# jtschwar/tomo_TV

Hardware: AMD Instinct MI355X
Metric: SART+TV Gvoxel-updates/s (ASD-POCS outer iterations x voxels, 512x512x512 x 90 tilts, at 1/2/4/8 GPU) (higher is better)
Workload: dtype f32; 1 GPU; ASD-POCS iteration (SART sweep beta0=0.25 + 10 TV-GD steps) on ONE 512x512x512 volume, 90 tilts -70..70 deg (headline SART+TV 512^3x90 = BASELINE configs[2] shape), 512 slices on rank 0; volume=512x512x512, slices_per_gpu=512, nray=512, nproj=90, sub_slab_engines_per_gpu=1, sart_chains_per_engine=1

## Files before the change

include/tomo_hip.h:

```cpp
#ifndef TOMO_HIP_H
#define TOMO_HIP_H

#include <stdint.h>

#ifdef __cplusplus
extern "C" {
#endif

typedef struct tomo_engine tomo_engine;

enum tomo_status { TOMO_OK = 0, TOMO_ERR_ARG = 1, TOMO_ERR_HIP = 2, TOMO_ERR_STATE = 3, TOMO_ERR_GEOMETRY = 4 };

enum tomo_volume { TOMO_VOL_RECON = 0, TOMO_VOL_TEMP = 1, TOMO_VOL_ORIGINAL = 2, TOMO_VOL_YK = 3, TOMO_VOL_RECON_OLD = 4,
                   TOMO_VOL_COUNT = 5,
                   TOMO_VOL_USER0 = 5,
                   TOMO_VOL_SLOTS = 5 + 40 };
enum tomo_sinogram { TOMO_SINO_B = 0, TOMO_SINO_G = 1, TOMO_SINO_R = 2 ,
                     TOMO_SINO_USER0 = 3,
                     TOMO_SINO_SLOTS = 3 + 40,
                     TOMO_SINO_YK_MODEL = 1000 };

enum tomo_scalar { TOMO_S_DD = 0,
                   TOMO_S_DIFF = 1,
                   TOMO_S_TV = 2,
// ... 49 lines not shown
int tomo_sirt_data(tomo_engine *e, int vol, int sino_b, int niter);
int tomo_sart(tomo_engine *e, int vol, float beta, int niter, const int32_t *order);
int tomo_sart_data(tomo_engine *e, int vol, int sino_b, float beta, int niter, const int32_t *order);
int tomo_sart_tracked(tomo_engine *e, int vol, int sino_b, float beta, int niter, const int32_t *order, int track_vol, int slot);
int tomo_cgls(tomo_engine *e, int vol, int niter);
int tomo_fbp(tomo_engine *e, const float *taps_host, float scale, int apply_positivity);
int tomo_art(tomo_engine *e, float beta);
int tomo_art_order(tomo_engine *e, float beta, const int32_t *order_host);
int tomo_poisson_ml(tomo_engine *e, float lambda);
int tomo_poisson_residual(tomo_engine *e, int vol, int sino_b, int sino_out);
int tomo_scale_volume(tomo_engine *e, int vol, float factor);
int tomo_positivity(tomo_engine *e, int vol);
int tomo_soft_threshold(tomo_engine *e, int vol, float lambda);
int tomo_fista_momentum(tomo_engine *e, float beta);
int tomo_fista_project_yk(tomo_engine *e, int *done);

int tomo_data_distance_sq(tomo_engine *e, int vol);
int tomo_data_distance_sq_async(tomo_engine *e, int vol);
int tomo_async_wait(tomo_engine *e);
int tomo_diff_norm_sq(tomo_engine *e, int a, int b, int slot);
int tomo_sino_diff_norm_sq(tomo_engine *e, int a, int b, int slot);
int tomo_sino_proj_max(tomo_engine *e, int sino, float *out_host);
int tomo_sino_proj_scale(tomo_engine *e, int sino, const float *div_host, const float *mul_host);
int tomo_l1_norm(tomo_engine *e, int vol);
int tomo_read_scalars(tomo_engine *e, double *out, int count);
int tomo_scalars_snapshot(tomo_engine *e);
int tomo_scalars_snapshot_read(tomo_engine *e, double *out, int count);
int tomo_bind_scalar_buffer(tomo_engine *e, void *device_doubles);

int tomo_bind_halo(tomo_engine *e, void *device_lo, void *device_hi);
int tomo_halo_pack(tomo_engine *e, int field, int last, void *device_dst);
int tomo_halo_pack_both(tomo_engine *e, int field, void *first_plane, void *last_plane);
int tomo_halo_local(tomo_engine *e, int field);
enum tomo_field { TOMO_FIELD_FGP_D = 100, TOMO_FIELD_FGP_P1 = 101 };
int tomo_wait_for(tomo_engine *e, tomo_engine *other);
int tomo_halo_from(tomo_engine *e, int field, tomo_engine *lo_src, tomo_engine *hi_src);
int tomo_scalar_sum_from(tomo_engine *e, int dst_slot, tomo_engine **srcs, int n, int src_slot);
int tomo_set_slab_edges(tomo_engine *e, int is_first, int is_last);

int tomo_tv_set_target(tomo_engine *e, int vol);
int tomo_tv_partial(tomo_engine *e, int vol, float eps);
int tomo_tv_grad(tomo_engine *e, float eps);
int tomo_tv_grad_tv(tomo_engine *e, float eps);
int tomo_tv_update(tomo_engine *e, float dPOCS, int clamp);
int tomo_tv_update_planes(tomo_engine *e, float dPOCS, int clamp, void *first_plane, void *last_plane);
int tomo_tv_grad_planes(tomo_engine *e, float eps, int with_tv, void *g_first, void *g_last);
int tomo_tv_halo_apply(tomo_engine *e, float dPOCS, int clamp, const void *g_lo, const void *g_hi);
int tomo_tv_update_tracked(tomo_engine *e, float dPOCS, int clamp, int track_vol, int slot);
int tomo_fgp_begin(tomo_engine *e);
int tomo_fgp_begin_vol(tomo_engine *e, int vol);
int tomo_fgp_obj(tomo_engine *e, float lambda);
int tomo_fgp_grad(tomo_engine *e, float lambda);
int tomo_fgp_end(tomo_engine *e, int iters);
int tomo_bind_fgp_halo(tomo_engine *e, void *lo, void *hi, void *send_first, void *send_last);
int tomo_bind_fgp_halo2(tomo_engine *e, void *lo, void *hi, void *send_first, void *send_last);
int tomo_fgp_fused_begin(tomo_engine *e, int vol);
int tomo_fgp_fused_step(tomo_engine *e, float lambda, int first_iteration);
int tomo_fgp_fused_step2(tomo_engine *e, float lambda, int first_iteration);
int tomo_fgp_fused_end(tomo_engine *e, float lambda);
int tomo_fgp_fused_last(tomo_engine *e, float lambda, int first_iteration);

int tomo_tv(tomo_engine *e, int vol, float eps);
int tomo_tv_gd(tomo_engine *e, int ng, float dPOCS, float eps);
int tomo_tv_gd_tracked(tomo_engine *e, int ng, float dPOCS, float eps, int track_vol, int slot);
int tomo_tv_fgp(tomo_engine *e, int iters, float lambda);
int tomo_tv_fgp_vol(tomo_engine *e, int vol, int iters, float lambda);
// ... 40 lines not shown
```

tomo_tv_amd/_lib.py:

```python
import ctypes
import os
import sys

_HERE = os.path.dirname(os.path.abspath(__file__))
LIB_PATH = os.path.join(_HERE, "libtomo_hip.so")

VOL_RECON, VOL_TEMP, VOL_ORIGINAL, VOL_YK, VOL_RECON_OLD = 0, 1, 2, 3, 4
SINO_B, SINO_G, SINO_R, SINO_USER0 = 0, 1, 2, 3
SINO_YK_MODEL = 1000
VOL_USER0 = 5
S_DD, S_DIFF, S_TV, S_GNORM, S_RMSE, S_COST, S_L1, S_DIFF2, S_GNORM_ALL, S_COUNT = 0, 1, 2, 3, 4, 5, 6, 7, 8, 16
FIELD_FGP_D, FIELD_FGP_P1 = 100, 101
K_BP_ANGLE, K_FP_ANGLE, K_TV_GRAD, K_TV_UPDATE, K_FGP_OBJ, K_FGP_GRAD, K_SART_FUSED, K_FP_TILE, K_BP_TILE, K_FP_REDUCE, K_SART_RESIDENT = range(11)
FORM_FP = ("rows", "tile", "strip", "list")
FORM_BP = ("all", "tile", "list")
FORM_SART = ("angle", "tile", "resident")

_i, _i64, _f, _p = ctypes.c_int, ctypes.c_int64, ctypes.c_float, ctypes.c_void_p
_pp = ctypes.POINTER(ctypes.c_void_p)

SIGNATURES = {
    "tomo_device_count": [ctypes.POINTER(_i)],
    "tomo_system_matrix": [_i, _i, _p, _i64, _p, _p, _p, ctypes.POINTER(_i64)],
    "tomo_create": [_i, _i, _i, _p, _i, _pp],
# ... 13 lines not shown
    "tomo_copy_volume": [_p, _i, _i],
    "tomo_copy_volume_from": [_p, _i, _p, _i],
    "tomo_forward_projection": [_p, _i, _i],
    "tomo_back_projection": [_p, _i, _i],
    "tomo_lipschitz": [_p, ctypes.POINTER(_f)],
    "tomo_row_inner_product": [_p],
    "tomo_sirt_landweber": [_p, _i, _f, _i],
    "tomo_sirt": [_p, _i, _i],
    "tomo_sirt_cimmino": [_p, _i, _f, _i],
    "tomo_lipschitz_cimmino": [_p, ctypes.POINTER(_f)],
    "tomo_release_geometry": [_p],
    "tomo_adopt_volumes": [_p, _p],
    "tomo_sart": [_p, _i, _f, _i, _p],
    "tomo_art": [_p, _f],
    "tomo_art_order": [_p, _f, _p],
    "tomo_poisson_ml": [_p, _f],
    "tomo_positivity": [_p, _i],
    "tomo_soft_threshold": [_p, _i, _f],
    "tomo_fista_momentum": [_p, _f],
    "tomo_fista_project_yk": [_p, ctypes.POINTER(_i)],
    "tomo_data_distance_sq": [_p, _i],
    "tomo_diff_norm_sq": [_p, _i, _i, _i],
    "tomo_data_distance_sq_async": [_p, _i],
    "tomo_async_wait": [_p],
    "tomo_l1_norm": [_p, _i],
    "tomo_read_scalars": [_p, _p, _i],
    "tomo_scalars_snapshot": [_p],
    "tomo_scalars_snapshot_read": [_p, _p, _i],
    "tomo_bind_scalar_buffer": [_p, _p],
    "tomo_bind_halo": [_p, _p, _p],
    "tomo_halo_pack": [_p, _i, _i, _p],
    "tomo_halo_pack_both": [_p, _i, _p, _p],
    "tomo_halo_local": [_p, _i],
    "tomo_set_slab_edges": [_p, _i, _i],
    "tomo_wait_for": [_p, _p],
    "tomo_halo_from": [_p, _i, _p, _p],
    "tomo_scalar_sum_from": [_p, _i, _p, _i, _i],
    "tomo_profile_intervals": [_p, _i, _p, _p, _p, _i, ctypes.POINTER(_i)],
    "tomo_tv_partial": [_p, _i, _f],
    "tomo_tv_set_target": [_p, _i],
    "tomo_tv_grad": [_p, _f],
    "tomo_tv_grad_tv": [_p, _f],
    "tomo_tv_update": [_p, _f, _i],
    "tomo_fgp_begin": [_p],
    "tomo_fgp_obj": [_p, _f],
    "tomo_fgp_grad": [_p, _f],
    "tomo_fgp_end": [_p, _i],
    "tomo_tv": [_p, _i, _f],
    "tomo_tv_gd": [_p, _i, _f, _f],
    "tomo_tv_fgp": [_p, _i, _f],
    "tomo_set_option": [_p, ctypes.c_char_p, _i],
    "tomo_get_option": [_p, ctypes.c_char_p, ctypes.POINTER(_i)],
    "tomo_set_sinogram": [_p, _i, _p],
    "tomo_cgls": [_p, _i, _i],
    "tomo_fbp": [_p, _p, _f, _i],
    "tomo_sirt_data": [_p, _i, _i, _i],
    "tomo_sart_data": [_p, _i, _i, _f, _i, _p],
    "tomo_sart_tracked": [_p, _i, _i, _f, _i, _p, _i, _i],
    "tomo_tv_update_tracked": [_p, _f, _i, _i, _i],
    "tomo_tv_update_planes": [_p, _f, _i, _p, _p],
    "tomo_tv_grad_planes": [_p, _f, _i, _p, _p],
    "tomo_tv_halo_apply": [_p, _f, _i, _p, _p],
    "tomo_tv_gd_tracked": [_p, _i, _f, _f, _i, _i],
    "tomo_poisson_residual": [_p, _i, _i, _i],
    "tomo_scale_volume": [_p, _i, _f],
    "tomo_sino_diff_norm_sq": [_p, _i, _i, _i],
# ... 74 lines not shown
```

tomo_tv_amd/csrc/engine_api.inc:

```


const char *tomo_last_error(void) { return g_err.c_str(); }

int tomo_device_count(int *count)
{
    if (!count) return fail(TOMO_ERR_ARG, "null count");
    int n = 0;
    hipError_t err = hipGetDeviceCount(&n);
    if (err != hipSuccess) { n = 0; (void)hipGetLastError(); }
    *count = n;
    return TOMO_OK;
}

int tomo_system_matrix(int nray, int nproj, const double *angles_rad, int64_t cap, float *rows, float *cols,
                       float *vals, int64_t *nnz)
{
    if (!angles_rad || !nnz) return fail(TOMO_ERR_ARG, "null argument");
    int rc = check_dims(1, nray, nproj);
    if (rc) return rc;
    Coo m;
    build_parallel_ray(nray, nproj, angles_rad, m);
    *nnz = m.ptr[m.nrow];
    if (cap == 0) return TOMO_OK;
    if (cap < *nnz || !rows || !cols || !vals) return fail(TOMO_ERR_ARG, "output capacity too small");
// ... 41 lines not shown
                     (void **)&e->d_rowcross, (void **)&e->d_cell,
                     (void **)&e->d_fs_items, (void **)&e->d_fs_orient, (void **)&e->d_fs_shift, (void **)&e->d_fs_cnt, (void **)&e->d_fs_gstart,
                     (void **)&e->d_fs_gseg0, (void **)&e->d_fs_ent, (void **)&e->d_fs_zero, (void **)&e->d_fs_rsptr, (void **)&e->d_fs_rsidx, (void **)&e->fs_part, (void **)&e->fs_part_aux,
                     (void **)&e->d_fl_items, (void **)&e->d_fl_orient, (void **)&e->d_fl_shift, (void **)&e->d_fl_ent, (void **)&e->d_fl_ptr, (void **)&e->d_fl_fent, (void **)&e->d_fl_fptr,
                     (void **)&e->d_fl_rsptr, (void **)&e->d_fl_rsidx, (void **)&e->d_fl_zero, (void **)&e->fl_part, (void **)&e->fl_part_aux,
                     (void **)&e->d_rs_hdr, (void **)&e->d_rs_cell, (void **)&e->d_rs_ts, (void **)&e->d_rs_rl, (void **)&e->rs_pb, (void **)&e->rs_rb, (void **)&e->d_rs_angs, (void **)&e->d_rs_abort, (void **)&e->d_rs_commit};
    for (void **p : ptrs) if (*p) { (void)hipFree(*p); *p = nullptr; }
    e->rs_ok = false; e->rs_angs_cap = 0; e->rs_angs_host.clear(); e->seg_ready = false;
    for (int i = 0; i < TOMO_SINO_SLOTS; ++i) if (e->sino[i]) { (void)hipFree(e->sino[i]); e->sino[i] = nullptr; }
    if (e->g_prev) { (void)hipFree(e->g_prev); e->g_prev = nullptr; }
    if (e->g_yk) { (void)hipFree(e->g_yk); e->g_yk = nullptr; }
    e->yk_claim.valid = false;
    e->g_prev_valid = e->mom_p_ok = e->mom.set = false;
    e->geometry_released = true;
}

int tomo_destroy(tomo_engine *e)
{
    if (!e) return TOMO_OK;
    (void)hipSetDevice(e->device);
    if (e->stream) (void)hipStreamSynchronize(e->stream);
    if (e->aux) { (void)hipStreamSynchronize(e->aux); (void)hipStreamDestroy(e->aux); (void)hipEventDestroy(e->ev_fork); (void)hipEventDestroy(e->ev_join); }
    for (int u = 0; u < tomo_engine::MAX_CHAINS; ++u) if (e->sub_stream[u]) { (void)hipStreamSynchronize(e->sub_stream[u]); (void)hipStreamDestroy(e->sub_stream[u]); (void)hipEventDestroy(e->ev_sjoin[u]); }
    for (int w = 0; w < 2; ++w) if (e->fp_red_stream[w]) { (void)hipStreamSynchronize(e->fp_red_stream[w]); (void)hipStreamDestroy(e->fp_red_stream[w]); for (int h = 0; h < 2; ++h) { (void)hipEventDestroy(e->ev_fp_tile[w][h]); (void)hipEventDestroy(e->ev_fp_red[w][h]); } }
    comm_release(e);
    if (e->ev_sfork) (void)hipEventDestroy(e->ev_sfork);
    if (e->ev_peer) (void)hipEventDestroy(e->ev_peer);
    if (e->ev_snap) (void)hipEventDestroy(e->ev_snap);
    if (e->h_snap) (void)hipHostFree(e->h_snap);
    if (e->rs_abort) (void)hipHostFree(e->rs_abort);
    if (e->rs_done) (void)hipHostFree(e->rs_done);
    free_geometry(e);
    void *ptrs[] = {e->tv_alt, e->halo_lo_alt, e->halo_hi_alt, e->d_part_tv, e->d_part_aux, e->fgp_q[0], e->fgp_q[1], e->fgp_q[2], e->cg_p, e->cg_z, e->cg_sums, e->cg_part, e->cg_coef, e->sart_alt,
                    e->tvg, e->fgp_p[0], e->fgp_p[1], e->fgp_p[2], e->stage, e->d_scal_own, e->d_part, e->halo_lo_own, e->halo_hi_own};
    for (void *p : ptrs) if (p) (void)hipFree(p);
    for (int i = 0; i < TOMO_VOL_SLOTS; ++i) if (e->vol[i]) (void)hipFree(e->vol[i]);
    for (auto &p : e->prof) { for (auto ev : p.ev) (void)hipEventDestroy(ev); if (p.ref) (void)hipEventDestroy(p.ref); }
    if (e->own_stream && e->stream) (void)hipStreamDestroy(e->stream);
    delete e;
    return TOMO_OK;
}

int tomo_release_geometry(tomo_engine *e)
{
    NEED(e);
    HIPCHK(hipStreamSynchronize(e->stream));
    if (e->aux) HIPCHK(hipStreamSynchronize(e->aux));
    for (int u = 0; u < tomo_engine::MAX_CHAINS; ++u) if (e->sub_stream[u]) HIPCHK(hipStreamSynchronize(e->sub_stream[u]));
    e->async_pending = false;
    free_geometry(e);
    return TOMO_OK;
}

int tomo_adopt_volumes(tomo_engine *dst, tomo_engine *src)
{
    if (!dst || !src) return fail(TOMO_ERR_ARG, "null engine");
    if (dst->nx != src->nx || dst->n != src->n || dst->sx != src->sx || dst->device != src->device) return fail(TOMO_ERR_ARG, "engines differ in slab shape or device");
    HIPCHK(hipSetDevice(dst->device));
    HIPCHK(hipStreamSynchronize(src->stream));
    if (src->aux) HIPCHK(hipStreamSynchronize(src->aux));
    for (int u = 0; u < tomo_engine::MAX_CHAINS; ++u) if (src->sub_stream[u]) HIPCHK(hipStreamSynchronize(src->sub_stream[u]));
    src->async_pending = false;
    HIPCHK(hipStreamSynchronize(dst->stream));
    for (int i = 0; i < TOMO_VOL_SLOTS; ++i) {
        if (!src->vol[i]) continue;
        if (dst->vol[i]) HIPCHK(hipFree(dst->vol[i]));
        dst->vol[i] = src->vol[i];
        src->vol[i] = nullptr;
    }
    dst->old_is_recon = src->old_is_recon;
    src->old_is_recon = false;
    for (int i = 0; i < TOMO_VOL_SLOTS; ++i) ++dst->vol_version[i];
    g_clear(dst);
    return TOMO_OK;
}

int tomo_set_stream(tomo_engine *e, void *hip_stream)
{
    NEED(e);
    HIPCHK(hipStreamSynchronize(e->stream));
    if (e->own_stream) { HIPCHK(hipStreamDestroy(e->stream)); e->own_stream = false; }
    e->stream = (hipStream_t)hip_stream;
    return TOMO_OK;
}

int tomo_synchronize(tomo_engine *e) { NEED(e); HIPCHK(hipStreamSynchronize(e->stream)); return TOMO_OK; }
int tomo_get_device(tomo_engine *e, int *device) { if (!e || !device) return fail(TOMO_ERR_ARG, "null"); *device = e->device; return TOMO_OK; }
int tomo_get_dims(tomo_engine *e, int *nslice, int *nray, int *nproj, int64_t *nnz)
{
    if (!e) return fail(TOMO_ERR_ARG, "null engine");
    if (nslice) *nslice = e->nx;
    if (nray) *nray = e->n;
    if (nproj) *nproj = e->np;
    if (nnz) *nnz = e->nnz;
    return TOMO_OK;
}

int tomo_sart_chain_count(tomo_engine *e, int *count)
{
    if (!e || !count) return fail(TOMO_ERR_ARG, "null");
    *count = chain_count(e);
    return TOMO_OK;
}

static int upload(tomo_engine *e, const float *host, float *dst, int64_t m)
{
// ... 22 lines not shown
}

int tomo_set_sinogram(tomo_engine *e, int which, const float *b)
{
    NEED(e);
    if (!b) return fail(TOMO_ERR_ARG, "null sinogram");
    float *dst; int rc = sino_slot(e, which, &dst); if (rc) return rc;
    return upload(e, b, dst, e->nrows);
}

int tomo_set_tilt_series(tomo_engine *e, const float *b) { return tomo_set_sinogram(e, TOMO_SINO_B, b); }

int tomo_get_sinogram(tomo_engine *e, int which, float *out)
{
    NEED(e);
    if (!out) return fail(TOMO_ERR_ARG, "null output");
    if (which == TOMO_SINO_YK_MODEL) {
        const float *yk = projection_in_hand(e, TOMO_VOL_YK);
        if (!yk) return fail(TOMO_ERR_STATE, "no projection of the extrapolated point in hand (tomo_fista_project_yk)");
        return download(e, yk, out, e->nrows);
    }
    float *src;
    int rc = sino_slot(e, which, &src);
    if (rc) return rc;
    return download(e, src, out, e->nrows);
}

int tomo_set_volume(tomo_engine *e, int vol, const float *data)
{
    NEED(e);
    { int rc_ = order_after_async(e); if (rc_) return rc_; }
    float *dst; int rc = get_vol(e, vol, &dst); if (rc) return rc;
    if (!data) return fail(TOMO_ERR_ARG, "null volume");
    return upload(e, data, dst, e->npix);
}

int tomo_get_volume(tomo_engine *e, int vol, float *data)
{
    NEED(e);
    float *src; int rc = get_vol_ro(e, vol, &src); if (rc) return rc;
    if (!data) return fail(TOMO_ERR_ARG, "null volume");
    return download(e, src, data, e->npix);
}

int tomo_set_slice(tomo_engine *e, int vol, int s, const float *img)
{
    NEED(e);
    { int rc_ = order_after_async(e); if (rc_) return rc_; }
    float *dst; int rc = get_vol(e, vol, &dst); if (rc) return rc;
    if (s < 0 || s >= e->nx || !img) return fail(TOMO_ERR_ARG, "slice index out of range");
    if ((rc = ensure_stage(e, e->npix * sizeof(float)))) return rc;
    HIPCHK(hipMemcpyAsync(e->stage, img, e->npix * sizeof(float), hipMemcpyHostToDevice, e->stream));
    hipLaunchKernelGGL(k_scatter_slice, dim3((unsigned)((e->npix + 255) / 256)), dim3(256), 0, e->stream, e->stage, dst, e->npix, e->sx, s);
    LAUNCHCHK();
    HIPCHK(hipStreamSynchronize(e->stream));
    return TOMO_OK;
}

int tomo_get_slice(tomo_engine *e, int vol, int s, float *img)
{
    NEED(e);
    float *src; int rc = get_vol_ro(e, vol, &src); if (rc) return rc;
    if (s < 0 || s >= e->nx || !img) return fail(TOMO_ERR_ARG, "slice index out of range");
    if ((rc = ensure_stage(e, e->npix * sizeof(float)))) return rc;
    hipLaunchKernelGGL(k_gather_slice, dim3((unsigned)((e->npix + 255) / 256)), dim3(256), 0, e->stream, src, e->stage, e->npix, e->sx, s);
    LAUNCHCHK();
    HIPCHK(hipMemcpyAsync(img, e->stage, e->npix * sizeof(float), hipMemcpyDeviceToHost, e->stream));
    HIPCHK(hipStreamSynchronize(e->stream));
    return TOMO_OK;
}

int tomo_restart_recon(tomo_engine *e)
{
    NEED(e);
    { int rc_ = order_after_async(e); if (rc_) return rc_; }
    HIPCHK(hipMemsetAsync(e->vol[TOMO_VOL_RECON], 0, e->vol_elems() * sizeof(float), e->stream));
    if (e->vol[TOMO_VOL_YK]) HIPCHK(hipMemsetAsync(e->vol[TOMO_VOL_YK], 0, e->vol_elems() * sizeof(float), e->stream));
    if (e->vol[TOMO_VOL_RECON_OLD]) HIPCHK(hipMemsetAsync(e->vol[TOMO_VOL_RECON_OLD], 0, e->vol_elems() * sizeof(float), e->stream));
    e->old_is_recon = false;
    ++e->vol_version[TOMO_VOL_RECON]; ++e->vol_version[TOMO_VOL_YK]; ++e->vol_version[TOMO_VOL_RECON_OLD];
    return TOMO_OK;
}

int tomo_copy_volume(tomo_engine *e, int dst, int src)
{
    NEED(e);
    { int rc_ = order_after_async(e); if (rc_) return rc_; }
    float *d, *s; int rc;
    const bool g_src = g_is_projection_of(e, src);
    if ((rc = get_vol(e, dst, &d)) || (rc = get_vol_ro(e, src, &s))) return rc;
    if (d != s) HIPCHK(hipMemcpyAsync(d, s, e->vol_elems() * sizeof(float), hipMemcpyDeviceToDevice, e->stream));
    if (g_src && dst != src) { e->g_valid[1].vol = dst; e->g_valid[1].ver = e->vol_version[dst]; }
    return TOMO_OK;
}

int tomo_forward_projection(tomo_engine *e, int vol, int sino)
{
    NEED(e);
    { int rc_ = order_after_async(e); if (rc_) return rc_; }
    float *x, *g; int rc;
    if ((rc = get_vol_ro(e, vol, &x))) return rc;
    if ((rc = sino_slot(e, sino, &g))) return rc;
    if ((rc = launch_fp_all<FP_STORE>(e, x, nullptr, g))) return rc;
    if (sino == TOMO_SINO_G) g_set(e, vol);
    return TOMO_OK;
}

int tomo_back_projection(tomo_engine *e, int sino, int vol)
{
    NEED(e);
    float *x, *g; int rc;
    if ((rc = get_vol(e, vol, &x))) return rc;
// ... 25 lines not shown
    const float *rs = e->d_rowsum;
    for (int it = 0; it < niter; ++it) {
        e->d_rowsum = e->d_rowinner;
        rc = launch_fp_all<FP_RESID_MUL>(e, x, e->sino[TOMO_SINO_B], r);
        e->d_rowsum = const_cast<float *>(rs);
        if (rc) return rc;
        if ((rc = launch_bp_all(e, x, r, nullptr, 1.f, beta / (float)e->nrows, 1))) return rc;
    }
    return TOMO_OK;
}

int tomo_sirt(tomo_engine *e, int vol, int niter) { return tomo_sirt_data(e, vol, TOMO_SINO_B, niter); }

int tomo_sirt_data(tomo_engine *e, int vol, int sino_b, int niter)
{
    NEED(e);
    float *x, *r, *b; int rc;
    const float *have = (niter > 0 && sino_b != TOMO_SINO_G) ? projection_in_hand(e, vol) : nullptr;
    const bool reuse = have != nullptr;
    if (reuse) { if ((rc = order_after_async(e))) return rc; }
    if ((rc = get_vol(e, vol, &x)) || (rc = get_sino(e, &e->sino[TOMO_SINO_R], &r)) || (rc = sino_slot(e, sino_b, &b))) return rc;
    for (int it = 0; it < niter; ++it) {
        if (it == 0 && reuse) { if ((rc = launch_sino_resid<FP_RESID_NORM>(e, b, have, r))) return rc; }
        else if ((rc = launch_fp_all<FP_RESID_NORM>(e, x, b, r))) return rc;
        if ((rc = launch_bp_all(e, x, r, e->d_colsum_all, 1.f, 1.f, 1))) return rc;
    }
    return TOMO_OK;
}

static std::mutex g_rs_mu;
static hipEvent_t g_rs_last[64] = {};

static int launch_sart_resident(tomo_engine *e, float *x, float beta, int64_t steps, const std::function<int(int64_t)> &angle_at, float *track,
                                std::vector<std::pair<int, int>> &failed)
{
    failed.clear();
    if (steps > (int64_t)1 << 24) return fail(TOMO_ERR_ARG, "too many SART steps in one call");
    const int c0 = e->sub_nc ? e->sub_c0 : 0, nc = e->sub_nc ? e->sub_nc : e->sxc / 64;
    const int groups = std::max(1, std::min(e->rs_groups, nc)), rounds = (nc + groups - 1) / groups;
    {
        std::vector<int> seq((size_t)steps);
        for (int64_t k = 0; k < steps; ++k) seq[(size_t)k] = angle_at(k);
        if (seq != e->rs_angs_host) {
            HIPCHK(hipStreamSynchronize(e->stream));
            if ((size_t)steps > e->rs_angs_cap) {
                if (e->d_rs_angs) { HIPCHK(hipFree(e->d_rs_angs)); e->d_rs_angs = nullptr; e->rs_angs_cap = 0; }
                HIPCHK(hipMalloc((void **)&e->d_rs_angs, (size_t)steps * sizeof(int)));
                e->rs_angs_cap = (size_t)steps;
            }
            HIPCHK(hipMemcpy(e->d_rs_angs, seq.data(), (size_t)steps * sizeof(int), hipMemcpyHostToDevice));
            e->rs_angs_host.swap(seq);
        }
    }
    const uint64_t need = (uint64_t)rounds * (uint64_t)steps;
    if ((uint64_t)e->rs_epoch + need + 16 > 0xFFFFFFFFull) {
        HIPCHK(hipMemsetAsync(e->rs_pb, 0, e->rs_pb_bytes, e->stream));
        HIPCHK(hipMemsetAsync(e->rs_rb, 0, e->rs_rb_bytes, e->stream));
        e->rs_epoch = 0;
    }
    if (c0 != 0 || nc != e->sxc / 64) return fail(TOMO_ERR_STATE, "the resident sweep covers the whole slab");
    if (e->rs_commit_dirty || e->rs_commit_base > 0x7F000000u) {
        HIPCHK(hipMemsetAsync(e->d_rs_commit, 0, (size_t)(e->sxc / 64) * sizeof(unsigned), e->stream));
        e->rs_commit_base = 0; e->rs_commit_dirty = false;
    }
    if (++e->rs_seq >= 0x7FFFFFF0u) { std::memset(e->rs_done, 0, (size_t)(e->sxc / 64) * sizeof(int)); e->rs_seq = 1; }
    RsArgs A{};
    A.x = x; A.b = e->cur_b; A.rowsum = e->d_rowsum; A.hdr = e->d_rs_hdr; A.cell = e->d_rs_cell; A.ts = e->d_rs_ts; A.rl = e->d_rs_rl;
    A.pb = e->rs_pb; A.rb = e->rs_rb; A.angs = e->d_rs_angs; A.track = track; A.part = e->d_part; A.abort_word = e->d_rs_abort; A.abort_host = e->rs_abort;
    A.commit = e->d_rs_commit; A.done_host = e->rs_done; A.seq = e->rs_seq; A.commit_base = e->rs_commit_base; A.test_fail = e->rs_test_fail;
    A.n = e->n; A.sx = e->sx; A.np = e->np; A.ntiles = e->rs_ntiles; A.tiles = e->rs_tiles; A.rpt = e->rs_rpt; A.steps = (int)steps; A.chunk0 = c0; A.nchunk = nc;
    A.epoch0 = e->rs_epoch; A.spin_limit = e->rs_spin_limit; A.beta = beta; A.prof = nullptr;
    e->rs_epoch += (uint32_t)need;
    if (e->device < 0 || e->device >= 64) return fail(TOMO_ERR_ARG, "device index");
    {
        std::lock_guard<std::mutex> lk(g_rs_mu);
        hipEvent_t &last = g_rs_last[e->device];
        if (!last) HIPCHK(hipEventCreateWithFlags(&last, hipEventDisableTiming));
        else HIPCHK(hipStreamWaitEvent(e->stream, last, 0));
        {
            ProfScope ps(e, TOMO_K_SART_RESIDENT);
            hipLaunchKernelGGL(k_sart_resident, dim3((unsigned)(e->rs_ntiles * groups)), dim3(RS_THREADS), 0, e->stream, A);
            LAUNCHCHK();
        }
        HIPCHK(hipEventRecord(last, e->stream));
    }
    HIPCHK(hipStreamSynchronize(e->stream));
    int nfailed = 0;
    for (int c = c0; c < c0 + nc; ++c) {
        if (e->rs_done[c] == (int)e->rs_seq) continue;
        ++nfailed;
        if (!failed.empty() && failed.back().first + failed.back().second == c) ++failed.back().second;
        else failed.emplace_back(c, 1);
    }
    if (nfailed) {
        e->rs_commit_dirty = true;
        e->rs_last_code = *e->rs_abort;
        *e->rs_abort = 0;
        HIPCHK(hipMemsetAsync(e->d_rs_abort, 0, sizeof(int), e->stream));
        ++e->rs_fallbacks;
        e->rs_fallback_chunks += nfailed;
        e->rs_backoff = std::min(64, std::max(1, 2 * e->rs_backoff));
        e->rs_skip = e->rs_backoff;
    } else {
        e->rs_commit_base += (unsigned)e->rs_ntiles;
        e->rs_backoff = 0;
    }
    return TOMO_OK;
}

int tomo_sart(tomo_engine *e, int vol, float beta, int niter, const int32_t *order)
{
    return tomo_sart_data(e, vol, TOMO_SINO_B, beta, niter, order);
}

static int sart_impl(tomo_engine *e, int vol, int sino_b, float beta, int niter, const int32_t *order, int track_vol, int slot)
{
    NEED(e);
    float *x, *r, *track = nullptr; int rc;
    if ((rc = get_vol(e, vol, &x)) || (rc = get_sino(e, &e->sino[TOMO_SINO_R], &r)) || (rc = sino_slot(e, sino_b, &e->cur_b))) return rc;
    if (track_vol >= 0) {
        if (track_vol == vol) return fail(TOMO_ERR_ARG, "the tracked volume must differ from the swept one");
        if (slot < 0 || slot >= TOMO_S_COUNT) return fail(TOMO_ERR_ARG, "bad scalar slot");
        if ((rc = get_vol(e, track_vol, &track))) return rc;
        if ((int64_t)niter * e->np <= 0) {
            if ((rc = tomo_diff_norm_sq(e, vol, track_vol, slot))) return rc;
            return tomo_copy_volume(e, track_vol, vol);
        }
        if ((rc = reduce_begin(e))) return rc;
    }
    auto finish = [&]() -> int { return track ? reduce_end(e, slot) : TOMO_OK; };
    if (order) {
        std::vector<char> seen(e->np, 0);
        for (int q = 0; q < e->np; ++q) {
            if (order[q] < 0 || order[q] >= e->np || seen[order[q]]) return fail(TOMO_ERR_ARG, "SART order is not a permutation of the angles");
            seen[order[q]] = 1;
        }
    }
    const int64_t steps = (int64_t)niter * e->np;
    auto angle_at = [&](int64_t k) { int q = (int)(k % e->np); return order ? order[q] : q; };
    if (!e->sart_fused) {
        for (int64_t k = 0; k < steps; ++k) {
            int i = angle_at(k);
            {
                ProfScope ps(e, TOMO_K_FP_ANGLE);
                if ((rc = launch_fp<FP_RESID_NORM>(e, x, i * e->n, e->n, e->cur_b, r))) return rc;
            }
            if ((rc = launch_bp_angle(e, x, i, r + (size_t)i * e->n * e->sx, beta, k == steps - 1 ? track : nullptr))) return rc;
        }
        return finish();
    }
    if (steps <= 0) return TOMO_OK;
    int form = select_forms(e).sart;
    if (form == TOMO_FORM_SART_RESIDENT && e->rs_skip > 0 && e->sart_resident != 1) {
        --e->rs_skip;
        form = TOMO_FORM_SART_TILE;
    }
    auto sweep_tiles = [&](const std::vector<std::pair<int, int>> *ranges) -> int {
        const bool coop = e->sart_coop && e->np >= 2 && steps >= 2 && !ranges;
        int rc2;
        if ((rc2 = sart_tile_prepare(e, coop))) return rc2;
        const uint32_t epoch0 = e->st_epoch + 1;
// ... 3 lines not shown
            if (coop) {
                float *pk = (k & 1) ? e->st_partial2 : e->st_partial, *pk1 = (k & 1) ? e->st_partial : e->st_partial2;
                if (k == 0) return launch_sart_tile<false>(e, sb, x, 0, angle_at(0), r, beta, pk, false);
                if (k == steps) {
                    int last = angle_at(steps - 1);
                    if ((rc3 = launch_resid_finish_tile(e, sb, pk1, last, r))) return rc3;
                    return launch_bp_angle(e, sb, x, last, r + (size_t)last * e->n * e->sx, beta, track);
                }
                return launch_sart_coop(e, sb, x, angle_at(k - 1), angle_at(k), r, beta, pk1, pk, epoch0 + (uint32_t)k, k);
            }
            if (k == 0) return launch_sart_tile<false>(e, sb, x, 0, angle_at(0), r, beta);
            if (k == steps) { int last = angle_at(steps - 1); return launch_bp_angle(e, sb, x, last, r + (size_t)last * e->n * e->sx, beta, track); }
            int prev = angle_at(k - 1), next = angle_at(k);
            if (prev == next) {
                if ((rc3 = launch_bp_angle(e, sb, x, prev, r + (size_t)prev * e->n * e->sx, beta))) return rc3;
                return launch_sart_tile<false>(e, sb, x, 0, next, r, beta);
            }
            return launch_sart_tile<true>(e, sb, x, prev, next, r, beta, nullptr, true, k);
        };
        auto chain = [&](const Sub &sb) -> int {
            for (int64_t k = 0; k <= steps; ++k) { int rc3 = link(k, sb); if (rc3) return rc3; }
            return TOMO_OK;
        };
        if (!ranges) return run_chains(e, chain);
        for (const auto &rg : *ranges) {
            const int c0 = rg.first, nc = rg.second;
            const int vec = (c0 % 4 == 0 && nc % 4 == 0) ? 4 : (c0 % 2 == 0 && nc % 2 == 0) ? 2 : 1;
            if ((rc2 = chain(Sub{e->stream, c0, nc, vec}))) return rc2;
        }
        return TOMO_OK;
    };
    if (form == TOMO_FORM_SART_RESIDENT) {
        std::vector<std::pair<int, int>> failed;
        if ((rc = launch_sart_resident(e, x, beta, steps, angle_at, track, failed))) return rc;
        if (!failed.empty() && (rc = sweep_tiles(&failed))) return rc;
        return finish();
    }
    if (e->sart_resident == 1 && !e->rs_ok) return fail(TOMO_ERR_STATE, "\"sart_resident\" = 1, but this engine has no tables of the resident sweep (N not a multiple of 8, more 32 x 32 tiles than CUs, or a matrix whose ray windows do not fit)");
    if (form == TOMO_FORM_SART_TILE) {
        if ((rc = sweep_tiles(nullptr))) return rc;
        return finish();
    }
    float *alt;
    if ((rc = ensure_seg_tables(e))) return rc;
    if ((rc = get_scratch(e, &e->sart_alt, &alt))) return rc;
    float *cur = x;
    if ((rc = launch_sart_seg<false>(e, cur, nullptr, 0, angle_at(0), r, beta))) return rc;
    for (int64_t k = 1; k < steps; ++k) {
        int prev = angle_at(k - 1), next = angle_at(k);
        if (prev == next) {
            if ((rc = launch_bp_angle(e, cur, prev, r + (size_t)prev * e->n * e->sx, beta))) return rc;
            if ((rc = launch_fp<FP_RESID_NORM>(e, cur, next * e->n, e->n, e->cur_b, r))) return rc;
            continue;
        }
        if ((rc = launch_sart_seg<true>(e, cur, alt, prev, next, r, beta))) return rc;
        std::swap(cur, alt);
    }
    int last = angle_at(steps - 1);
    if ((rc = launch_bp_angle(e, cur, last, r + (size_t)last * e->n * e->sx, beta, track))) return rc;
    if (cur != x) { e->vol[vol] = cur; e->sart_alt = x; }
    return finish();
}

int tomo_sart_data(tomo_engine *e, int vol, int sino_b, float beta, int niter, const int32_t *order)
{
    return sart_impl(e, vol, sino_b, beta, niter, order, -1, 0);
}

int tomo_sart_tracked(tomo_engine *e, int vol, int sino_b, float beta, int niter, const int32_t *order, int track_vol, int slot)
{
    return sart_impl(e, vol, sino_b, beta, niter, order, track_vol, slot);
}

int tomo_art(tomo_engine *e, float beta) { return tomo_art_order(e, beta, nullptr); }

int tomo_art_order(tomo_engine *e, float beta, const int32_t *order_host)
{
    NEED(e);
    float *x;
    { int rc_ = get_vol(e, TOMO_VOL_RECON, &x); if (rc_) return rc_; }
    int32_t *d_order = nullptr;
    if (order_host) {
        std::vector<char> seen(e->nrows, 0);
        for (int64_t q = 0; q < e->nrows; ++q) {
            if (order_host[q] < 0 || order_host[q] >= e->nrows || seen[order_host[q]]) return fail(TOMO_ERR_ARG, "row order is not a permutation");
            seen[order_host[q]] = 1;
        }
        int rc = ensure_stage(e, e->nrows * sizeof(int32_t)); if (rc) return rc;
        HIPCHK(hipMemcpyAsync(e->stage, order_host, e->nrows * sizeof(int32_t), hipMemcpyHostToDevice, e->stream));
        d_order = (int32_t *)e->stage;
    }
    if (!order_host && e->art_chain && e->art_chain_ok) {
        float *d, *a; int rc;
// ... 37 lines not shown
            LAUNCHCHK();
            const CellD *cell = e->d_cell + (size_t)i * e->npix;
            const float *ai = a + (size_t)i * e->n * e->sx;
            switch (e->vec) {
            case 4: hipLaunchKernelGGL((k_bp_art<4, BP_PPW>), bgrid, dim3(256), 0, e->stream, x, cell, ai, beta, (int)e->npix, e->sx, ngroups, nchunk, slab_streams(e) ? 1 : 0, 0); break;
            case 2: hipLaunchKernelGGL((k_bp_art<2, BP_PPW>), bgrid, dim3(256), 0, e->stream, x, cell, ai, beta, (int)e->npix, e->sx, ngroups, nchunk, slab_streams(e) ? 1 : 0, 0); break;
            default: hipLaunchKernelGGL((k_bp_art<1, BP_PPW>), bgrid, dim3(256), 0, e->stream, x, cell, ai, beta, (int)e->npix, e->sx, ngroups, nchunk, slab_streams(e) ? 1 : 0, 0); break;
            }
            LAUNCHCHK();
        }
        return tomo_positivity(e, TOMO_VOL_RECON);
    }
    hipLaunchKernelGGL(k_art, dim3(e->sxc / 64), dim3(64 * ART_WAVES), 0, e->stream, x, e->d_rptr, e->d_rent, e->sino[TOMO_SINO_B], e->d_rowinner, beta, (int)e->nrows, e->sx, d_order);
    LAUNCHCHK();
    int rc = tomo_positivity(e, TOMO_VOL_RECON);
    if (!rc && order_host) HIPCHK(hipStreamSynchronize(e->stream));
    return rc;
}

int tomo_poisson_ml(tomo_engine *e, float lambda)
{
    int rc;
    if ((rc = tomo_poisson_residual(e, TOMO_VOL_RECON, TOMO_SINO_B, TOMO_SINO_R))) return rc;
    float *x;
    if ((rc = get_vol(e, TOMO_VOL_RECON, &x))) return rc;
    return launch_bp_all(e, x, e->sino[TOMO_SINO_R], nullptr, 1.f, -(lambda / e->lipschitz), 1);
}

int tomo_poisson_residual(tomo_engine *e, int vol, int sino_b, int sino_out)
{
    NEED(e);
    float *x, *b, *r; int rc;
    if ((rc = get_vol(e, vol, &x)) || (rc = sino_slot(e, sino_b, &b)) || (rc = sino_slot(e, sino_out, &r))) return rc;
    if ((rc = reduce_begin(e))) return rc;
    if ((rc = launch_fp_all<FP_POISSON>(e, x, b, r))) return rc;
    return reduce_end(e, TOMO_S_COST);
}

static int slice_sumsq(tomo_engine *e, const float *v, int64_t m, double *sums)
{
    const int cols = e->sx / 4, per = cols >= 256 ? 256 : (cols >= 128 ? 128 : 64);
    const int nby = (int)std::min<int64_t>(1024, std::max<int64_t>(1, (m + 63) / 64));
    const int rpb = (int)((m + nby - 1) / nby);
    if (!e->cg_part) { int rc = dev_alloc((void **)&e->cg_part, (size_t)1024 * e->sx * sizeof(double), false, e->stream); if (rc) return rc; }
    dim3 grid((unsigned)((cols + per - 1) / per), (unsigned)nby);
    hipLaunchKernelGGL(k_slice_sumsq, grid, dim3(256), 0, e->stream, v, e->cg_part, m, e->sx, rpb);
    LAUNCHCHK();
    hipLaunchKernelGGL(k_slice_sumsq_finish, dim3((e->sx + 255) / 256), dim3(256), 0, e->stream, (const double *)e->cg_part, sums, nby, e->sx);
    LAUNCHCHK();
    return TOMO_OK;
}

static unsigned slice_grid(const tomo_engine *e, int64_t n4)
{
    const int64_t unit = std::max(1, e->sx / 64);
    int64_t b = std::min<int64_t>((n4 + 255) / 256, 8192);
    b = std::max<int64_t>(unit, (b / unit) * unit);
    return (unsigned)b;
}

int tomo_cgls(tomo_engine *e, int vol, int niter)
{
    NEED(e);
    float *x, *r, *b, *w; int rc;
    const bool reuse_g = g_is_projection_of(e, vol);
    if (reuse_g) { if ((rc = order_after_async(e))) return rc; }
    if ((rc = get_vol(e, vol, &x)) || (rc = get_sino(e, &e->sino[TOMO_SINO_R], &r)) || (rc = sino_slot(e, TOMO_SINO_B, &b))) return rc;
// ... 163 lines not shown
    { int rc_ = order_after_async(e); if (rc_) return rc_; }
    float *x; int rc; if ((rc = get_vol(e, vol, &x))) return rc;
    int64_t n4 = e->vol_elems() / 4;
    hipLaunchKernelGGL(k_clamp, dim3(grid_1d(n4)), dim3(256), 0, e->stream, (f4 *)x, n4);
    LAUNCHCHK();
    return TOMO_OK;
}

int tomo_soft_threshold(tomo_engine *e, int vol, float lambda)
{
    NEED(e);
    float *x; int rc; if ((rc = get_vol(e, vol, &x))) return rc;
    int64_t n4 = e->vol_elems() / 4;
    hipLaunchKernelGGL(k_soft_threshold, dim3(grid_1d(n4)), dim3(256), 0, e->stream, (f4 *)x, lambda, n4);
    LAUNCHCHK();
    return TOMO_OK;
}

int tomo_fista_momentum(tomo_engine *e, float beta)
{
    NEED(e);
    { int rc_ = order_after_async(e); if (rc_) return rc_; }
    e->mom_p_ok = e->g_prev_valid && e->mom.set && e->vol_version[TOMO_VOL_RECON] == e->mom.ver_recon
                  && e->vol_version[TOMO_VOL_RECON_OLD] == e->mom.ver_old && e->g_prev_recon_ver == e->vol_version[TOMO_VOL_RECON];
    float *x, *yk, *old; int rc;
    const bool aliased = e->old_is_recon;
    if ((rc = get_vol_ro(e, TOMO_VOL_RECON, &x)) || (rc = get_vol_ro(e, TOMO_VOL_YK, &yk))) return rc;
    if (aliased) old = x;
    else if ((rc = get_vol_ro(e, TOMO_VOL_RECON_OLD, &old))) return rc;
    int64_t n4 = e->vol_elems() / 4;
    hipLaunchKernelGGL(k_momentum, dim3(grid_1d(n4)), dim3(256), 0, e->stream, (const f4 *)yk, (const f4 *)old, (f4 *)x, beta, n4);
    LAUNCHCHK();
    ++e->vol_version[TOMO_VOL_RECON]; ++e->vol_version[TOMO_VOL_YK]; ++e->vol_version[TOMO_VOL_RECON_OLD];
    e->vol[TOMO_VOL_RECON] = yk;
    e->vol[TOMO_VOL_YK] = x;
    e->old_is_recon = true;
    e->mom.beta = beta; e->mom.set = true;
    e->mom.ver_recon = e->vol_version[TOMO_VOL_RECON]; e->mom.ver_yk = e->vol_version[TOMO_VOL_YK]; e->mom.ver_old = e->vol_version[TOMO_VOL_RECON_OLD];
    return TOMO_OK;
}

int tomo_fista_project_yk(tomo_engine *e, int *done)
{
    NEED(e);
    if (done) *done = 0;
    if (!e->fp_reuse || !g_is_projection_of(e, TOMO_VOL_RECON) || !e->mom.set) return TOMO_OK;
    if (e->vol_version[TOMO_VOL_RECON] != e->mom.ver_recon || e->vol_version[TOMO_VOL_YK] != e->mom.ver_yk) return TOMO_OK;
    { int rc_ = order_after_async(e); if (rc_) return rc_; }
    int rc; float *p, *q;
    if ((rc = get_sino(e, &e->g_prev, &p)) || (rc = get_sino(e, &e->g_yk, &q))) return rc;
    const float *g = e->sino[TOMO_SINO_G];
    const int64_t n4 = (int64_t)e->sino_elems() / 4;
    const bool have_prev = e->mom_p_ok;
    e->yk_claim.valid = false;
    if (have_prev) {
        hipLaunchKernelGGL(k_sino_extrapolate, dim3(grid_1d(n4)), dim3(256), 0, e->stream, (const VecOf<4>::T *)g, (VecOf<4>::T *)p, (VecOf<4>::T *)q, e->mom.beta, n4);
        LAUNCHCHK();
    } else {
        HIPCHK(hipMemcpyAsync(p, g, e->sino_elems() * sizeof(float), hipMemcpyDeviceToDevice, e->stream));
    }
    e->g_prev_valid = true;
    e->g_prev_recon_ver = e->vol_version[TOMO_VOL_RECON];
    if (have_prev) {
        e->yk_claim.valid = true; e->yk_claim.ver = e->vol_version[TOMO_VOL_YK];
        if (done) *done = 1;
    } else if (e->mom.beta == 0.f) {
        e->g_valid[1].vol = TOMO_VOL_YK; e->g_valid[1].ver = e->vol_version[TOMO_VOL_YK];
        if (done) *done = 1;
    }
    return TOMO_OK;
}

int tomo_data_distance_sq(tomo_engine *e, int vol)
{
    NEED(e);
    float *x, *g; int rc;
    if ((rc = get_vol_ro(e, vol, &x)) || (rc = get_sino(e, &e->sino[TOMO_SINO_G], &g))) return rc;
    if ((rc = reduce_begin(e))) return rc;
    if ((rc = launch_fp_all<FP_DD>(e, x, e->sino[TOMO_SINO_B], g))) return rc;
    g_set(e, vol);
    return reduce_end(e, TOMO_S_DD);
}

int tomo_data_distance_sq_async(tomo_engine *e, int vol)
{
    NEED(e);
    if (e->async_pending) return fail(TOMO_ERR_STATE, "an asynchronous evaluation is already in flight");
    if (!e->aux) {
        HIPCHK(hipStreamCreateWithFlags(&e->aux, hipStreamNonBlocking));
        HIPCHK(hipEventCreateWithFlags(&e->ev_fork, hipEventDisableTiming));
        HIPCHK(hipEventCreateWithFlags(&e->ev_join, hipEventDisableTiming));
        int rc = dev_alloc((void **)&e->d_part_aux, NPART * sizeof(double), true, e->stream);
        if (rc) return rc;
    }
    float *tmp; int rc;
    if ((rc = get_vol_ro(e, vol, &tmp)) || (rc = get_sino(e, &e->sino[TOMO_SINO_G], &tmp))) return rc;
    HIPCHK(hipEventRecord(e->ev_fork, e->stream));
    HIPCHK(hipStreamWaitEvent(e->aux, e->ev_fork, 0));
    hipStream_t main_stream = e->stream;
    double *main_part = e->d_part;
    e->stream = e->aux; e->d_part = e->d_part_aux;
    rc = tomo_data_distance_sq(e, vol);
    e->stream = main_stream; e->d_part = main_part;
    if (rc) return rc;
    HIPCHK(hipEventRecord(e->ev_join, e->aux));
    e->async_pending = true;
    return TOMO_OK;
}

int tomo_async_wait(tomo_engine *e)
{
// ... 76 lines not shown
```

tomo_tv_amd/csrc/engine_create.inc:

```

template <class V> static void release(V &v) { V().swap(v); }

static int build_seg_tables(tomo_engine *e, const Coo &m, Tables &t)
{
    int rc;
    build_walk(m, e->n, e->np, t);
    {
        std::vector<uint2> went(t.walk_pix.size() ? t.walk_pix.size() : 1);
        for (size_t k = 0; k < t.walk_pix.size(); ++k) { uint32_t bits; std::memcpy(&bits, &t.walk_w[k], 4); went[k] = make_uint2(t.walk_pix[k], bits); }
        if ((rc = dev_alloc((void **)&e->d_wptr, t.walk_ptr.size() * 4, false, e->stream))) return rc;
        if ((rc = dev_alloc((void **)&e->d_went, went.size() * sizeof(uint2), false, e->stream))) return rc;
        HIPCHK(hipMemcpy(e->d_wptr, t.walk_ptr.data(), t.walk_ptr.size() * 4, hipMemcpyHostToDevice));
        HIPCHK(hipMemcpy(e->d_went, went.data(), t.walk_pix.size() * sizeof(uint2), hipMemcpyHostToDevice));
    }
    {
        const int seg_len = 32;
        build_segments(e->n, e->np, seg_len, t);
        static_assert(sizeof(Tables::SegItem) == sizeof(SegItemD), "segment item layout");
        e->h_seg_exec_ptr = t.seg_exec_ptr;
        e->max_items = t.max_items_per_angle;
        if ((rc = dev_alloc((void **)&e->d_seg_exec, std::max<size_t>(1, t.seg_exec.size()) * sizeof(SegItemD), false, e->stream))) return rc;
        if ((rc = dev_alloc((void **)&e->d_row_first, t.row_first.size() * 4, false, e->stream))) return rc;
        if ((rc = dev_alloc((void **)&e->d_row_nseg, t.row_nseg.size() * 4, false, e->stream))) return rc;
        HIPCHK(hipMemcpy(e->d_seg_exec, t.seg_exec.data(), t.seg_exec.size() * sizeof(SegItemD), hipMemcpyHostToDevice));
// ... 220 lines not shown
        e->bl_ok = false;
        if (e->fb_ok) {
            if ((rc = dev_alloc((void **)&e->d_fb_cell, t.bp_cell.size() * sizeof(uint4), false, e->stream))) return rc;
            if ((rc = dev_alloc((void **)&e->d_fb_win, t.bp_win.size() * 4, false, e->stream))) return rc;
            HIPCHK(hipMemcpy(e->d_fb_cell, t.bp_cell.data(), t.bp_cell.size() * sizeof(uint4), hipMemcpyHostToDevice));
            HIPCHK(hipMemcpy(e->d_fb_win, t.bp_win.data(), t.bp_win.size() * 4, hipMemcpyHostToDevice));
            release(t.bp_cell);
        }
        lap("build_bp_tiles + upload");
        static_assert(BL_TY == Tables::BL_TY && BL_TZ == Tables::BL_TZ && BL_WAVES == Tables::BL_WAVES && BL_A == Tables::BL_A && BL_MAXR == Tables::BL_MAXR &&
                      BL_ROWB == Tables::BL_ROWB && BL_BATCH == Tables::BL_BATCH, "k_bp_list geometry (sysmat.h)");
        build_bp_lists(e->n, e->np, BL_TY, BL_TZ, BL_A, BL_MAXR, BL_ROWB, BL_WAVES, BL_BATCH, Tables::BL_REGS, t);
        e->bl_ok = t.bl_ok && (e->np + BL_A - 1) / BL_A <= 64;
        if (e->bl_ok) {
            const size_t nent = (size_t)(t.bl_nbatch + 1) * BL_BATCH;
            e->bl_tiles_z = (e->n + BL_TZ - 1) / BL_TZ;
            e->bl_ntiles = ((e->n + BL_TY - 1) / BL_TY) * e->bl_tiles_z;
            if ((rc = dev_alloc((void **)&e->d_bl_ent, nent * sizeof(uint4), false, e->stream))) return rc;
            if ((rc = dev_alloc((void **)&e->d_bl_ptr, t.bl_ptr.size() * 4, false, e->stream))) return rc;
            if ((rc = dev_alloc((void **)&e->d_bl_win, t.bl_win.size() * 4, false, e->stream))) return rc;
            HIPCHK(hipMemcpy(e->d_bl_ent, t.bl_ent.get(), nent * sizeof(uint4), hipMemcpyHostToDevice));
            HIPCHK(hipMemcpy(e->d_bl_ptr, t.bl_ptr.data(), t.bl_ptr.size() * 4, hipMemcpyHostToDevice));
            HIPCHK(hipMemcpy(e->d_bl_win, t.bl_win.data(), t.bl_win.size() * 4, hipMemcpyHostToDevice));
            t.bl_ent.reset();
        }
        release(t.bl_win); release(t.bl_ptr);
    }
    lap("build_bp_lists + upload");
    static_assert(sizeof(Cell) == sizeof(CellD), "cell layout");
    HIPCHK(hipMemcpy(e->d_cell, t.cell.data(), t.cell.size() * sizeof(CellD), hipMemcpyHostToDevice));
    g_alloc_meter = nullptr;
    if ((rc = dev_alloc((void **)&e->d_scal_own, TOMO_S_COUNT * sizeof(double), true, e->stream))) return rc;
    if ((rc = dev_alloc((void **)&e->d_part, NPART * sizeof(double), true, e->stream))) return rc;
    e->d_scal = e->d_scal_own;
    if ((rc = dev_alloc((void **)&e->halo_lo_own, e->npix * sizeof(float), true, e->stream))) return rc;
    if ((rc = dev_alloc((void **)&e->halo_hi_own, e->npix * sizeof(float), true, e->stream))) return rc;
    e->halo_lo = e->halo_lo_own; e->halo_hi = e->halo_hi_own;
    float *tmp;
    if ((rc = get_vol(e, TOMO_VOL_RECON, &tmp))) return rc;
    if ((rc = get_sino(e, &e->sino[TOMO_SINO_B], &tmp))) return rc;
    HIPCHK(hipStreamSynchronize(e->stream));
    *out = e;
    return TOMO_OK;
}

extern "C" int tomo_destroy(tomo_engine *e);

static int finish_create(tomo_engine *e, Coo &m, tomo_engine **out, double t_begin)
{
    int rc = finish_create_impl(e, m, out);
    e->create_ms = (std::chrono::duration<double>(std::chrono::steady_clock::now().time_since_epoch()).count() - t_begin) * 1e3;
    if (rc) {
        std::string first = g_err;
        tomo_destroy(e);
        g_err = first;
    }
    return rc;
}

static tomo_engine *new_engine(int nslice, int nray, int nproj, int device)
{
    tomo_engine *e = new tomo_engine();
    e->nx = nslice; e->n = nray; e->np = nproj; e->device = device;
    e->sxc = ((nslice + 63) / 64) * 64;
    e->vec = (e->sxc % 256 == 0) ? 4 : (e->sxc % 128 == 0) ? 2 : 1;
    e->sx = e->sxc;
// ... 63 lines not shown
```

tomo_tv_amd/csrc/engine_launch.inc:

```

template <int MODE>
static int launch_fp(tomo_engine *e, const float *x, int row0, int nrows, const float *b, float *out, int lpr = 0)
{
    if (lpr == 16 || lpr == 32) {
        int R = 64 / lpr;
        int nchunk = e->sxc / (lpr * 4);
        int64_t waves = (int64_t)((nrows + R - 1) / R) * nchunk;
        dim3 grid((unsigned)((waves + 3) / 4)), block(256);
        if (lpr == 16) hipLaunchKernelGGL((k_fp_rows_g<16, MODE>), grid, block, 0, e->stream, x, e->d_rptr, e->d_rent, b, e->d_rowsum, out, e->d_part, row0, nrows, e->sx, nchunk);
        else hipLaunchKernelGGL((k_fp_rows_g<32, MODE>), grid, block, 0, e->stream, x, e->d_rptr, e->d_rent, b, e->d_rowsum, out, e->d_part, row0, nrows, e->sx, nchunk);
        LAUNCHCHK();
        return TOMO_OK;
    }
    int vec = e->vec;
    int nchunk = e->sxc / (64 * vec);
    dim3 grid((unsigned)((int64_t)nrows * nchunk)), block(256);
    switch (vec) {
    case 4: hipLaunchKernelGGL((k_fp_rows<4, MODE>), grid, block, 0, e->stream, x, e->d_rptr, e->d_rent, b, e->d_rowsum, out, e->d_part, row0, nrows, e->sx); break;
    case 2: hipLaunchKernelGGL((k_fp_rows<2, MODE>), grid, block, 0, e->stream, x, e->d_rptr, e->d_rent, b, e->d_rowsum, out, e->d_part, row0, nrows, e->sx); break;
    default: hipLaunchKernelGGL((k_fp_rows<1, MODE>), grid, block, 0, e->stream, x, e->d_rptr, e->d_rent, b, e->d_rowsum, out, e->d_part, row0, nrows, e->sx); break;
    }
    LAUNCHCHK();
    return TOMO_OK;
}

template <int MODE>
static void launch_fp_reduce(tomo_engine *e, hipStream_t rs, const float *part, const uint32_t *rsptr, const uint32_t *rsidx, const float *b,
                             float *out, int c0, int ncp)
{
    int lpr = (ncp % 4 == 0) ? 64 : (ncp % 2 == 0) ? 32 : 16;
    int64_t items = (int64_t)e->nrows * (ncp * 16 / lpr);
    int64_t waves = (items + 64 / lpr - 1) / (64 / lpr);
    dim3 grid((unsigned)((waves + 3) / 4)), block(256);
    switch (lpr) {
    case 64: hipLaunchKernelGGL((k_fp_tile_reduce<64, MODE>), grid, block, 0, rs, part, rsptr, rsidx, b, e->d_rowsum, out, e->d_part, (int)e->nrows, e->sx, c0, ncp); break;
    case 32: hipLaunchKernelGGL((k_fp_tile_reduce<32, MODE>), grid, block, 0, rs, part, rsptr, rsidx, b, e->d_rowsum, out, e->d_part, (int)e->nrows, e->sx, c0, ncp); break;
    default: hipLaunchKernelGGL((k_fp_tile_reduce<16, MODE>), grid, block, 0, rs, part, rsptr, rsidx, b, e->d_rowsum, out, e->d_part, (int)e->nrows, e->sx, c0, ncp); break;
    }
}

template <int MODE>
static int launch_fp_strip(tomo_engine *e, const float *x, const float *b, float *out)
{
    const int nchunk = e->sxc / 64;
    if (!e->fs_ncp) {
        size_t per_chunk = (size_t)std::max<uint32_t>(1, e->fs_nseg) * 64 * sizeof(float);
        int ncp = (int)std::min<size_t>(nchunk, std::max<size_t>(1, e->ft_scratch_cap / per_chunk));
        if (e->ft_ncp_forced > 0) ncp = std::min(nchunk, e->ft_ncp_forced);
        else if (ncp >= 4) ncp &= ~3; else if (ncp >= 2) ncp &= ~1;
        e->fs_ncp = ncp;
    }
    const int which = (e->aux && e->stream == e->aux) ? 1 : 0;
    float **slot = which ? &e->fs_part_aux : &e->fs_part;
    if (!*slot) {
        int rc = dev_alloc((void **)slot, (size_t)std::max<uint32_t>(1, e->fs_nseg) * e->fs_ncp * 64 * sizeof(float), false, e->stream);
        if (rc) return rc;
    }
    for (int c0 = 0; c0 < nchunk; c0 += e->fs_ncp) {
        const int ncp = std::min(e->fs_ncp, nchunk - c0);
        {
            ProfScope ps(e, TOMO_K_FP_TILE);
            dim3 grid((unsigned)(8 * ((e->fs_nitems + 7) / 8) * ncp)), block(FS_THREADS);
#define FS_LAUNCH(KK) hipLaunchKernelGGL((k_fp_strip<KK>), grid, block, 0, e->stream, x, e->d_fs_items, e->d_fs_orient, e->d_fs_shift, e->d_fs_cnt, \
                                         e->d_fs_gstart, e->d_fs_gseg0, e->d_fs_ent, *slot, e->n, e->sx, e->fs_nitems, c0, ncp, e->d_fs_zero)
            if (e->fs_kused <= 8) FS_LAUNCH(8); else if (e->fs_kused <= 12) FS_LAUNCH(12); else FS_LAUNCH(16);
#undef FS_LAUNCH
            LAUNCHCHK();
        }
        {
            ProfScope ps(e, TOMO_K_FP_REDUCE);
            launch_fp_reduce<MODE>(e, e->stream, *slot, e->d_fs_rsptr, e->d_fs_rsidx, b, out, c0, ncp);
            LAUNCHCHK();
        }
    }
    return TOMO_OK;
}

template <int MODE>
static int launch_fp_list(tomo_engine *e, const float *x, const float *b, float *out)
{
    const int nchunk = e->sxc / 64;
    if (!e->fl_ncp) {
        size_t per_chunk = (size_t)std::max<uint32_t>(1, e->fl_nseg) * 64 * sizeof(float);
        int ncp = (int)std::min<size_t>(nchunk, std::max<size_t>(2, e->ft_scratch_cap / per_chunk));
        if (e->ft_ncp_forced > 0) ncp = std::min(nchunk, std::max(2, e->ft_ncp_forced));
        if (ncp >= 4) ncp &= ~3; else ncp = 2;
        e->fl_ncp = ncp;
    }
    if (!e->attr_fl) {
        HIPCHK(hipFuncSetAttribute((const void *)k_fp_list, hipFuncAttributeMaxDynamicSharedMemorySize, FL_LDS_BYTES));
        e->attr_fl = true;
    }
    const int which = (e->aux && e->stream == e->aux) ? 1 : 0;
    float **slot = which ? &e->fl_part_aux : &e->fl_part;
    if (!*slot) {
        int rc = dev_alloc((void **)slot, (size_t)std::max<uint32_t>(1, e->fl_nseg) * e->fl_ncp * 64 * sizeof(float), false, e->stream);
        if (rc) return rc;
    }
    for (int c0 = 0; c0 < nchunk; c0 += e->fl_ncp) {
        const int ncp = std::min(e->fl_ncp, nchunk - c0);
        {
            ProfScope ps(e, TOMO_K_FP_TILE);
            dim3 grid((unsigned)(8 * ((e->fl_nitems + 7) / 8) * (ncp / 2))), block(FL_THREADS);
            hipLaunchKernelGGL(k_fp_list, grid, block, FL_LDS_BYTES, e->stream, x, e->d_fl_items, e->d_fl_orient, e->d_fl_shift, e->d_fl_ent, e->d_fl_ptr,
                               e->d_fl_fent, e->d_fl_fptr, *slot, e->n, e->sx, e->fl_nitems, c0 / 2, ncp / 2, ncp, e->d_fl_zero);
            LAUNCHCHK();
        }
        {
            ProfScope ps(e, TOMO_K_FP_REDUCE);
            launch_fp_reduce<MODE>(e, e->stream, *slot, e->d_fl_rsptr, e->d_fl_rsidx, b, out, c0, ncp);
            LAUNCHCHK();
        }
    }
    return TOMO_OK;
}

struct Forms { int fp, bp, sart; };
static Forms select_forms(const tomo_engine *e)
{
    Forms f;
    f.fp = (e->fp_strip && e->fp_list && e->fl_ok && e->sxc % 128 == 0) ? TOMO_FORM_FP_LIST
         : (e->fp_strip && e->fs_ok) ? TOMO_FORM_FP_STRIP
         : e->fp_tile ? TOMO_FORM_FP_TILE : TOMO_FORM_FP_ROWS;
    f.bp = (e->bp_tile && e->bl_ok && e->bp_list && e->sxc % 128 == 0) ? TOMO_FORM_BP_LIST
         : (e->bp_tile && e->fb_ok) ? TOMO_FORM_BP_TILE : TOMO_FORM_BP_ALL;
    f.sart = !e->sart_fused ? TOMO_FORM_SART_ANGLE
           : (e->sart_resident != 0 && e->rs_ok) ? TOMO_FORM_SART_RESIDENT
           : (e->sart_tile && e->st_ok) ? TOMO_FORM_SART_TILE : TOMO_FORM_SART_ANGLE;
    return f;
}

template <int MODE>
static int launch_fp_all(tomo_engine *e, const float *x, const float *b, float *out)
{
    const int form = select_forms(e).fp;
    if (form == TOMO_FORM_FP_LIST) return launch_fp_list<MODE>(e, x, b, out);
    if (form == TOMO_FORM_FP_STRIP) return launch_fp_strip<MODE>(e, x, b, out);
    if (form == TOMO_FORM_FP_ROWS) return launch_fp<MODE>(e, x, 0, (int)e->nrows, b, out, e->fp_all_lpr);
    const int nchunk = e->sxc / 64;
    if (!e->ft_ncp) {
        size_t per_chunk = (size_t)std::max<uint32_t>(1, e->ft_nseg) * 64 * sizeof(float);
        int ncp = (int)std::min<size_t>(nchunk, std::max<size_t>(1, e->ft_scratch_cap / per_chunk));
        if (e->ft_ncp_forced > 0) ncp = std::min(nchunk, e->ft_ncp_forced);
// ... 16 lines not shown
    if (!*slot) {
        size_t chunks = std::max<size_t>(e->ft_ncp, 2 * (size_t)((((e->sxc / 64 + 1) / 2) + 1) & ~1));
        int rc = dev_alloc((void **)slot, (size_t)std::max<uint32_t>(1, e->ft_nseg) * chunks * 64 * sizeof(float), false, e->stream);
        if (rc) return rc;
    }
    if (pipe && !e->fp_red_stream[which]) {
        HIPCHK(hipStreamCreateWithFlags(&e->fp_red_stream[which], hipStreamNonBlocking));
        for (int h = 0; h < 2; ++h) {
            HIPCHK(hipEventCreateWithFlags(&e->ev_fp_tile[which][h], hipEventDisableTiming));
            HIPCHK(hipEventCreateWithFlags(&e->ev_fp_red[which][h], hipEventDisableTiming));
        }
    }
    const size_t half_elems = (size_t)std::max<uint32_t>(1, e->ft_nseg) * ncp_call * 64;
    int k = 0;
    for (int c0 = 0; c0 < nchunk; c0 += ncp_call, ++k) {
        int ncp = std::min(ncp_call, nchunk - c0);
        const int half = k & 1;
        float *part = *slot + (pipe ? half * half_elems : 0);
        hipStream_t rs = pipe ? e->fp_red_stream[which] : e->stream;
        if (pipe && k >= 2) HIPCHK(hipStreamWaitEvent(e->stream, e->ev_fp_red[which][half], 0));
        {
            ProfScope ps(e, TOMO_K_FP_TILE);
            dim3 grid((unsigned)(8 * ((e->ft_ntiles + 7) / 8) * ncp)), block(FT_THREADS);
            hipLaunchKernelGGL(k_fp_tile, grid, block, FT_LDS_BYTES, e->stream, x, e->d_ft_slot_ptr, e->d_ft_slot_seg0, e->d_ft_tent, part,
                               e->n, e->sx, e->ft_tiles_z, e->ft_ntiles, c0, ncp);
            LAUNCHCHK();
        }
        if (pipe) {
            HIPCHK(hipEventRecord(e->ev_fp_tile[which][half], e->stream));
            HIPCHK(hipStreamWaitEvent(rs, e->ev_fp_tile[which][half], 0));
        }
        {
            ProfScope ps(e, TOMO_K_FP_REDUCE, rs);
            launch_fp_reduce<MODE>(e, rs, part, e->d_ft_rsptr, e->d_ft_rsidx, b, out, c0, ncp);
            LAUNCHCHK();
        }
        if (pipe) HIPCHK(hipEventRecord(e->ev_fp_red[which][half], rs));
    }
    if (pipe) {
        HIPCHK(hipStreamWaitEvent(e->stream, e->ev_fp_red[which][0], 0));
        if (k >= 2) HIPCHK(hipStreamWaitEvent(e->stream, e->ev_fp_red[which][1], 0));
    }
    return TOMO_OK;
}

template <int MODE>
static int launch_sino_resid(tomo_engine *e, const float *b, const float *g, float *out)
{
    const int64_t n4 = (int64_t)e->sino_elems() / 4;
    hipLaunchKernelGGL((k_sino_resid<MODE>), dim3(grid_1d(n4)), dim3(256), 0, e->stream, b, g, e->d_rowsum, out, n4, e->sx / 4);
    LAUNCHCHK();
    return TOMO_OK;
}

constexpr int BP_PPW = 4;

static int launch_bp_angle(tomo_engine *e, const Sub &sb, float *x, int angle, const float *r_angle, float beta, float *track = nullptr)
{
    ProfScope ps(e, TOMO_K_BP_ANGLE, sb.stream);
    const int vec = sub_vec(e, sb);
    int nchunk = e->sxc / (64 * vec), chunk0 = 0;
    if (sb.nc) { nchunk = sb.nc / vec; chunk0 = sb.c0 / vec; }
    int ngroups = (int)((e->npix + BP_PPW - 1) / BP_PPW);
    int64_t waves = (int64_t)ngroups * nchunk;
    dim3 grid((unsigned)((waves + 3) / 4)), block(256);
    const CellD *cell = e->d_cell + (size_t)angle * e->npix;
    if (track) {
// ... 212 lines not shown
```

tomo_tv_amd/csrc/engine_options.inc:

```

int tomo_get_option(tomo_engine *e, const char *name, int *value)
{
    if (!e || !name || !value) return fail(TOMO_ERR_ARG, "null argument");
    if (std::strcmp(name, "fp_strip") == 0) { *value = e->fp_strip; return TOMO_OK; }
    if (std::strcmp(name, "fp_strip_ready") == 0) { *value = e->fs_ok ? 1 : 0; return TOMO_OK; }
    if (std::strcmp(name, "fp_strip_slots") == 0) { *value = e->fs_ok ? e->fs_kused : 0; return TOMO_OK; }
    if (std::strcmp(name, "fp_tile") == 0) { *value = e->fp_tile; return TOMO_OK; }
    if (std::strcmp(name, "bp_tile") == 0) { *value = e->bp_tile; return TOMO_OK; }
    if (std::strcmp(name, "bp_list") == 0) { *value = e->bp_list; return TOMO_OK; }
    if (std::strcmp(name, "fgp_pair") == 0) { *value = e->fgp_pair; return TOMO_OK; }
    if (std::strcmp(name, "fp_list") == 0) { *value = e->fp_list; return TOMO_OK; }
    if (std::strcmp(name, "fp_list_ready") == 0) { *value = e->fl_ok ? 1 : 0; return TOMO_OK; }
    if (std::strcmp(name, "bp_list_ready") == 0) { *value = e->bl_ok ? 1 : 0; return TOMO_OK; }
    if (std::strcmp(name, "fp_reuse") == 0) { *value = e->fp_reuse; return TOMO_OK; }
    if (std::strcmp(name, "art_chain_ready") == 0) { *value = e->art_chain_ok ? 1 : 0; return TOMO_OK; }
    if (std::strcmp(name, "sart_tile") == 0) { *value = e->sart_tile; return TOMO_OK; }
    if (std::strcmp(name, "sart_resident") == 0) { *value = e->sart_resident; return TOMO_OK; }
    if (std::strcmp(name, "sart_resident_ready") == 0) { *value = e->rs_ok ? 1 : 0; return TOMO_OK; }
    if (std::strcmp(name, "sart_resident_active") == 0) { *value = (e->rs_ok && e->sart_resident != 0) ? 1 : 0; return TOMO_OK; }
    if (std::strcmp(name, "sart_resident_spin") == 0) { *value = (int)std::min<uint32_t>(e->rs_spin_limit, 0x7FFFFFFFu); return TOMO_OK; }
    if (std::strcmp(name, "sart_resident_fallbacks") == 0) { *value = e->rs_fallbacks; return TOMO_OK; }
    if (std::strcmp(name, "sart_resident_fallback_chunks") == 0) { *value = e->rs_fallback_chunks; return TOMO_OK; }
    if (std::strcmp(name, "sart_resident_skip") == 0) { *value = e->rs_skip; return TOMO_OK; }
    if (std::strcmp(name, "sart_resident_last_code") == 0) { *value = e->rs_last_code; return TOMO_OK; }
    if (std::strcmp(name, "table_kib") == 0) { *value = (int)std::min<size_t>(e->table_bytes >> 10, 0x7FFFFFFF); return TOMO_OK; }
    if (std::strcmp(name, "create_ms") == 0) { *value = (int)std::min(e->create_ms + 0.5, 2147483647.0); return TOMO_OK; }
    if (std::strcmp(name, "tv_halo_fold") == 0) { *value = e->tv_halo_fold; return TOMO_OK; }
    if (std::strcmp(name, "form_fp") == 0) { *value = select_forms(e).fp; return TOMO_OK; }
    if (std::strcmp(name, "form_bp") == 0) { *value = select_forms(e).bp; return TOMO_OK; }
    if (std::strcmp(name, "form_sart") == 0) { *value = select_forms(e).sart; return TOMO_OK; }
    if (std::strcmp(name, "rccl_version") == 0) { *value = g_rccl.version; return TOMO_OK; }
    if (std::strcmp(name, "comm_rounds") == 0) { *value = (int)std::min<int64_t>(e->comm_rounds, 0x7FFFFFFF); return TOMO_OK; }
    return fail(TOMO_ERR_ARG, std::string("unknown option ") + name);
}

int tomo_set_option(tomo_engine *e, const char *name, int value)
{
    if (!e || !name) return fail(TOMO_ERR_ARG, "null argument");
    if (std::strcmp(name, "fgp_fused") == 0) { e->fgp_fused = value ? 1 : 0; return TOMO_OK; }
    if (std::strcmp(name, "fgp_pair") == 0) { e->fgp_pair = value ? 1 : 0; return TOMO_OK; }
    if (std::strcmp(name, "sart_fused") == 0) { e->sart_fused = value ? 1 : 0; return TOMO_OK; }
    if (std::strcmp(name, "fp_all_lpr") == 0) { e->fp_all_lpr = (value == 16 || value == 32) ? value : 0; return TOMO_OK; }
    if (std::strcmp(name, "art_chain") == 0) { e->art_chain = value ? 1 : 0; return TOMO_OK; }
    if (std::strcmp(name, "sart_tile") == 0) { e->sart_tile = value ? 1 : 0; return TOMO_OK; }
    if (std::strcmp(name, "sart_resident") == 0) { e->sart_resident = value < 0 ? -1 : (value ? 1 : 0); e->rs_skip = e->rs_backoff = 0; return TOMO_OK; }
    if (std::strcmp(name, "sart_resident_spin") == 0) { e->rs_spin_limit = value < 0 ? (1u << 21) : (uint32_t)value; return TOMO_OK; }
    if (std::strcmp(name, "sart_resident_test_fail") == 0) { e->rs_test_fail = std::max(0, value); return TOMO_OK; }
    if (std::strcmp(name, "fp_reuse") == 0) { e->fp_reuse = value != 0; g_clear(e); e->yk_claim.valid = false; return TOMO_OK; }
    if (std::strcmp(name, "fp_tile_pipe") == 0) { e->fp_tile_pipe = std::max(0, value); return TOMO_OK; }
    if (std::strcmp(name, "sart_streams") == 0) { e->sart_streams = value >= 2 ? std::min(value, (int)tomo_engine::MAX_CHAINS) : (value == 1 ? 1 : 0); return TOMO_OK; }
    if (std::strcmp(name, "art_tile") == 0) { e->art_tile = value ? 1 : 0; return TOMO_OK; }
    if (std::strcmp(name, "sart_skip_same") == 0) { e->sart_skip_same = value ? 1 : 0; return TOMO_OK; }
    if (std::strcmp(name, "sart_nt") == 0) { e->sart_nt = value < 0 ? -1 : (value ? 1 : 0); return TOMO_OK; }
    if (std::strcmp(name, "sart_coop") == 0) { e->sart_coop = value ? 1 : 0; return TOMO_OK; }
    if (std::strcmp(name, "sart_coop_spin") == 0) { e->sart_coop_spin = value < 0 ? -1 : value; return TOMO_OK; }
    if (std::strcmp(name, "bp_tile") == 0) { e->bp_tile = value ? 1 : 0; return TOMO_OK; }
    if (std::strcmp(name, "bp_list") == 0) { e->bp_list = value ? 1 : 0; return TOMO_OK; }
    if (std::strcmp(name, "bp_list_band") == 0) { e->bp_list_band = value ? 1 : 0; return TOMO_OK; }
    if (std::strcmp(name, "fp_list") == 0) { e->fp_list = value ? 1 : 0; return TOMO_OK; }
    if (std::strcmp(name, "fp_strip") == 0) { e->fp_strip = value ? 1 : 0; return TOMO_OK; }
    if (std::strcmp(name, "fp_tile") == 0) { e->fp_tile = value ? 1 : 0; e->fp_strip = 0; return TOMO_OK; }
    if (std::strcmp(name, "fp_tile_chunks_per_pass") == 0) {
        if (value < 0 || e->ft_part || e->ft_part_aux || e->fs_part || e->fs_part_aux || e->fl_part || e->fl_part_aux) return fail(TOMO_ERR_STATE, "fp_tile_chunks_per_pass must be set before the first projection");
        e->ft_ncp_forced = value; e->ft_ncp = 0; e->fs_ncp = 0; e->fl_ncp = 0; return TOMO_OK;
    }
    if (std::strcmp(name, "fp_tile_scratch_mib") == 0) {
        if (value <= 0 || e->ft_part || e->ft_part_aux || e->fs_part || e->fs_part_aux || e->fl_part || e->fl_part_aux) return fail(TOMO_ERR_STATE, "fp_tile_scratch_mib must be positive and set before the first projection");
        e->ft_scratch_cap = (size_t)value << 20; e->ft_ncp = 0; e->fs_ncp = 0; e->fl_ncp = 0; return TOMO_OK;
    }
    if (std::strcmp(name, "tv_gnorm_slot") == 0) {
        if (value < 0 || value >= TOMO_S_COUNT) return fail(TOMO_ERR_ARG, "bad scalar slot");
        e->gnorm_slot = value; return TOMO_OK;
    }
    if (std::strcmp(name, "tv_tz") == 0) { e->tv_tz = value == 4 ? 4 : 8; return TOMO_OK; }
    if (std::strcmp(name, "tv_halo_fold") == 0) { e->tv_halo_fold = value < 0 ? -1 : (value ? 1 : 0); return TOMO_OK; }
    if (std::strcmp(name, "tv_march4") == 0) { e->tv_march4 = value ? 1 : 0; return TOMO_OK; }
    if (std::strcmp(name, "tv_yseg") == 0) { e->tv_yseg = value < 0 ? 0 : value; return TOMO_OK; }
    if (std::strcmp(name, "tv_recompute") == 0) { e->tv_recompute = value ? 1 : 0; return TOMO_OK; }
    if (std::strcmp(name, "tv_lds") == 0) { e->tv_lds = value; return TOMO_OK; }
    return fail(TOMO_ERR_ARG, std::string("unknown option ") + name);
}

int tomo_profile_enable(tomo_engine *e, int kernel, int on)
{
    NEED(e);
    if (kernel < 0 || kernel >= PROF_MAX_KERNELS) return fail(TOMO_ERR_ARG, "bad kernel id");
    HIPCHK(hipStreamSynchronize(e->stream));
    e->prof[kernel].on = on != 0;
    e->prof[kernel].stride = on > 1 ? (unsigned)on : 1u;
    e->prof[kernel].seen = 0;
    e->prof[kernel].used = 0;
    e->prof[kernel].dropped = 0;
    if (on) {
        if (!e->prof[kernel].ref) HIPCHK(hipEventCreate(&e->prof[kernel].ref));
        HIPCHK(hipEventRecord(e->prof[kernel].ref, e->stream));
    }
    return TOMO_OK;
}

int tomo_profile_read2(tomo_engine *e, int kernel, int64_t *launches, double *total_ms, double *busy_ms)
{
    NEED(e);
    if (kernel < 0 || kernel >= PROF_MAX_KERNELS || !launches || !total_ms) return fail(TOMO_ERR_ARG, "bad argument");
    HIPCHK(hipStreamSynchronize(e->stream));
    for (int u = 0; u < tomo_engine::MAX_CHAINS; ++u) if (e->sub_stream[u]) HIPCHK(hipStreamSynchronize(e->sub_stream[u]));
    if (e->aux) HIPCHK(hipStreamSynchronize(e->aux));
// ... 59 lines not shown
```

tomo_tv_amd/csrc/engine_tv.inc:

```

static int field_ptr(tomo_engine *e, int field, float **out)
{
    if (field == TOMO_FIELD_FGP_D) return get_scratch(e, &e->tvg, out);
    if (field == TOMO_FIELD_FGP_P1) return get_scratch(e, &e->fgp_p[0], out);
    return get_vol_ro(e, field, out);
}

int tomo_bind_halo(tomo_engine *e, void *device_lo, void *device_hi)
{
    NEED(e);
    HIPCHK(hipStreamSynchronize(e->stream));
    e->halo_lo = device_lo ? (float *)device_lo : e->halo_lo_own;
    e->halo_hi = device_hi ? (float *)device_hi : e->halo_hi_own;
    return TOMO_OK;
}

int tomo_halo_pack(tomo_engine *e, int field, int last, void *device_dst)
{
    NEED(e);
    float *x; int rc; if ((rc = field_ptr(e, field, &x))) return rc;
    if (!device_dst) return fail(TOMO_ERR_ARG, "null destination");
    hipLaunchKernelGGL(k_halo_pack, dim3((unsigned)((e->npix + 255) / 256)), dim3(256), 0, e->stream, x, (float *)device_dst, (int)e->npix, e->sx, last ? e->nx - 1 : 0);
    LAUNCHCHK();
    return TOMO_OK;
}

int tomo_halo_pack_both(tomo_engine *e, int field, void *first_plane, void *last_plane)
{
    NEED(e);
    float *x; int rc; if ((rc = field_ptr(e, field, &x))) return rc;
    if (!first_plane || !last_plane) return fail(TOMO_ERR_ARG, "null destination");
    hipLaunchKernelGGL(k_halo_wrap, dim3((unsigned)((e->npix + 255) / 256)), dim3(256), 0, e->stream, x, (float *)last_plane, (float *)first_plane, (int)e->npix, e->sx, e->nx);
    LAUNCHCHK();
    return TOMO_OK;
}

int tomo_halo_local(tomo_engine *e, int field)
{
    NEED(e);
    float *x; int rc; if ((rc = field_ptr(e, field, &x))) return rc;
    hipLaunchKernelGGL(k_halo_wrap, dim3((unsigned)((e->npix + 255) / 256)), dim3(256), 0, e->stream, x, e->halo_lo, e->halo_hi, (int)e->npix, e->sx, e->nx);
    LAUNCHCHK();
    return TOMO_OK;
}


int tomo_wait_for(tomo_engine *e, tomo_engine *other)
{
    NEED(e);
    if (!other) return fail(TOMO_ERR_ARG, "null engine");
    if (other->device != e->device) return fail(TOMO_ERR_ARG, "engines on different devices");
    if (other == e || other->stream == e->stream) return TOMO_OK;
    if (!other->ev_peer) HIPCHK(hipEventCreateWithFlags(&other->ev_peer, hipEventDisableTiming));
    HIPCHK(hipEventRecord(other->ev_peer, other->stream));
    HIPCHK(hipStreamWaitEvent(e->stream, other->ev_peer, 0));
    return TOMO_OK;
}

int tomo_halo_from(tomo_engine *e, int field, tomo_engine *lo_src, tomo_engine *hi_src)
{
    NEED(e);
    if (!lo_src || !hi_src) return fail(TOMO_ERR_ARG, "null engine");
    if (lo_src->n != e->n || hi_src->n != e->n || lo_src->device != e->device || hi_src->device != e->device) return fail(TOMO_ERR_ARG, "engines differ in image size or device");
    float *xl, *xh; int rc;
    if ((rc = field_ptr(lo_src, field, &xl)) || (rc = field_ptr(hi_src, field, &xh))) return rc;
    dim3 grid((unsigned)((e->npix + 255) / 256));
    hipLaunchKernelGGL(k_halo_pack, grid, dim3(256), 0, e->stream, xl, e->halo_lo, (int)e->npix, lo_src->sx, lo_src->nx - 1);
    hipLaunchKernelGGL(k_halo_pack, grid, dim3(256), 0, e->stream, xh, e->halo_hi, (int)e->npix, hi_src->sx, 0);
    LAUNCHCHK();
    return TOMO_OK;
}

int tomo_scalar_sum_from(tomo_engine *e, int dst_slot, tomo_engine **srcs, int n, int src_slot)
{
    NEED(e);
    if (!srcs || n < 1 || n > 8 || dst_slot < 0 || dst_slot >= TOMO_S_COUNT || src_slot < 0 || src_slot >= TOMO_S_COUNT) return fail(TOMO_ERR_ARG, "bad argument");
    SumSrc s{};
    s.n = n;
    for (int i = 0; i < n; ++i) { if (!srcs[i] || srcs[i]->device != e->device) return fail(TOMO_ERR_ARG, "bad source engine"); s.p[i] = srcs[i]->d_scal + src_slot; }
    hipLaunchKernelGGL(k_sum_doubles, dim3(1), dim3(1), 0, e->stream, s, e->d_scal + dst_slot);
    LAUNCHCHK();
    return TOMO_OK;
}

int tomo_set_slab_edges(tomo_engine *e, int is_first, int is_last)
{
    if (!e) return fail(TOMO_ERR_ARG, "null engine");
    e->is_first = is_first ? 1 : 0; e->is_last = is_last ? 1 : 0;
    return TOMO_OK;
}

static int tv_grid(tomo_engine *e)
{
    int64_t items = e->npix * (e->sx / 64);
    return (int)std::min<int64_t>((items + 3) / 4, 256 * 16);
}

int tomo_tv_partial(tomo_engine *e, int vol, float eps)
{
    NEED(e);
    float *x; int rc; if ((rc = get_vol_ro(e, vol, &x))) return rc;
    Halo h{e->halo_lo, e->halo_hi};
    if (e->tv_lds != 8 && e->tv_lds != 1) {
        if ((rc = reduce_begin(e))) return rc;
        hipLaunchKernelGGL(k_tv_value, dim3(tv_grid(e)), dim3(256), 0, e->stream, x, h, e->d_part, eps, e->n, e->nx, e->sx);
        LAUNCHCHK();
        return reduce_end(e, TOMO_S_TV);
    }
    if (!e->d_part_tv) { if ((rc = dev_alloc((void **)&e->d_part_tv, NPART * sizeof(double), true, e->stream))) return rc; }
    if ((rc = part_begin(e, e->d_part_tv))) return rc;
    const int yseg = 32;
    if (e->tv_lds == 1 && e->tv_march4 && e->nx % 64 == 0 && e->n % 8 == 0) {
        hipLaunchKernelGGL((k_tv_march4<8, true, TVM_VALUE, false>), dim3(tv_march_grid(e->n, 8, e->sxc / 64, (e->n + yseg - 1) / yseg)), dim3(256), 0, e->stream, x, h, (double *)nullptr, eps, e->n, e->nx, e->sx, yseg, e->d_part_tv, TvUpd{});
    } else if (e->tv_lds == 1) {
        hipLaunchKernelGGL((k_tv_grad_reg<8, true, false>), dim3(tv_march_grid(e->n, 8, e->sxc / 64, (e->n + yseg - 1) / yseg)), dim3(256), 0, e->stream, x, h, (float *)nullptr, (double *)nullptr, eps, e->n, e->nx, e->sx, yseg, e->d_part_tv, TvUpd{});
    } else {
        dim3 grid((unsigned)(((e->n + 7) / 8) * (e->sxc / 64)), (unsigned)((e->n + yseg - 1) / yseg));
        hipLaunchKernelGGL((k_tv_grad_lds<8, true, false>), grid, dim3(256), 0, e->stream, x, h, (float *)nullptr, (double *)nullptr, eps, e->n, e->nx, e->sx, yseg, e->d_part_tv);
    }
    LAUNCHCHK();
    return part_end(e, e->d_part_tv, TOMO_S_TV);
}

static int tv_rows_per_wave(const tomo_engine *e, int tz)
{
    if (e->tv_yseg > 0) return e->tv_yseg;
    const int64_t cols = (int64_t)((e->n + tz - 1) / tz) * (e->sxc / 64);
    int yseg = 32;
    while (yseg > TV_YSEG_MIN && cols * ((e->n + yseg - 1) / yseg) < TV_WAVES_WANTED) yseg >>= 1;
    return yseg;
}

static int tv_grad_impl(tomo_engine *e, float eps, bool with_tv, float *g_first = nullptr, float *g_last = nullptr)
{
    NEED(e);
    float *x, *g; int rc;
    if ((rc = get_vol(e, e->tv_target, &x))) return rc;
    if ((rc = get_scratch(e, &e->tvg, &g))) return rc;
    if ((rc = reduce_begin(e))) return rc;
    Halo h{e->halo_lo, e->halo_hi};
    if ((g_first || g_last) && !(e->tv_lds == 1 && e->tv_recompute)) return fail(TOMO_ERR_STATE, "gradient planes need the recompute form of the TV march (tv_lds = 1, tv_recompute = 1)");
    if (with_tv && e->tv_lds != 8 && e->tv_lds != 1) with_tv = false;
    if (with_tv) {
        if (!e->d_part_tv) { if ((rc = dev_alloc((void **)&e->d_part_tv, NPART * sizeof(double), true, e->stream))) return rc; }
        if ((rc = part_begin(e, e->d_part_tv))) return rc;
    }
    {
        ProfScope ps(e, TOMO_K_TV_GRAD);
        e->tv_last_eps = eps;
        if (e->tv_lds == 1 && e->tv_recompute) {
            TvUpd gp{};
            gp.wrap_lo = g_last; gp.wrap_hi = g_first;
            const int yseg = tv_rows_per_wave(e, e->tv_tz == 4 ? 4 : 8);
            if (e->tv_tz == 4) {
                dim3 grid(tv_march_grid(e->n, 4, e->sxc / 64, (e->n + yseg - 1) / yseg));
                if (with_tv) hipLaunchKernelGGL((k_tv_grad_reg<4, true, true, TVM_NORM>), grid, dim3(256), 0, e->stream, x, h, (float *)nullptr, e->d_part, eps, e->n, e->nx, e->sx, yseg, e->d_part_tv, gp);
                else hipLaunchKernelGGL((k_tv_grad_reg<4, false, true, TVM_NORM>), grid, dim3(256), 0, e->stream, x, h, (float *)nullptr, e->d_part, eps, e->n, e->nx, e->sx, yseg, (double *)nullptr, gp);
            } else {
            dim3 grid(tv_march_grid(e->n, 8, e->sxc / 64, (e->n + yseg - 1) / yseg));
            if (e->tv_march4) {
                const bool edge = e->nx % 64 != 0 || e->n % 8 != 0;
#define TV4_NORM(WTV, EDGE, PTV) hipLaunchKernelGGL((k_tv_march4<8, WTV, TVM_NORM, EDGE>), grid, dim3(256), 0, e->stream, x, h, e->d_part, eps, e->n, e->nx, e->sx, yseg, PTV, gp)
                if (with_tv) { if (edge) TV4_NORM(true, true, e->d_part_tv); else TV4_NORM(true, false, e->d_part_tv); }
                else { if (edge) TV4_NORM(false, true, (double *)nullptr); else TV4_NORM(false, false, (double *)nullptr); }
#undef TV4_NORM
            }
            else if (with_tv) hipLaunchKernelGGL((k_tv_grad_reg<8, true, true, TVM_NORM>), grid, dim3(256), 0, e->stream, x, h, (float *)nullptr, e->d_part, eps, e->n, e->nx, e->sx, yseg, e->d_part_tv, gp);
            else hipLaunchKernelGGL((k_tv_grad_reg<8, false, true, TVM_NORM>), grid, dim3(256), 0, e->stream, x, h, (float *)nullptr, e->d_part, eps, e->n, e->nx, e->sx, yseg, (double *)nullptr, gp);
            }
        } else if (e->tv_lds == 1) {
            int yseg = 32;
            dim3 grid(tv_march_grid(e->n, 8, e->sxc / 64, (e->n + yseg - 1) / yseg));
            if (with_tv) hipLaunchKernelGGL((k_tv_grad_reg<8, true>), grid, dim3(256), 0, e->stream, x, h, g, e->d_part, eps, e->n, e->nx, e->sx, yseg, e->d_part_tv, TvUpd{});
            else hipLaunchKernelGGL((k_tv_grad_reg<8, false>), grid, dim3(256), 0, e->stream, x, h, g, e->d_part, eps, e->n, e->nx, e->sx, yseg, (double *)nullptr, TvUpd{});
        } else if (e->tv_lds) {
            int yseg = 32;
            if (e->tv_lds == 16) {
                dim3 grid((unsigned)(((e->n + 15) / 16) * (e->sxc / 64)), (unsigned)((e->n + yseg - 1) / yseg));
                hipLaunchKernelGGL((k_tv_grad_lds<16, false>), grid, dim3(256), 0, e->stream, x, h, g, e->d_part, eps, e->n, e->nx, e->sx, yseg, (double *)nullptr);
            } else {
                dim3 grid((unsigned)(((e->n + 7) / 8) * (e->sxc / 64)), (unsigned)((e->n + yseg - 1) / yseg));
                if (with_tv) hipLaunchKernelGGL((k_tv_grad_lds<8, true>), grid, dim3(256), 0, e->stream, x, h, g, e->d_part, eps, e->n, e->nx, e->sx, yseg, e->d_part_tv);
                else hipLaunchKernelGGL((k_tv_grad_lds<8, false>), grid, dim3(256), 0, e->stream, x, h, g, e->d_part, eps, e->n, e->nx, e->sx, yseg, (double *)nullptr);
            }
        } else {
            hipLaunchKernelGGL(k_tv_grad, dim3(tv_grid(e)), dim3(256), 0, e->stream, x, h, g, e->d_part, eps, e->n, e->nx, e->sx);
        }
    }
    LAUNCHCHK();
    if (with_tv && (rc = part_end(e, e->d_part_tv, TOMO_S_TV))) return rc;
    return reduce_end(e, TOMO_S_GNORM);
}

int tomo_tv_set_target(tomo_engine *e, int vol)
{
// ... 13 lines not shown
        return rc ? rc : tv_grad_impl(e, eps, false);
    }
    return tv_grad_impl(e, eps, true);
}

int tomo_tv_grad_planes(tomo_engine *e, float eps, int with_tv, void *g_first, void *g_last)
{
    if (!g_first || !g_last) return fail(TOMO_ERR_ARG, "null plane buffer");
    return tv_grad_impl(e, eps, with_tv != 0, (float *)g_first, (float *)g_last);
}

int tomo_tv_halo_apply(tomo_engine *e, float dPOCS, int clamp, const void *g_lo, const void *g_hi)
{
    NEED(e);
    if (!g_lo || !g_hi) return fail(TOMO_ERR_ARG, "null plane buffer");
    hipLaunchKernelGGL(k_halo_apply, dim3((unsigned)((e->npix + 255) / 256)), dim3(256), 0, e->stream, e->halo_lo, e->halo_hi,
                       (const float *)g_lo, (const float *)g_hi, gnorm_ptr(e), dPOCS, clamp, (int)e->npix);
    LAUNCHCHK();
    return TOMO_OK;
}

static int tv_update_impl(tomo_engine *e, float dPOCS, int clamp, int track_vol, int slot, bool wrap = false,
                          float *plane_last = nullptr, float *plane_first = nullptr, const float *hg_lo = nullptr, const float *hg_hi = nullptr)
{
    NEED(e);
    float *x, *g, *track = nullptr; int rc;
    if ((rc = get_vol(e, e->tv_target, &x))) return rc;
    if ((rc = get_scratch(e, &e->tvg, &g))) return rc;
    if (track_vol >= 0) {
        if (track_vol == e->tv_target) return fail(TOMO_ERR_ARG, "the tracked volume must differ from the one descended");
        if (slot < 0 || slot >= TOMO_S_COUNT) return fail(TOMO_ERR_ARG, "bad scalar slot");
        if ((rc = get_vol(e, track_vol, &track))) return rc;
        if ((rc = order_after_async(e))) return rc;
        if ((rc = reduce_begin(e))) return rc;
    }
    if (e->tv_lds == 1 && e->tv_recompute) {
        float *alt;
        if ((rc = get_scratch(e, &e->tv_alt, &alt))) return rc;
        const bool own_halo = e->halo_lo == e->halo_lo_own || e->halo_lo == e->halo_lo_alt;
        float *wl = plane_last, *wh = plane_first;
        if (wrap && own_halo) {
            if (!e->halo_lo_alt) {
                if ((rc = dev_alloc((void **)&e->halo_lo_alt, e->npix * sizeof(float), true, e->stream))) return rc;
                if ((rc = dev_alloc((void **)&e->halo_hi_alt, e->npix * sizeof(float), true, e->stream))) return rc;
            }
            wl = e->halo_lo == e->halo_lo_own ? e->halo_lo_alt : e->halo_lo_own;
            wh = e->halo_hi == e->halo_hi_own ? e->halo_hi_alt : e->halo_hi_own;
        }
        Halo h{e->halo_lo, e->halo_hi};
        TvUpd up{alt, gnorm_ptr(e), dPOCS, clamp, track, wl, wh, slab_streams(e) ? 1 : 0, nullptr, nullptr, nullptr, nullptr};
        const bool fold = hg_lo && hg_hi && (e->tv_halo_fold < 0 ? e->sxc >= 128 : e->tv_halo_fold != 0) && own_halo && !wrap && e->tv_tz != 4 && e->tv_march4;
        if (fold) {
            if (!e->halo_lo_alt) {
                if ((rc = dev_alloc((void **)&e->halo_lo_alt, e->npix * sizeof(float), true, e->stream))) return rc;
                if ((rc = dev_alloc((void **)&e->halo_hi_alt, e->npix * sizeof(float), true, e->stream))) return rc;
            }
            up.hg_lo = hg_lo; up.hg_hi = hg_hi;
            up.ho_lo = e->halo_lo == e->halo_lo_own ? e->halo_lo_alt : e->halo_lo_own;
            up.ho_hi = e->halo_hi == e->halo_hi_own ? e->halo_hi_alt : e->halo_hi_own;
        }
        {
            ProfScope ps(e, TOMO_K_TV_UPDATE);
            const int yseg = tv_rows_per_wave(e, e->tv_tz == 4 ? 4 : 8);
            if (e->tv_tz == 4) {
                dim3 grid(tv_march_grid(e->n, 4, e->sxc / 64, (e->n + yseg - 1) / yseg));
                hipLaunchKernelGGL((k_tv_grad_reg<4, false, true, TVM_UPDATE>), grid, dim3(256), 0, e->stream, x, h, (float *)nullptr, e->d_part, e->tv_last_eps, e->n, e->nx, e->sx, yseg, (double *)nullptr, up);
            } else {
            dim3 grid(tv_march_grid(e->n, 8, e->sxc / 64, (e->n + yseg - 1) / yseg));
            if (e->tv_march4) {
                const bool edge = e->nx % 64 != 0 || e->n % 8 != 0, trk = track != nullptr, strm = up.stream != 0;
#define TV4_UPD(EDGE, TRK, STRM) hipLaunchKernelGGL((k_tv_march4<8, false, TVM_UPDATE, EDGE, TRK, STRM>), grid, dim3(256), 0, e->stream, x, h, e->d_part, e->tv_last_eps, e->n, e->nx, e->sx, yseg, (double *)nullptr, up)
                if (edge) { if (trk) { if (strm) TV4_UPD(true, true, true); else TV4_UPD(true, true, false); } else { if (strm) TV4_UPD(true, false, true); else TV4_UPD(true, false, false); } }
                else { if (trk) { if (strm) TV4_UPD(false, true, true); else TV4_UPD(false, true, false); } else { if (strm) TV4_UPD(false, false, true); else TV4_UPD(false, false, false); } }
#undef TV4_UPD
            }
            else hipLaunchKernelGGL((k_tv_grad_reg<8, false, true, TVM_UPDATE>), grid, dim3(256), 0, e->stream, x, h, (float *)nullptr, e->d_part, e->tv_last_eps, e->n, e->nx, e->sx, yseg, (double *)nullptr, up);
            }
        }
        LAUNCHCHK();
        e->vol[e->tv_target] = alt; e->tv_alt = x;
        if (wrap && own_halo) { e->halo_lo = wl; e->halo_hi = wh; }
        else if (wrap) { if ((rc = tomo_halo_local(e, e->tv_target))) return rc; }
        if (fold) { e->halo_lo = up.ho_lo; e->halo_hi = up.ho_hi; }
        else if (hg_lo && hg_hi && (rc = tomo_tv_halo_apply(e, dPOCS, clamp, hg_lo, hg_hi))) return rc;
        return track ? reduce_end(e, slot) : TOMO_OK;
    }
    int64_t n4 = e->vol_elems() / 4;
    {
        ProfScope ps(e, TOMO_K_TV_UPDATE);
        float *wl = wrap ? e->halo_lo : plane_last, *wh = wrap ? e->halo_hi : plane_first;
        if (track) hipLaunchKernelGGL(k_tv_update<true>, dim3(grid_1d(n4)), dim3(256), 0, e->stream, (f4 *)x, (const f4 *)g, gnorm_ptr(e), dPOCS, clamp, n4, (f4 *)track, e->d_part, wl, wh, e->nx, e->sx / 4);
        else hipLaunchKernelGGL(k_tv_update<false>, dim3(grid_1d(n4)), dim3(256), 0, e->stream, (f4 *)x, (const f4 *)g, gnorm_ptr(e), dPOCS, clamp, n4, (f4 *)nullptr, (double *)nullptr, wl, wh, e->nx, e->sx / 4);
    }
    LAUNCHCHK();
    if (hg_lo && hg_hi && (rc = tomo_tv_halo_apply(e, dPOCS, clamp, hg_lo, hg_hi))) return rc;
    return track ? reduce_end(e, slot) : TOMO_OK;
}

int tomo_tv_update(tomo_engine *e, float dPOCS, int clamp) { return tv_update_impl(e, dPOCS, clamp, -1, 0); }

int tomo_tv_update_planes(tomo_engine *e, float dPOCS, int clamp, void *first_plane, void *last_plane)
{
    if (!first_plane || !last_plane) return fail(TOMO_ERR_ARG, "null plane buffer");
    return tv_update_impl(e, dPOCS, clamp, -1, 0, false, (float *)last_plane, (float *)first_plane);
}

int tomo_tv_update_tracked(tomo_engine *e, float dPOCS, int clamp, int track_vol, int slot)
{
    return tv_update_impl(e, dPOCS, clamp, track_vol, slot);
}

int tomo_fgp_begin(tomo_engine *e) { return tomo_fgp_begin_vol(e, TOMO_VOL_RECON); }

// ... 30 lines not shown
{
    NEED(e);
    if (!e->tvg || !e->fgp_p[2]) return fail(TOMO_ERR_STATE, "tomo_fgp_begin has not been called");
    float multip = 1.0f / (26.0f * lambda);
    ProfScope ps(e, TOMO_K_FGP_GRAD);
    hipLaunchKernelGGL(k_fgp_grad, dim3(tv_grid(e)), dim3(256), 0, e->stream, e->tvg, e->fgp_p[0], e->fgp_p[1], e->fgp_p[2], e->halo_hi, e->is_last, multip, e->n, e->nx, e->sx);
    LAUNCHCHK();
    return TOMO_OK;
}

int tomo_fgp_end(tomo_engine *e, int iters)
{
    if (e && e->fgp_target >= 0 && e->fgp_target < TOMO_VOL_SLOTS) ++e->vol_version[e->fgp_target];

    NEED(e);
    if (!e->tvg) return fail(TOMO_ERR_STATE, "tomo_fgp_begin has not been called");
    (void)iters;
    HIPCHK(hipMemcpyAsync(e->vol[e->fgp_target], e->tvg, e->vol_elems() * sizeof(float), hipMemcpyDeviceToDevice, e->stream));
    return TOMO_OK;
}

int tomo_tv(tomo_engine *e, int vol, float eps)
{
    int rc;
    if ((rc = tomo_halo_local(e, vol))) return rc;
    return tomo_tv_partial(e, vol, eps);
}

static int tv_gd_impl(tomo_engine *e, int ng, float dPOCS, float eps, int track_vol, int slot)
{
    int rc;
    if (!e) return fail(TOMO_ERR_ARG, "null engine");
    const bool fold_tv = ng > 0 && (e->tv_lds == 8 || e->tv_lds == 1);
    if (fold_tv) { if ((rc = tomo_halo_local(e, e->tv_target))) return rc; }
    else if ((rc = tomo_tv(e, e->tv_target, eps))) return rc;
    for (int g = 0; g < ng; ++g) {
        if ((rc = tv_grad_impl(e, eps, fold_tv && g == 0))) return rc;
        if ((rc = tv_update_impl(e, dPOCS, g == ng - 1, g == ng - 1 ? track_vol : -1, slot, g < ng - 1))) return rc;
    }
    if (ng <= 0) {
        if ((rc = tomo_positivity(e, e->tv_target))) return rc;
        if (track_vol >= 0) {
            if ((rc = tomo_diff_norm_sq(e, e->tv_target, track_vol, slot))) return rc;
            return tomo_copy_volume(e, track_vol, e->tv_target);
        }
    }
    return TOMO_OK;
}

int tomo_tv_gd(tomo_engine *e, int ng, float dPOCS, float eps) { return tv_gd_impl(e, ng, dPOCS, eps, -1, 0); }

int tomo_tv_gd_tracked(tomo_engine *e, int ng, float dPOCS, float eps, int track_vol, int slot)
{
    if (track_vol < 0) return fail(TOMO_ERR_ARG, "bad tracked volume");
    return tv_gd_impl(e, ng, dPOCS, eps, track_vol, slot);
}

int tomo_tv_fgp(tomo_engine *e, int iters, float lambda) { return tomo_tv_fgp_vol(e, TOMO_VOL_RECON, iters, lambda); }

int tomo_bind_fgp_halo(tomo_engine *e, void *lo, void *hi, void *send_first, void *send_last)
{
    NEED(e);
    if (!lo || !hi || !send_first || !send_last) return fail(TOMO_ERR_ARG, "null plane buffer");
    HIPCHK(hipStreamSynchronize(e->stream));
    e->fgp_lo = (float *)lo; e->fgp_hi = (float *)hi; e->fgp_send_first = (float *)send_first; e->fgp_send_last = (float *)send_last;
    e->fgp_planes2 = false;
    return TOMO_OK;
}
// ... 64 lines not shown
    const float multip = 1.0f / (26.0f * lambda);
    {
        ProfScope ps(e, TOMO_K_FGP_GRAD);
        if (fgp_sharded(e)) {
            Fgp2Edge ed{e->fgp_lo, e->fgp_hi, e->fgp_send_first, e->fgp_send_last, e->is_first, e->is_last};
            hipLaunchKernelGGL((k_fgp_fused2<false, true>), grid, dim3(256), 0, e->stream, e->vol[e->fgp_target], e->fgp_p[0], e->fgp_p[1], e->fgp_p[2],
                               e->fgp_q[0], e->fgp_q[1], e->fgp_q[2], lambda, multip, e->n, e->nx, e->sx, yseg, first_iteration ? 1 : 0, ed);
        } else
        hipLaunchKernelGGL((k_fgp_fused2<false, false>), grid, dim3(256), 0, e->stream, e->vol[e->fgp_target], e->fgp_p[0], e->fgp_p[1], e->fgp_p[2],
                           e->fgp_q[0], e->fgp_q[1], e->fgp_q[2], lambda, multip, e->n, e->nx, e->sx, yseg, first_iteration ? 1 : 0, Fgp2Edge{});
    }
    LAUNCHCHK();
    for (int k = 0; k < 3; ++k) std::swap(e->fgp_p[k], e->fgp_q[k]);
    return TOMO_OK;
}

int tomo_fgp_fused_last(tomo_engine *e, float lambda, int first_iteration)
{
    NEED(e);
    if (!e->fgp_q[2] || !e->fgp_p[2]) return fail(TOMO_ERR_STATE, "tomo_fgp_fused_begin has not been called");
    if (fgp_sharded(e)) return fail(TOMO_ERR_STATE, "tomo_fgp_fused_last is for a slab that is the whole volume");
    if (e->fgp_target < 0 || e->fgp_target >= TOMO_VOL_SLOTS) return fail(TOMO_ERR_STATE, "no target volume");
    const int yseg = 32;
    const int nzb = (e->n + F2_TZ - 1) / F2_TZ, nys = (e->n + yseg - 1) / yseg, nchunk = (e->nx + F2_SC - 1) / F2_SC;
    dim3 grid((nzb & 7) == 0 ? 8u * (unsigned)((nzb >> 3) * nchunk * nys) : (unsigned)(nzb * nchunk * nys));
    const float multip = 1.0f / (26.0f * lambda);
    {
        ProfScope ps(e, TOMO_K_FGP_OBJ);
        hipLaunchKernelGGL((k_fgp_fused2<true, false>), grid, dim3(256), 0, e->stream, e->vol[e->fgp_target], e->fgp_p[0], e->fgp_p[1], e->fgp_p[2],
                           e->fgp_q[0], e->fgp_q[1], e->fgp_q[2], lambda, multip, e->n, e->nx, e->sx, yseg, first_iteration ? 1 : 0, Fgp2Edge{});
    }
    LAUNCHCHK();
    std::swap(e->vol[e->fgp_target], e->fgp_q[0]);
    ++e->vol_version[e->fgp_target];
    return TOMO_OK;
}

int tomo_fgp_fused_end(tomo_engine *e, float lambda)
{
    if (e && e->fgp_target >= 0 && e->fgp_target < TOMO_VOL_SLOTS) ++e->vol_version[e->fgp_target];

    NEED(e);
    if (!e->fgp_p[2]) return fail(TOMO_ERR_STATE, "tomo_fgp_fused_begin has not been called");
    ProfScope ps(e, TOMO_K_FGP_OBJ);
    float *a = e->vol[e->fgp_target];
    hipLaunchKernelGGL(k_fgp_obj, dim3(tv_grid(e)), dim3(256), 0, e->stream, a, a, e->fgp_p[0], e->fgp_p[1], e->fgp_p[2],
                       fgp_sharded(e) ? e->fgp_lo : e->halo_lo, e->is_first, lambda, e->n, e->nx, e->sx);
    LAUNCHCHK();
    return TOMO_OK;
}

int tomo_tv_fgp_vol(tomo_engine *e, int vol, int iters, float lambda)
{
    int rc;
    if ((rc = tomo_tv(e, vol, 1e-6f))) return rc;
    const bool fused = e && e->fgp_fused && iters > 1;
    int f = e->is_first, l = e->is_last;
    e->is_first = e->is_last = 1;
    if (fused) {
        rc = tomo_fgp_fused_begin(e, vol);
        int i = 0;
        if (e->fgp_pair) for (; i + 2 < iters && !rc; i += 2) rc = tomo_fgp_fused_step2(e, lambda, i == 0);
        if (e->fgp_pair && i + 2 == iters) {
            if (!rc) rc = tomo_fgp_fused_last(e, lambda, i == 0);
        } else {
            for (; i + 1 < iters && !rc; ++i) rc = tomo_fgp_fused_step(e, lambda, i == 0);
// ... 14 lines not shown
```

tomo_tv_amd/csrc/kernels_common.hip.h:

```cpp
#pragma once

namespace tomo {


template <int V> struct VecOf;
template <> struct VecOf<1> { typedef float T; };
template <> struct VecOf<2> { typedef float T __attribute__((ext_vector_type(2))); };
template <> struct VecOf<4> { typedef float T __attribute__((ext_vector_type(4))); };

template <int V> __device__ __forceinline__ typename VecOf<V>::T vzero();
template <> __device__ __forceinline__ float vzero<1>() { return 0.f; }
template <> __device__ __forceinline__ VecOf<2>::T vzero<2>() { VecOf<2>::T v = {0.f, 0.f}; return v; }
template <> __device__ __forceinline__ VecOf<4>::T vzero<4>() { VecOf<4>::T v = {0.f, 0.f, 0.f, 0.f}; return v; }

template <int V> __device__ __forceinline__ float velem(const typename VecOf<V>::T &v, int i);
template <> __device__ __forceinline__ float velem<1>(const float &v, int) { return v; }
template <> __device__ __forceinline__ float velem<2>(const VecOf<2>::T &v, int i) { return v[i]; }
template <> __device__ __forceinline__ float velem<4>(const VecOf<4>::T &v, int i) { return v[i]; }

template <int V> __device__ __forceinline__ void vset(typename VecOf<V>::T &v, int i, float f);
template <> __device__ __forceinline__ void vset<1>(float &v, int, float f) { v = f; }
template <> __device__ __forceinline__ void vset<2>(VecOf<2>::T &v, int i, float f) { v[i] = f; }
template <> __device__ __forceinline__ void vset<4>(VecOf<4>::T &v, int i, float f) { v[i] = f; }

// ... 22 lines not shown
#ifndef TOMO_NT_OFF
#define TOMO_NT_OFF 0
#endif
constexpr int NT_DEFAULT = 32 | 256;
template <int BIT, typename T>
__device__ __forceinline__ T nt_ld(const T *p)
{
    if constexpr (((TOMO_NT | NT_DEFAULT) & ~TOMO_NT_OFF & BIT) != 0) return __builtin_nontemporal_load(p);
    else return *p;
}
template <int BIT, typename T>
__device__ __forceinline__ void nt_st(T v, T *p)
{
    if constexpr (((TOMO_NT | NT_DEFAULT) & ~TOMO_NT_OFF & BIT) != 0) {
        __builtin_nontemporal_store(v, p);
    } else *p = v;
}

__global__ void k_finalize(double *__restrict__ part, double *__restrict__ dst)
{
    double v = part[threadIdx.x];
    part[threadIdx.x] = 0.0;
    __shared__ double red[NPART / 64];
    v = wave_sum(v);
    if ((threadIdx.x & 63) == 0) red[threadIdx.x >> 6] = v;
    __syncthreads();
    if (threadIdx.x == 0) {
        double s = 0;
        for (int i = 0; i < NPART / 64; ++i) s += red[i];
        *dst = s;
    }
}

__global__ __launch_bounds__(256) void k_transpose_in(const float *__restrict__ src, float *__restrict__ dst,
                                                       int ns, int64_t m, int sx)
{
    __shared__ float tile[32][33];
    int64_t m0 = (int64_t)blockIdx.x * 32;
    int s0 = blockIdx.y * 32;
    int tx = threadIdx.x & 31, ty = threadIdx.x >> 5;
    for (int r = ty; r < 32; r += 8) {
        int s = s0 + r;
        int64_t mm = m0 + tx;
        tile[r][tx] = (s < ns && mm < m) ? src[(int64_t)s * m + mm] : 0.f;
    }
    __syncthreads();
    for (int r = ty; r < 32; r += 8) {
        int64_t mm = m0 + r;
        int s = s0 + tx;
        if (mm < m && s < sx) dst[mm * sx + s] = tile[tx][r];
    }
}

__global__ __launch_bounds__(256) void k_transpose_out(const float *__restrict__ src, float *__restrict__ dst,
                                                        int ns, int64_t m, int sx)
{
    __shared__ float tile[32][33];
    int64_t m0 = (int64_t)blockIdx.x * 32;
    int s0 = blockIdx.y * 32;
    int tx = threadIdx.x & 31, ty = threadIdx.x >> 5;
    for (int r = ty; r < 32; r += 8) {
        int64_t mm = m0 + r;
        int s = s0 + tx;
        tile[r][tx] = (mm < m && s < sx) ? src[mm * sx + s] : 0.f;
    }
    __syncthreads();
// ... 25 lines not shown
```

tomo_tv_amd/csrc/kernels_fp.hip.h:

```cpp
#pragma once

namespace tomo {

constexpr int RAY_GROUP = 16;

__device__ __forceinline__ void ray_block_map(int bid, int nb, int nrows, int &chunk, int &rowidx)
{
    if ((nrows % (8 * RAY_GROUP)) == 0 && (nb & 7) == 0) {
        int xcd = bid & 7, l = bid >> 3;
        int per = nrows >> 3;
        chunk = l / per;
        int li = l - chunk * per;
        int g = li / RAY_GROUP, w = li - g * RAY_GROUP;
        rowidx = (g * 8 + xcd) * RAY_GROUP + w;
    } else {
        chunk = bid / nrows;
        rowidx = bid - chunk * nrows;
    }
}

enum { FP_STORE = 0, FP_RESID = 1, FP_RESID_NORM = 2, FP_DD = 3, FP_POISSON = 4, FP_RESID_MUL = 5 };

template <int VEC, int MODE>
__global__ __launch_bounds__(256) void k_fp_rows(const float *__restrict__ x, const uint32_t *__restrict__ rptr,
// ... 329 lines not shown
            FS_NEXT                                                                                       \
            const uint32_t off = e.x & 0x7FFFFFFFu, wb = e.y;                                             \
            V xv[FT_BATCH];                                                                               \
            FS_LD1(0) FS_LD1(1) FS_LD1(2) FS_LD1(3)                                                       \
            if (FULL) { FS_LD1(4) FS_LD1(5) FS_LD1(6) FS_LD1(7) }                                         \
            FS_FM1(0) FS_FM1(1) FS_FM1(2) FS_FM1(3)                                                       \
            if (FULL) { FS_FM1(4) FS_FM1(5) FS_FM1(6) FS_FM1(7) }                                         \
            if (e.x >> 31) {    \
                nt_st<32>(acc[k], reinterpret_cast<V *>(pp));                                             \
                acc[k] = vzero<4>();                                                                      \
                pp += pstep;                                                                              \
            }                                                                                             \
        }
#pragma unroll
        for (int k = 0; k < K; ++k) {
            const uint32_t word = k < 4 ? c4.x : k < 8 ? c4.y : k < 12 ? c4.z : c4.w;
            const uint32_t h = __builtin_amdgcn_readfirstlane((word >> (8 * (k & 3))) & 0xFFu);
            for (uint32_t b = h >> 1; b > 0; --b) FS_UNIT(true)
            if (h & 1) FS_UNIT(false)
        }
#undef FS_UNIT
#undef FS_NEXT
#undef FS_FM1
#undef FS_LD1
    }
    asm volatile("s_waitcnt vmcnt(0) lgkmcnt(0)" : "+v"(en) : : "memory");
#undef FS_DMA
}

template <int LPR, int MODE>
__global__ __launch_bounds__(256) void k_fp_tile_reduce(const float *__restrict__ part, const uint32_t *__restrict__ rsptr,
                                                         const uint32_t *__restrict__ rsidx, const float *__restrict__ b,
                                                         const float *__restrict__ rowsum, float *__restrict__ out,
                                                         double *__restrict__ dpart, int nrows, int sx, int chunk0, int ncp)
{
    typedef VecOf<4>::T V;
    constexpr int R = 64 / LPR, U = 8;
    const int lane = threadIdx.x & 63, wave = threadIdx.x >> 6;
    const int grp = lane / LPR, gl = lane - grp * LPR;
    const int spans = ncp * 16 / LPR;
    int64_t item = ((int64_t)blockIdx.x * 4 + wave) * R + grp;
    int row = (int)(item / spans), span = (int)(item - (int64_t)row * spans);
    bool valid = row < nrows;
    if (!__any(valid)) return;
    if (!valid) row = 0;
    uint32_t kb = rsptr[row], ke = valid ? rsptr[row + 1] : kb;
    const float *pp = part + (size_t)span * (LPR * 4) + gl * 4;
    V acc = vzero<4>();
    uint32_t sidx[U], sn[U];
#pragma unroll
    for (int u = 0; u < U; ++u) sidx[u] = (kb + u < ke) ? rsidx[kb + u] : 0xFFFFFFFFu;
    for (uint32_t k = kb; __any(k < ke); k += U) {
        V pv[U];
#pragma unroll
        for (int u = 0; u < U; ++u) pv[u] = (sidx[u] != 0xFFFFFFFFu) ? nt_ld<32>(reinterpret_cast<const V *>(pp + (size_t)sidx[u] * ncp * 64)) : vzero<4>();
#pragma unroll
        for (int u = 0; u < U; ++u) sn[u] = (k + U + u < ke) ? rsidx[k + U + u] : 0xFFFFFFFFu;
#pragma unroll
        for (int u = 0; u < U; ++u) acc += pv[u];
#pragma unroll
        for (int u = 0; u < U; ++u) sidx[u] = sn[u];
    }
    double local = 0.0;
    if (valid) {
        size_t o = (size_t)row * sx + (size_t)chunk0 * 64 + (size_t)span * (LPR * 4) + gl * 4;
        if (MODE == FP_STORE) {
            *reinterpret_cast<V *>(out + o) = acc;
        } else {
            V bv = *reinterpret_cast<const V *>(b + o);
            V r;
            if (MODE == FP_RESID) {
                r = bv - acc;
            } else if (MODE == FP_RESID_NORM) {
                float rs = rowsum[row];
                r = rs > 0.f ? (bv - acc) / rs : vzero<4>();
            } else if (MODE == FP_RESID_MUL) {
                r = (bv - acc) * rowsum[row];
            } else if (MODE == FP_DD) {
                r = acc;
#pragma unroll
                for (int i = 0; i < 4; ++i) { float d = acc[i] - bv[i]; local += (double)(d * d); }
            } else {
                const float eps = 1e-1f;
#pragma unroll
                for (int i = 0; i < 4; ++i) {
                    float a = acc[i], bb = bv[i];
                    r[i] = (a - bb) / (a + eps);
                    local += (double)(a - bb * logf(a + eps));
                }
            }
            *reinterpret_cast<V *>(out + o) = r;
        }
    }
    if (MODE == FP_DD || MODE == FP_POISSON) {
        local = wave_sum(local);
        if (lane == 0) atomicAdd(&dpart[blockIdx.x & (NPART - 1)], local);
    }
}

template <int MODE>
__global__ __launch_bounds__(256) void k_sino_resid(const float *__restrict__ b, const float *__restrict__ g,
                                                     const float *__restrict__ rowsum, float *__restrict__ out, int64_t n4, int sx4)
{
    typedef VecOf<4>::T V;
    for (int64_t i = (int64_t)blockIdx.x * 256 + threadIdx.x; i < n4; i += (int64_t)gridDim.x * 256) {
        V bv = reinterpret_cast<const V *>(b)[i], acc = reinterpret_cast<const V *>(g)[i], r;
        if (MODE == FP_RESID) {
            r = bv - acc;
        } else {
            float rs = rowsum[i / sx4];
            r = rs > 0.f ? (bv - acc) / rs : vzero<4>();
        }
        reinterpret_cast<V *>(out)[i] = r;
    }
}

__global__ __launch_bounds__(256) void k_sino_extrapolate(const VecOf<4>::T *__restrict__ g, VecOf<4>::T *__restrict__ p,
                                                          VecOf<4>::T *__restrict__ q, float beta, int64_t n4)
{
    for (int64_t i = (int64_t)blockIdx.x * 256 + threadIdx.x; i < n4; i += (int64_t)gridDim.x * 256) {
        VecOf<4>::T a = g[i], b = p[i];
        q[i] = a + beta * (a - b);
        p[i] = a;
    }
}

constexpr int FL_W = 16, FL_TH = 8, FL_PIX = FL_W * FL_TH, FL_THREADS = 1024, FL_WAVES = FL_THREADS / 64, FL_BATCH = 16, FL_PIXB = 512;
constexpr int FL_TILE_BYTES = 2 * FL_PIX * FL_PIXB, FL_MAXSTEPS = 64 * FL_TH, FL_LDS_BYTES = FL_TILE_BYTES + FL_MAXSTEPS * 4;
struct FlItemD { int pass, v0; uint32_t tile0, ntiles, lp0, work, pad0, pad1; };
// ... 169 lines not shown
```

tomo_tv_amd/csrc/kernels_tv.hip.h:

```cpp
#pragma once

namespace tomo {

struct Halo { const float *lo; const float *hi; };

__device__ __forceinline__ float ldx(const float *__restrict__ x, const Halo &h, int pix, int s, int nx, int sx)
{
    if (s < 0) return h.lo[pix];
    if (s >= nx) return h.hi[pix];
    return x[(size_t)pix * sx + s];
}

__global__ void k_halo_pack(const float *__restrict__ x, float *__restrict__ dst, int npix, int sx, int s)
{
    int i = blockIdx.x * blockDim.x + threadIdx.x;
    if (i < npix) dst[i] = x[(size_t)i * sx + s];
}

__global__ void k_scalars_to_host(const double *__restrict__ src, double *__restrict__ host_dst, int n)
{
    int i = threadIdx.x;
    if (i < n) host_dst[i] = src[i];
}

// ... 426 lines not shown
                            if (up.stream) __builtin_nontemporal_store(v, tr + (unsigned)s);
                            else tr[(unsigned)s] = v;
                        }
                    }
                }
            }
#pragma unroll
            for (int j = 0; j < TZ + 2; ++j) { cm[j] = c0[j]; c0[j] = cp[j]; cp[j] = cn[j]; E0[j] = Ep[j]; Ep[j] = En[j]; }
            PE0 = PEp; PEp = PEn; PC0 = PCp;
#pragma unroll
            for (int j = 1; j <= TZ; ++j) Rm[j] = R0[j];
        }
#undef TVR_RINV
    }
    if (GRAD) block_accumulate(acc, part);
    if (WITH_TV) {
        __syncthreads();
        block_accumulate(tvacc, part_tv);
    }
}

#ifndef TV4_PACKED
#define TV4_PACKED 1
#endif
#ifndef TV4_PACKED_EDGE
#define TV4_PACKED_EDGE 0
#endif
#ifndef TV4_UPD_WAVES
#define TV4_UPD_WAVES 4
#endif
#define TV4_OCC __attribute__((amdgpu_waves_per_eu((MODE == TVM_UPDATE && !TRACK) ? TV4_UPD_WAVES : 4, (MODE == TVM_UPDATE && !TRACK) ? TV4_UPD_WAVES : 8)))
template <int TZ, bool WITH_TV, int MODE, bool EDGE, bool TRACK = false, bool STREAM = false>
__global__ __launch_bounds__(256) TV4_OCC void k_tv_march4(const float *__restrict__ x, Halo h, double *__restrict__ part, float eps,
                                                    int n, int nx, int sx, int yseg, double *__restrict__ part_tv, TvUpd up)
{
    static_assert(MODE == TVM_NORM || MODE == TVM_UPDATE || MODE == TVM_VALUE, "modes without a stored gradient");
    static_assert(MODE != TVM_VALUE || WITH_TV, "the value mode sums the TV integrand");
    const int lane = threadIdx.x & 63, wave = __builtin_amdgcn_readfirstlane(threadIdx.x >> 6);
    const int nzb = (n + TZ - 1) / TZ, nchunk = (nx + 63) >> 6   , nys = (n + yseg - 1) / yseg;
    double acc = 0.0, tvacc = 0.0;
    float nrm_ = 1.f;
    if (MODE == TVM_UPDATE) nrm_ = tv_step_len(up.dPOCS, up.gnorm2);
    int bs, bz, ys;
    if ((nzb & 7) == 0) {
        const int zpx = nzb >> 3;
        const int64_t li = (int64_t)(blockIdx.x >> 3) * 4 + wave;
        bs = (int)(li % nchunk); bz = (int)(blockIdx.x & 7) * zpx + (int)((li / nchunk) % zpx); ys = (int)(li / ((int64_t)nchunk * zpx));
    } else {
        const int64_t item = (int64_t)blockIdx.x * 4 + wave;
        bs = (int)(item % nchunk); bz = (int)((item / nchunk) % nzb); ys = (int)(item / ((int64_t)nchunk * nzb));
    }
    if (ys < nys) {
        const int y0 = ys * yseg, y1 = min(y0 + yseg, n);
        const int z0 = bz * TZ, s0 = bs * 64, s = s0 + lane;
        int zc[TZ + 2];
#pragma unroll
        for (int j = 0; j < TZ + 2; ++j) { int z = (z0 - 1 + j) % n; zc[j] = z < 0 ? z + n : z; }
        int zl;
        { int z = (z0 - 1 + (lane < TZ + 2 ? lane : 0)) % n; zl = z < 0 ? z + n : z; }
        auto yrow = [&](int y) { int r = y % n; return r < 0 ? r + n : r; };
        float rows[4][TZ + 2], Ta[TZ + 1], Tb[TZ + 1];
        float pe[4], pf[4], pc[4];
        const bool lo_in = s0 > 0, hi_in = s0 + 64 < nx;
        const unsigned zls = (unsigned)zl * (unsigned)sx;
        const unsigned off_lo = lo_in ? zls + (unsigned)(s0 - 1) : (unsigned)zl, off_hi = hi_in ? zls + (unsigned)(s0 + 64) : (unsigned)zl;
        constexpr bool SOFF = !EDGE && !(WITH_TV && MODE == TVM_NORM);
        unsigned vb[TZ + 2];
// ... 191 lines not shown
                    if (s == 0) {
#pragma unroll
                        for (int j = 1; j <= TZ; ++j)
                            if (z0 + j - 1 < n) up.ho_lo[pix0 + (j - 1)] = fmaxf(tv_step(h.lo[pix0 + (j - 1)], up.hg_lo[pix0 + (j - 1)], nrm_), vmin);
                    }
                    if (s == nx - 1) {
#pragma unroll
                        for (int j = 1; j <= TZ; ++j)
                            if (z0 + j - 1 < n) up.ho_hi[pix0 + (j - 1)] = fmaxf(tv_step(h.hi[pix0 + (j - 1)], up.hg_hi[pix0 + (j - 1)], nrm_), vmin);
                    }
                }
            }
        };
        fetch(y0 - 1, rows[0], pe[0], pf[0], pc[0]);
        fetch(y0, rows[1], pe[1], pf[1], pc[1]);
        fetch(y0 + 1, rows[2], pe[2], pf[2], pc[2]);
#pragma unroll
        for (int j = 1; MODE != TVM_VALUE && j <= TZ; ++j) {
            float xi = shl(col(pf[0], j), rows[0][j]), r, dd, d1, d2, d3;
            TV4_RINV(rows[0][j], xi, rows[1][j], rows[0][j + 1], r, dd, d1, d2, d3)
            (void)dd; (void)d1; (void)d3;
            Ta[j] = nc_mul(d2, r);
        }
#define TV4_ROW(S0, SP, SN, TP, TN) row(y, rows[S0], rows[SP], rows[SN], pe[S0], pf[S0], pc[S0], pe[SP], pe[SN], pf[SN], pc[SN], TP, TN)
        for (int y = y0; y < y1;) {
            TV4_ROW(1, 2, 3, Ta, Tb); if (++y >= y1) break;
            TV4_ROW(2, 3, 0, Tb, Ta); if (++y >= y1) break;
            TV4_ROW(3, 0, 1, Ta, Tb); if (++y >= y1) break;
            TV4_ROW(0, 1, 2, Tb, Ta); ++y;
        }
#undef TV4_ROW
#undef TV4_RINV
    }
    if (MODE != TVM_VALUE) block_accumulate(acc, part);
    if (WITH_TV) {
        __syncthreads();
        block_accumulate(tvacc, part_tv);
    }
}

__global__ __launch_bounds__(256) void k_halo_apply(float *__restrict__ halo_lo, float *__restrict__ halo_hi,
                                                     const float *__restrict__ g_lo, const float *__restrict__ g_hi,
                                                     const double *__restrict__ gnorm2, float dPOCS, int clamp, int npix)
{
    const float len = tv_step_len(dPOCS, gnorm2);
    int p = blockIdx.x * 256 + threadIdx.x;
    if (p >= npix) return;
    float a = tv_step(halo_lo[p], g_lo[p], len);
    float b = tv_step(halo_hi[p], g_hi[p], len);
    if (clamp) { a = fmaxf(a, 0.f); b = fmaxf(b, 0.f); }
    halo_lo[p] = a;
    halo_hi[p] = b;
}

template <bool TRACK>
__global__ __launch_bounds__(256) void k_tv_update(f4 *__restrict__ x, const f4 *__restrict__ g,
                                                    const double *__restrict__ gnorm2, float dPOCS, int clamp,
                                                    int64_t n4, f4 *__restrict__ track, double *__restrict__ part,
                                                    float *__restrict__ wrap_lo, float *__restrict__ wrap_hi, int nx, int sx4)
{
    const float len = tv_step_len(dPOCS, gnorm2);
    double acc = 0.0;
    for (int64_t i = (int64_t)blockIdx.x * 256 + threadIdx.x; i < n4; i += (int64_t)gridDim.x * 256) {
        f4 xv = x[i], gv = g[i], v;
        v.x = tv_step(xv.x, gv.x, len); v.y = tv_step(xv.y, gv.y, len); v.z = tv_step(xv.z, gv.z, len); v.w = tv_step(xv.w, gv.w, len);
        if (clamp) { v.x = fmaxf(v.x, 0.f); v.y = fmaxf(v.y, 0.f); v.z = fmaxf(v.z, 0.f); v.w = fmaxf(v.w, 0.f); }
        x[i] = v;
        if (wrap_lo) {
            int64_t pix = i / sx4;
            int s = (int)(i - pix * sx4) * 4;
// ... 15 lines not shown
```

tomo_tv_amd/csrc/sart_resident.hip.h:

```cpp
#pragma once

namespace tomo {

typedef float v16f __attribute__((ext_vector_type(16)));
typedef unsigned long long rs_u64;
typedef uint32_t rs_u2 __attribute__((ext_vector_type(2)));
constexpr int RS_T = 32, RS_WAVES = 16, RS_THREADS = RS_WAVES * 64, RS_MAXWIN = 48, RS_RL = 32, RS_USABLE = 14;
struct RsHdrD { uint16_t jbase, nrays; uint32_t dw[4]; uint32_t pad[3]; };
static_assert(sizeof(RsHdrD) == 32, "header layout (resident.h)");
struct RsArgs {
    float *x;
    const float *b, *rowsum;
    const RsHdrD *hdr;
    const uint4 *cell;
    const uint2 *ts;
    const uint16_t *rl;
    rs_u64 *pb, *rb;
    const int *angs;
    float *track;
    double *part;
    int *abort_word, *abort_host;
    unsigned *commit;
    int *done_host;
    unsigned seq, commit_base;
    int test_fail;
    int n, sx, np, ntiles, tiles, rpt, steps, chunk0, nchunk;
    unsigned epoch0, spin_limit;
    float beta;
    long long *prof;
};
#ifdef RS_PROF
#define RS_STAMP(q) { const long long now_ = (long long)__builtin_amdgcn_s_memrealtime(); if (wave == 0) tacc[q] += now_ - tprev; tprev = now_; }
#define RS_TL(q) { if (k == 40 && blockIdx.x == 37 && lane == 0) rs_args()->prof[2048 + wave * 8 + (q)] = (long long)__builtin_amdgcn_s_memrealtime(); }
#else
#define RS_STAMP(q)
#define RS_TL(q)
#endif

__device__ __forceinline__ rs_u64 rs_gld(const rs_u64 *p)
{
    return __hip_atomic_load((const __attribute__((address_space(1))) rs_u64 *)p, __ATOMIC_RELAXED, __HIP_MEMORY_SCOPE_AGENT);
}
__device__ __forceinline__ void rs_gst(rs_u64 *p, float v, unsigned ep)
{
    __hip_atomic_store((__attribute__((address_space(1))) rs_u64 *)p, ((rs_u64)ep << 32) | (rs_u64)__float_as_uint(v), __ATOMIC_RELAXED, __HIP_MEMORY_SCOPE_AGENT);
}
__device__ __forceinline__ int rs_abort_ld(const int *p)
{
    return __hip_atomic_load((const __attribute__((address_space(1))) int *)p, __ATOMIC_RELAXED, __HIP_MEMORY_SCOPE_AGENT);
}
__device__ __forceinline__ bool rs_give_up(unsigned &spins, unsigned spin_limit, int *abort_word, int *abort_host, int lane, int code)
{
    if (((++spins) & 31u) != 0u && spin_limit != 0u) return false;
    if (spins > spin_limit) {
        if (lane == 0) {
            __hip_atomic_store((__attribute__((address_space(1))) int *)abort_word, code, __ATOMIC_RELAXED, __HIP_MEMORY_SCOPE_AGENT);
            if (abort_host) __hip_atomic_store((__attribute__((address_space(1))) int *)abort_host, code, __ATOMIC_RELAXED, __HIP_MEMORY_SCOPE_SYSTEM);
        }
        return true;
    }
    return rs_abort_ld(abort_word) != 0;
}
// ... 74 lines not shown
    "s_add_u32 s38, s38, %[rs]\n" "s_addc_u32 s39, s39, 0\n"                                              \
    "s_add_u32 s40, s40, %[rs]\n" "s_addc_u32 s41, s41, 0\n"

#define RS_K __attribute__((address_space(4)))
typedef const RS_K RsArgs *RsArgsP;
__device__ __forceinline__ RsArgsP rs_args()
{
    RsArgsP p = (RsArgsP)__builtin_amdgcn_kernarg_segment_ptr();
    asm volatile("" : "+s"(p) :: "memory");
    return p;
}

__device__ __forceinline__ int rs_angle(RsArgsP A, int k)
{
    return ((const RS_K int *)A->angs)[k];
}

__device__ __forceinline__ void rs_touch(RsArgsP A, int tile, int wave, int lane, int an, float *dump)
{
    if (lane < 8 && an >= 0) {
        const uint32_t *tp = reinterpret_cast<const uint32_t *>(A->cell + (((size_t)an * A->ntiles + tile) * RS_WAVES + wave) * 64) + lane * 32;
        __builtin_amdgcn_global_load_lds((const __attribute__((address_space(1))) void *)tp, (__attribute__((address_space(3))) void *)dump, 4, 0, 0);
    }
}

__global__ __launch_bounds__(RS_THREADS) __attribute__((amdgpu_waves_per_eu(4, 4)))
void k_sart_resident(const RsArgs unused_by_name)
{
    __shared__ float rs_pbuf[RS_WAVES][16][64];
    __shared__ float rs_rbuf[RS_MAXWIN][64];
    __shared__ float rs_sbuf[RS_WAVES][64];
    __shared__ float rs_dump[RS_WAVES][64];
    __shared__ int rs_dirty, rs_go, rs_store;
    const int lane = threadIdx.x & 63;
    const int wave = __builtin_amdgcn_readfirstlane(threadIdx.x >> 6);
    v32f xlo, xhi;
    v16f rr;
#ifdef RS_PROF
    long long tacc[8] = {0, 0, 0, 0, 0, 0, 0, 0}, tprev = (long long)__builtin_amdgcn_s_memrealtime();
    const long long clk0 = (long long)__builtin_amdgcn_s_memtime(), rt0 = tprev;
#endif
    int tile, grp, ngrp, chunk, chunk_end, steps;
    {
        RsArgsP A = rs_args();
        tile = (int)blockIdx.x % A->ntiles; grp = (int)blockIdx.x / A->ntiles; ngrp = (int)gridDim.x / A->ntiles;
        chunk = A->chunk0 + grp; chunk_end = A->chunk0 + A->nchunk; steps = A->steps;
    }
    for (int it = 0; chunk < chunk_end; chunk += ngrp, ++it) {
        const uint32_t voff = (uint32_t)(chunk * 64 + lane) * 4u;
        {
            if (threadIdx.x == 0) { rs_dirty = 0; rs_go = rs_abort_ld(rs_args()->abort_word) == 0 ? 1 : 0; }
            __syncthreads();
            if (rs_go == 0) break;
        }
        {
            RsArgsP A = rs_args();
            rs_touch(A, tile, wave, lane, rs_angle(A, 0), rs_dump[wave]);
            if (steps > 1) rs_touch(A, tile, wave, lane, rs_angle(A, 1), rs_dump[wave]);
            const int n = A->n, sx = A->sx;
            const int ty = tile / A->tiles, tz = tile - ty * A->tiles;
            const int y0 = ty * RS_T + (wave >> 2) * 8, z0 = tz * RS_T + (wave & 3) * 8;
            const int in = __builtin_amdgcn_readfirstlane((y0 < n && z0 < n) ? 1 : 0);
            const float *xb = A->x + ((size_t)min(y0, n - 1) * n + min(z0, n - 1)) * sx;
            const uint32_t ps = (uint32_t)sx * 4u, rs = (uint32_t)(n - 8) * ps;
            asm volatile("s_cmp_eq_u32 %[in], 0\n"
                         "s_cbranch_scc1 1f\n"
                         "s_mov_b64 s[36:37], %[xb]\n"
                         RS_XALL(RS_XLD1)
                         "s_waitcnt vmcnt(0)\n"
                         "s_branch 2f\n"
                         "1:\n"
                         RS_XZROW(0) RS_XZROW(1) RS_XZROW(2) RS_XZROW(3) RS_XZROW(4) RS_XZROW(5) RS_XZROW(6) RS_XZROW(7)
                         "2:\n"
                         : "={v[64:95]}"(xlo), "={v[96:127]}"(xhi)
                         : [in] "s"(in), [xb] "s"(xb), [voff] "v"(voff), [ps] "s"(ps), [rs] "s"(rs)
                         : "s36", "s37", "scc", "memory");
        }
        int c_jbase = 0, c_nr = 0, c_dwv = 0;
        for (int k = -1; k < steps; ++k) {
            int f_nr = 0, f_jbase = 0, f_rpt = 1, f_rpt2 = 1, f_wpr = RS_WAVES, f_cpw = RS_RL / RS_WAVES, f_jr0 = 0, f_sub = 0;
            uint32_t f_dwv = 0;
            rs_u2 f_ts0 = {0u, 0u}, f_ts1 = {0u, 0u}, f_ts2 = {0u, 0u};
            rs_u2 f_ids0 = {0xFFFFFFFFu, 0xFFFFFFFFu};
            float f_rs0 = 0.f, f_bv0 = 0.f;
// ... 138 lines not shown
                            acc += __uint_as_float((uint32_t)g0);
                            if (id1 != 0xFFFF) acc += __uint_as_float((uint32_t)g1);
                            if (id2 != 0xFFFF) acc += __uint_as_float((uint32_t)g2);
                            if (id3 != 0xFFFF) acc += __uint_as_float((uint32_t)g3);
                        }
                        rs_sbuf[wave][lane] = acc;
                    }
                    RS_STAMP(5)
                    RS_TL(5)
                    __syncthreads();
                    if (active && sub == 0) {
                        float tot = rs_sbuf[wave][lane];
                        for (int u = 1; u < wpr; ++u) tot += rs_sbuf[wave + u][lane];
                        const size_t row = (size_t)a * n + j;
                        const float bv = r0 == 0 ? bv0 : A->b[row * A->sx + (voff >> 2)], rs = r0 == 0 ? rs0 : ((const RS_K float *)A->rowsum)[row];
                        const float rv = rs > 0.f ? (bv - tot) / rs : 0.f;
                        rs_gst(A->rb + (((size_t)grp * A->np) * n + row) * 64 + lane, rv, ep);
                    }
                    if (r0 + rpt2 < rpt) __syncthreads();
                }
                RS_STAMP(6)
                RS_TL(6)
            }
        }
        {
            __syncthreads();
            if (threadIdx.x == 0) {
                RsArgsP A = rs_args();
                const bool clean = rs_dirty == 0 && rs_abort_ld(A->abort_word) == 0 && !(tile == 0 && A->test_fail == chunk + 1);
                const bool ok = rs_commit(A->commit + chunk, A->commit_base, (unsigned)A->ntiles, clean, A->spin_limit, A->abort_word);
                if (ok && tile == 0)
                    __hip_atomic_store((__attribute__((address_space(1))) int *)(A->done_host + chunk), (int)A->seq, __ATOMIC_RELAXED, __HIP_MEMORY_SCOPE_SYSTEM);
                rs_store = ok ? 1 : 0;
            }
            __syncthreads();
            if (rs_store == 0) continue;
        }
        {
            RsArgsP A = rs_args();
            const int n = A->n, sx = A->sx;
            const int ty = tile / A->tiles, tz = tile - ty * A->tiles;
            const int y0 = ty * RS_T + (wave >> 2) * 8, z0 = tz * RS_T + (wave & 3) * 8;
            const int in = __builtin_amdgcn_readfirstlane((y0 < n && z0 < n) ? 1 : 0);
            const size_t o0 = ((size_t)min(y0, n - 1) * n + min(z0, n - 1)) * sx;
            float *xb = A->x + o0;
            const uint32_t ps = (uint32_t)sx * 4u, rs = (uint32_t)(n - 8) * ps;
            if (A->track) {
                float *tb = A->track + o0;
                double local = 0.0;
                asm volatile("s_cmp_eq_u32 %[in], 0\n"
                             "s_cbranch_scc1 1f\n"
                             "s_mov_b64 s[36:37], %[xb]\n"
                             "s_mov_b64 s[38:39], %[tb]\n"
                             "s_mov_b64 s[40:41], %[tb]\n"
                             RS_TROW(0) RS_TROW(1) RS_TROW(2) RS_TROW(3) RS_TROW(4) RS_TROW(5) RS_TROW(6) RS_TROW(7)
                             "s_waitcnt vmcnt(0)\n"
                             "1:\n"
                             : [sum] "+v"(local)
                             : "{v[64:95]}"(xlo), "{v[96:127]}"(xhi), [in] "s"(in), [xb] "s"(xb), [tb] "s"(tb), [voff] "v"(voff), [ps] "s"(ps), [rs] "s"(rs)
                             : "s36", "s37", "s38", "s39", "s40", "s41", "v48", "v49", "v50", "v51", "v52", "v53", "v54", "v55", "v56", "v58", "v59", "scc", "memory");
                double *red = reinterpret_cast<double *>(&rs_pbuf[wave][0][0]);
                red[lane] = local;
                __builtin_amdgcn_wave_barrier();
                if (lane == 0) {
                    local = 0.0;
                    for (int l = 0; l < 64; ++l) local += red[l];
                    const uint32_t slot = (blockIdx.x & (NPART - 1)) * 8u;
                    double *part = A->part;
                    asm volatile("global_atomic_add_f64 %0, %1, %2" :: "v"(slot), "v"(local), "s"(part) : "memory");
                }
            } else {
                asm volatile("s_cmp_eq_u32 %[in], 0\n"
                             "s_cbranch_scc1 1f\n"
                             "s_mov_b64 s[36:37], %[xb]\n"
                             RS_XALL(RS_XST1)
                             "s_waitcnt vmcnt(0)\n"
                             "1:\n"
                             :
                             : "{v[64:95]}"(xlo), "{v[96:127]}"(xhi), [in] "s"(in), [xb] "s"(xb), [voff] "v"(voff), [ps] "s"(ps), [rs] "s"(rs)
                             : "s36", "s37", "scc", "memory");
            }
        }
    }
#ifdef RS_PROF
    if (threadIdx.x == 0) {
        RsArgsP A = rs_args();
        for (int q = 0; q < 8; ++q) A->prof[blockIdx.x * 8 + q] = tacc[q];
        if (blockIdx.x == 0) { A->prof[2048 + 126] = (long long)__builtin_amdgcn_s_memtime() - clk0; A->prof[2048 + 127] = (long long)__builtin_amdgcn_s_memrealtime() - rt0; }
    }
#endif
}
#undef RS_K
#undef RS_TROW
#undef RS_TST1
#undef RS_TLD1
#undef RS_XST1
#undef RS_XZROW
#undef RS_XZ1
#undef RS_XLD1
#undef RS_XALL
#undef RS_XROW
#undef RS_CLOBBERS
#undef RS_CLOB4
#undef RS_SWEEP
#undef RS_WAIT
#undef RS_BATCH
#undef RS_FP1
#undef RS_IDX
#undef RS_BP1
#undef RS_LD

}
```

tomo_tv_amd/csrc/tomo_engine.hip:

```cpp
#include "../../include/tomo_hip.h"
#include "kernels.hip.h"
#include "sart_resident.hip.h"
#include "sysmat.h"
#include "resident.h"

#include <dlfcn.h>
#if __has_include(<rccl/rccl.h>)
#include <rccl/rccl.h>
#else
#define NCCL_UNIQUE_ID_BYTES 128
typedef struct ncclComm *ncclComm_t;
typedef struct { char internal[NCCL_UNIQUE_ID_BYTES]; } ncclUniqueId;
typedef enum { ncclSuccess = 0 } ncclResult_t;
typedef enum { ncclFloat32 = 7, ncclFloat64 = 8 } ncclDataType_t;
typedef enum { ncclSum = 0 } ncclRedOp_t;
#endif

#include <algorithm>
#include <atomic>
#include <chrono>
#include <cmath>
#include <condition_variable>
#include <functional>
#include <memory>
// ... 181 lines not shown
    int bp_tile = 1;
    int bp_list = 1;
    bool attr_bp2 = false, bl_ok = false;
    int bp_list_band = 0;
    uint4 *d_bl_ent = nullptr;
    uint32_t *d_bl_ptr = nullptr, *d_bl_win = nullptr;
    int bl_tiles_z = 0, bl_ntiles = 0;
    bool fb_ok = false;
    uint4 *d_fb_cell = nullptr;
    uint32_t *d_fb_win = nullptr;
    int ft_ncp = 0, ft_ncp_forced = 0;
    size_t ft_scratch_cap = (size_t)8 << 30;
    float *vol[TOMO_VOL_SLOTS] = {};
    float *sino[TOMO_SINO_SLOTS] = {};
    int fgp_target = TOMO_VOL_RECON;
    int tv_target = TOMO_VOL_RECON;
    float *cur_b = nullptr;
    float *cg_p = nullptr, *cg_z = nullptr, *cg_w = nullptr, *fbp_h = nullptr;
    double *cg_sums = nullptr;
    double *cg_part = nullptr;
    float *cg_coef = nullptr;
    float *tvg = nullptr;
    float *fgp_p[3] = {nullptr, nullptr, nullptr};
    float *fgp_q[3] = {nullptr, nullptr, nullptr};
    int fgp_fused = 1;
    int fgp_pair = 1;
    float *stage = nullptr;
    size_t stage_bytes = 0;
    double *d_scal = nullptr, *d_scal_own = nullptr, *d_part = nullptr, *d_part_aux = nullptr, *d_part_tv = nullptr;
    double *h_snap = nullptr;
    hipEvent_t ev_snap = nullptr;
    bool snap_pending = false;
    bool part_open[3] = {false, false, false};
    hipStream_t aux = nullptr;
    hipEvent_t ev_fork = nullptr, ev_join = nullptr;
    bool async_pending = false;
    struct CommRef *comm = nullptr;
    int64_t comm_rounds = 0;
    float *comm_send_first = nullptr, *comm_send_last = nullptr, *comm_g_lo = nullptr, *comm_g_hi = nullptr;
    float *comm_fgp = nullptr;
    double *comm_scal = nullptr;
    uint64_t vol_version[TOMO_VOL_SLOTS] = {};
    struct { int vol = -1; uint64_t ver = 0; } g_valid[2];
    int fp_reuse = 1;
    float *g_prev = nullptr;
    float *g_yk = nullptr;
    struct { bool valid = false; uint64_t ver = 0; } yk_claim;
    bool g_prev_valid = false, mom_p_ok = false;
    uint64_t g_prev_recon_ver = 0;
    struct { float beta = 0.f; uint64_t ver_recon = 0, ver_yk = 0, ver_old = 0; bool set = false; } mom;
    bool old_is_recon = false;
    bool geometry_released = false;
    float *halo_lo = nullptr, *halo_hi = nullptr, *halo_lo_own = nullptr, *halo_hi_own = nullptr;
    float *fgp_lo = nullptr, *fgp_hi = nullptr, *fgp_send_first = nullptr, *fgp_send_last = nullptr;
    bool fgp_planes2 = false;
    int is_first = 1, is_last = 1;
    ProfSlot prof[PROF_MAX_KERNELS];
    std::mutex prof_mu;
    size_t vol_elems() const { return (size_t)npix * sx; }
    size_t sino_elems() const { return (size_t)nrows * sx; }
};

static inline double *gnorm_ptr(const tomo_engine *e) { return e->gnorm_override ? e->gnorm_override : e->d_scal + e->gnorm_slot; }

static thread_local size_t *g_alloc_meter = nullptr;
static int dev_alloc(void **p, size_t bytes, bool zero, hipStream_t st)
// ... 2 lines not shown
    if (g_alloc_meter) *g_alloc_meter += bytes;
    if (zero) HIPCHK(hipMemsetAsync(*p, 0, bytes ? bytes : 4, st));
    return TOMO_OK;
}

static void g_clear(tomo_engine *e) { e->g_valid[0].vol = e->g_valid[1].vol = -1; }
static void g_set(tomo_engine *e, int vol) { e->g_valid[0].vol = vol; e->g_valid[0].ver = e->vol_version[vol]; e->g_valid[1].vol = -1; }
static bool g_is_projection_of(const tomo_engine *e, int vol)
{
    if (!e->fp_reuse || vol < 0 || vol >= TOMO_VOL_SLOTS || !e->sino[TOMO_SINO_G]) return false;
    for (int k = 0; k < 2; ++k) if (e->g_valid[k].vol == vol && e->g_valid[k].ver == e->vol_version[vol]) return true;
    return false;
}

static const float *projection_in_hand(const tomo_engine *e, int vol)
{
    if (g_is_projection_of(e, vol)) return e->sino[TOMO_SINO_G];
    if (e->fp_reuse && vol == TOMO_VOL_YK && e->g_yk && e->yk_claim.valid && e->yk_claim.ver == e->vol_version[TOMO_VOL_YK]) return e->g_yk;
    return nullptr;
}

static int get_vol_ro(tomo_engine *e, int id, float **out)
{
    if (id < 0 || id >= TOMO_VOL_SLOTS) return fail(TOMO_ERR_ARG, "bad volume id");
    if (id == TOMO_VOL_RECON_OLD && e->old_is_recon) id = TOMO_VOL_RECON;
    if (!e->vol[id]) {
        int rc = dev_alloc((void **)&e->vol[id], e->vol_elems() * sizeof(float), true, e->stream);
        if (rc) return rc;
    }
    *out = e->vol[id];
    return TOMO_OK;
}

static int get_vol(tomo_engine *e, int id, float **out)
{
    if (id < 0 || id >= TOMO_VOL_SLOTS) return fail(TOMO_ERR_ARG, "bad volume id");
    ++e->vol_version[id];
    if (e->old_is_recon && (id == TOMO_VOL_RECON || id == TOMO_VOL_RECON_OLD)) {
        e->old_is_recon = false;
        float *src, *dst; int rc;
        if ((rc = get_vol_ro(e, TOMO_VOL_RECON, &src)) || (rc = get_vol_ro(e, TOMO_VOL_RECON_OLD, &dst))) return rc;
        HIPCHK(hipMemcpyAsync(dst, src, e->vol_elems() * sizeof(float), hipMemcpyDeviceToDevice, e->stream));
    }
    return get_vol_ro(e, id, out);
}

static int get_sino(tomo_engine *e, float **slot, float **out)
{
    if (slot == &e->sino[TOMO_SINO_G]) g_clear(e);
    if (!*slot) {
        int rc = dev_alloc((void **)slot, e->sino_elems() * sizeof(float), true, e->stream);
        if (rc) return rc;
    }
    *out = *slot;
    return TOMO_OK;
}

static int sino_slot(tomo_engine *e, int id, float **out)
{
    if (id < 0 || id >= TOMO_SINO_SLOTS) return fail(TOMO_ERR_ARG, "bad sinogram id");
    return get_sino(e, &e->sino[id], out);
}

static int get_scratch(tomo_engine *e, float **slot, float **out)
{
    if (!*slot) {
        int rc = dev_alloc((void **)slot, e->vol_elems() * sizeof(float), true, e->stream);
        if (rc) return rc;
    }
    *out = *slot;
// ... 17 lines not shown

struct Sub {
    hipStream_t stream; int c0 = 0, nc = 0;
    int vec = 0;
};
static int sub_vec(const tomo_engine *e, const Sub &sb) { return sb.nc && sb.vec ? sb.vec : e->vec; }
static Sub whole(const tomo_engine *e) { return Sub{e->stream, e->sub_c0, e->sub_nc}; }

struct ProfScope {
    tomo_engine *e; int k; hipEvent_t stop = nullptr; hipStream_t st;
    ProfScope(tomo_engine *e_, int k_, hipStream_t st_ = nullptr, int64_t key = -1) : e(e_), k(k_), st(st_ ? st_ : e_->stream)
    {
        ProfSlot &p = e->prof[k];
        if (!p.on) return;
        hipEvent_t start;
        {
            std::lock_guard<std::mutex> lk(e->prof_mu);
            if (p.stride > 1 && ((key >= 0 ? (uint64_t)key : (uint64_t)p.seen++) % p.stride) != 0) return;
            if (p.used + 2 > p.ev.size()) {
                if (p.ev.size() >= PROF_MAX_EVENTS) { ++p.dropped; return; }
                hipEvent_t a, b;
                if (hipEventCreate(&a) != hipSuccess || hipEventCreate(&b) != hipSuccess) { ++p.dropped; return; }
                p.ev.push_back(a); p.ev.push_back(b);
            }
            start = p.ev[p.used];
            stop = p.ev[p.used + 1];
            p.used += 2;
        }
        (void)hipEventRecord(start, st);
    }
    ~ProfScope() { if (stop) (void)hipEventRecord(stop, st); }
};

static bool &part_open(tomo_engine *e, const double *part)
{
    return part == e->d_part_tv ? e->part_open[2] : part == e->d_part_aux ? e->part_open[1] : e->part_open[0];
}
static int part_begin(tomo_engine *e, double *part)
{
    bool &open = part_open(e, part);
    if (open) HIPCHK(hipMemsetAsync(part, 0, NPART * sizeof(double), e->stream));
    open = true;
    return TOMO_OK;
}
static int part_end(tomo_engine *e, double *part, int slot)
{
    hipLaunchKernelGGL(k_finalize, dim3(1), dim3(NPART), 0, e->stream, part, e->d_scal + slot);
    LAUNCHCHK();
    part_open(e, part) = false;
    return TOMO_OK;
}
static int reduce_begin(tomo_engine *e) { return part_begin(e, e->d_part); }
static int reduce_end(tomo_engine *e, int slot) { return part_end(e, e->d_part, slot); }

constexpr int TV_YSEG_MIN = 8, TV_WAVES_WANTED = 4096;
static int grid_1d(int64_t n4) { int64_t b = (n4 + 255) / 256; return (int)std::min<int64_t>(std::max<int64_t>(b, 1), 4096); }

#include "engine_launch.inc"
#include "engine_create.inc"

extern "C" {

#include "engine_api.inc"
#include "engine_tv.inc"
#include "engine_comm.inc"
#include "engine_options.inc"

}
```

Measured before the change: 10.60 Gvoxel-updates/s.

## Finalize reductions inline via tickets and emit halo planes from SART sweep

Reductions no longer need a separate single-block k_finalize launch. Each producing kernel, including the fp reduce, TV march and resident SART kernels, takes a ticket counter, and the last block to finish folds the partials into the scalar slot. The resident SART kernel also writes the first and last x-planes into the halo buffers during its sweep. A version-tracked halo cache then lets the TV step skip the separate k_halo_wrap gather. This removes small kernel launches and one volume pass per iteration. In exchange it adds atomics, a waitcnt after the f64 atomic add, and cache-invalidation bookkeeping that could go stale.

```diff
diff --git a/include/tomo_hip.h b/include/tomo_hip.h
--- a/include/tomo_hip.h
+++ b/include/tomo_hip.h
@@ -105,6 +105,7 @@
 int tomo_halo_pack(tomo_engine *e, int field, int last, void *device_dst);
 int tomo_halo_pack_both(tomo_engine *e, int field, void *first_plane, void *last_plane);
 int tomo_halo_local(tomo_engine *e, int field);
+int tomo_read_halo(tomo_engine *e, float *lo, float *hi);
 enum tomo_field { TOMO_FIELD_FGP_D = 100, TOMO_FIELD_FGP_P1 = 101 };
 int tomo_wait_for(tomo_engine *e, tomo_engine *other);
 int tomo_halo_from(tomo_engine *e, int field, tomo_engine *lo_src, tomo_engine *hi_src);
diff --git a/tomo_tv_amd/_lib.py b/tomo_tv_amd/_lib.py
--- a/tomo_tv_amd/_lib.py
+++ b/tomo_tv_amd/_lib.py
@@ -69,6 +69,7 @@
     "tomo_halo_pack": [_p, _i, _i, _p],
     "tomo_halo_pack_both": [_p, _i, _p, _p],
     "tomo_halo_local": [_p, _i],
+    "tomo_read_halo": [_p, _p, _p],
     "tomo_set_slab_edges": [_p, _i, _i],
     "tomo_wait_for": [_p, _p],
     "tomo_halo_from": [_p, _i, _p, _p],
diff --git a/tomo_tv_amd/csrc/engine_api.inc b/tomo_tv_amd/csrc/engine_api.inc
--- a/tomo_tv_amd/csrc/engine_api.inc
+++ b/tomo_tv_amd/csrc/engine_api.inc
@@ -97,7 +97,7 @@
     if (e->rs_done) (void)hipHostFree(e->rs_done);
     free_geometry(e);
     void *ptrs[] = {e->tv_alt, e->halo_lo_alt, e->halo_hi_alt, e->d_part_tv, e->d_part_aux, e->fgp_q[0], e->fgp_q[1], e->fgp_q[2], e->cg_p, e->cg_z, e->cg_sums, e->cg_part, e->cg_coef, e->sart_alt,
-                    e->tvg, e->fgp_p[0], e->fgp_p[1], e->fgp_p[2], e->stage, e->d_scal_own, e->d_part, e->halo_lo_own, e->halo_hi_own};
+                    e->tvg, e->fgp_p[0], e->fgp_p[1], e->fgp_p[2], e->stage, e->d_scal_own, e->d_part, e->d_tickets, e->halo_lo_own, e->halo_hi_own};
     for (void *p : ptrs) if (p) (void)hipFree(p);
     for (int i = 0; i < TOMO_VOL_SLOTS; ++i) if (e->vol[i]) (void)hipFree(e->vol[i]);
     for (auto &p : e->prof) { for (auto ev : p.ev) (void)hipEventDestroy(ev); if (p.ref) (void)hipEventDestroy(p.ref); }
@@ -137,6 +137,7 @@
     src->old_is_recon = false;
     for (int i = 0; i < TOMO_VOL_SLOTS; ++i) ++dst->vol_version[i];
     g_clear(dst);
+    halo_forget(dst); halo_forget(src);
     return TOMO_OK;
 }
 
@@ -225,6 +226,7 @@
     { int rc_ = order_after_async(e); if (rc_) return rc_; }
     float *dst; int rc = get_vol(e, vol, &dst); if (rc) return rc;
     if (!data) return fail(TOMO_ERR_ARG, "null volume");
+    halo_forget(e);
     return upload(e, data, dst, e->npix);
 }
 
@@ -271,6 +273,7 @@
     if (e->vol[TOMO_VOL_YK]) HIPCHK(hipMemsetAsync(e->vol[TOMO_VOL_YK], 0, e->vol_elems() * sizeof(float), e->stream));
     if (e->vol[TOMO_VOL_RECON_OLD]) HIPCHK(hipMemsetAsync(e->vol[TOMO_VOL_RECON_OLD], 0, e->vol_elems() * sizeof(float), e->stream));
     e->old_is_recon = false;
+    halo_forget(e);
     ++e->vol_version[TOMO_VOL_RECON]; ++e->vol_version[TOMO_VOL_YK]; ++e->vol_version[TOMO_VOL_RECON_OLD];
     return TOMO_OK;
 }
@@ -362,8 +365,9 @@
 static hipEvent_t g_rs_last[64] = {};
 
 static int launch_sart_resident(tomo_engine *e, float *x, float beta, int64_t steps, const std::function<int(int64_t)> &angle_at, float *track,
-                                std::vector<std::pair<int, int>> &failed)
-{
+                                std::vector<std::pair<int, int>> &failed, bool &wrote_planes)
+{
+    wrote_planes = false;
     failed.clear();
     if (steps > (int64_t)1 << 24) return fail(TOMO_ERR_ARG, "too many SART steps in one call");
     const int c0 = e->sub_nc ? e->sub_c0 : 0, nc = e->sub_nc ? e->sub_nc : e->sxc / 64;
@@ -400,6 +404,14 @@
     A.commit = e->d_rs_commit; A.done_host = e->rs_done; A.seq = e->rs_seq; A.commit_base = e->rs_commit_base; A.test_fail = e->rs_test_fail;
     A.n = e->n; A.sx = e->sx; A.np = e->np; A.ntiles = e->rs_ntiles; A.tiles = e->rs_tiles; A.rpt = e->rs_rpt; A.steps = (int)steps; A.chunk0 = c0; A.nchunk = nc;
     A.epoch0 = e->rs_epoch; A.spin_limit = e->rs_spin_limit; A.beta = beta; A.prof = nullptr;
+    const unsigned grid = (unsigned)(e->rs_ntiles * groups);
+    const PartFin fin = track ? part_fin(e, e->d_part, grid) : PartFin{};
+    A.fin_dst = fin.dst; A.fin_ticket = fin.ticket;
+    const bool planes = e->halo_from_sweep && (e->halo_lo == e->halo_lo_own || (e->halo_lo_alt && e->halo_lo == e->halo_lo_alt))
+                        && (e->halo_hi == e->halo_hi_own || (e->halo_hi_alt && e->halo_hi == e->halo_hi_alt))
+                        && e->is_first && e->is_last && !e->sub_nc && !e->comm && e->gnorm_slot == TOMO_S_GNORM;
+    A.halo_lo = planes ? e->halo_lo : nullptr; A.halo_hi = planes ? e->halo_hi : nullptr; A.nx = e->nx;
+    wrote_planes = false;
     e->rs_epoch += (uint32_t)need;
     if (e->device < 0 || e->device >= 64) return fail(TOMO_ERR_ARG, "device index");
     {
@@ -409,7 +421,7 @@
         else HIPCHK(hipStreamWaitEvent(e->stream, last, 0));
         {
             ProfScope ps(e, TOMO_K_SART_RESIDENT);
-            hipLaunchKernelGGL(k_sart_resident, dim3((unsigned)(e->rs_ntiles * groups)), dim3(RS_THREADS), 0, e->stream, A);
+            hipLaunchKernelGGL(k_sart_resident, dim3(grid), dim3(RS_THREADS), 0, e->stream, A);
             LAUNCHCHK();
         }
         HIPCHK(hipEventRecord(last, e->stream));
@@ -422,7 +434,9 @@
         if (!failed.empty() && failed.back().first + failed.back().second == c) ++failed.back().second;
         else failed.emplace_back(c, 1);
     }
+    wrote_planes = planes && nfailed == 0;
     if (nfailed) {
+        if (fin.dst) part_fin_revoke(e, e->d_part);
         e->rs_commit_dirty = true;
         e->rs_last_code = *e->rs_abort;
         *e->rs_abort = 0;
@@ -456,7 +470,7 @@
             if ((rc = tomo_diff_norm_sq(e, vol, track_vol, slot))) return rc;
             return tomo_copy_volume(e, track_vol, vol);
         }
-        if ((rc = reduce_begin(e))) return rc;
+        if ((rc = reduce_begin(e, slot))) return rc;
     }
     auto finish = [&]() -> int { return track ? reduce_end(e, slot) : TOMO_OK; };
     if (order) {
@@ -526,8 +540,10 @@
     };
     if (form == TOMO_FORM_SART_RESIDENT) {
         std::vector<std::pair<int, int>> failed;
-        if ((rc = launch_sart_resident(e, x, beta, steps, angle_at, track, failed))) return rc;
+        bool wrote_planes = false;
+        if ((rc = launch_sart_resident(e, x, beta, steps, angle_at, track, failed, wrote_planes))) return rc;
         if (!failed.empty() && (rc = sweep_tiles(&failed))) return rc;
+        if (wrote_planes) { e->halo_cur.vol = vol; e->halo_cur.ver = e->vol_version[vol]; e->halo_cur.lo = e->halo_lo; e->halo_cur.hi = e->halo_hi; }
         return finish();
     }
     if (e->sart_resident == 1 && !e->rs_ok) return fail(TOMO_ERR_STATE, "\"sart_resident\" = 1, but this engine has no tables of the resident sweep (N not a multiple of 8, more 32 x 32 tiles than CUs, or a matrix whose ray windows do not fit)");
@@ -552,7 +568,7 @@
     }
     int last = angle_at(steps - 1);
     if ((rc = launch_bp_angle(e, cur, last, r + (size_t)last * e->n * e->sx, beta, track))) return rc;
-    if (cur != x) { e->vol[vol] = cur; e->sart_alt = x; }
+    if (cur != x) { e->vol[vol] = cur; e->sart_alt = x; halo_forget(e); }
     return finish();
 }
 
@@ -656,7 +672,7 @@
     NEED(e);
     float *x, *b, *r; int rc;
     if ((rc = get_vol(e, vol, &x)) || (rc = sino_slot(e, sino_b, &b)) || (rc = sino_slot(e, sino_out, &r))) return rc;
-    if ((rc = reduce_begin(e))) return rc;
+    if ((rc = reduce_begin(e, TOMO_S_COST))) return rc;
     if ((rc = launch_fp_all<FP_POISSON>(e, x, b, r))) return rc;
     return reduce_end(e, TOMO_S_COST);
 }
@@ -886,6 +902,7 @@
     hipLaunchKernelGGL(k_momentum, dim3(grid_1d(n4)), dim3(256), 0, e->stream, (const f4 *)yk, (const f4 *)old, (f4 *)x, beta, n4);
     LAUNCHCHK();
     ++e->vol_version[TOMO_VOL_RECON]; ++e->vol_version[TOMO_VOL_YK]; ++e->vol_version[TOMO_VOL_RECON_OLD];
+    halo_forget(e);
     e->vol[TOMO_VOL_RECON] = yk;
     e->vol[TOMO_VOL_YK] = x;
     e->old_is_recon = true;
@@ -930,7 +947,7 @@
     NEED(e);
     float *x, *g; int rc;
     if ((rc = get_vol_ro(e, vol, &x)) || (rc = get_sino(e, &e->sino[TOMO_SINO_G], &g))) return rc;
-    if ((rc = reduce_begin(e))) return rc;
+    if ((rc = reduce_begin(e, TOMO_S_DD))) return rc;
     if ((rc = launch_fp_all<FP_DD>(e, x, e->sino[TOMO_SINO_B], g))) return rc;
     g_set(e, vol);
     return reduce_end(e, TOMO_S_DD);
diff --git a/tomo_tv_amd/csrc/engine_create.inc b/tomo_tv_amd/csrc/engine_create.inc
--- a/tomo_tv_amd/csrc/engine_create.inc
+++ b/tomo_tv_amd/csrc/engine_create.inc
@@ -276,6 +276,7 @@
     g_alloc_meter = nullptr;
     if ((rc = dev_alloc((void **)&e->d_scal_own, TOMO_S_COUNT * sizeof(double), true, e->stream))) return rc;
     if ((rc = dev_alloc((void **)&e->d_part, NPART * sizeof(double), true, e->stream))) return rc;
+    if ((rc = dev_alloc((void **)&e->d_tickets, 3 * NTICKET * sizeof(unsigned), true, e->stream))) return rc;
     e->d_scal = e->d_scal_own;
     if ((rc = dev_alloc((void **)&e->halo_lo_own, e->npix * sizeof(float), true, e->stream))) return rc;
     if ((rc = dev_alloc((void **)&e->halo_hi_own, e->npix * sizeof(float), true, e->stream))) return rc;
diff --git a/tomo_tv_amd/csrc/engine_launch.inc b/tomo_tv_amd/csrc/engine_launch.inc
--- a/tomo_tv_amd/csrc/engine_launch.inc
+++ b/tomo_tv_amd/csrc/engine_launch.inc
@@ -26,16 +26,17 @@
 
 template <int MODE>
 static void launch_fp_reduce(tomo_engine *e, hipStream_t rs, const float *part, const uint32_t *rsptr, const uint32_t *rsidx, const float *b,
-                             float *out, int c0, int ncp)
+                             float *out, int c0, int ncp, bool last_pass)
 {
     int lpr = (ncp % 4 == 0) ? 64 : (ncp % 2 == 0) ? 32 : 16;
     int64_t items = (int64_t)e->nrows * (ncp * 16 / lpr);
     int64_t waves = (items + 64 / lpr - 1) / (64 / lpr);
     dim3 grid((unsigned)((waves + 3) / 4)), block(256);
+    const PartFin fin = ((MODE == FP_DD || MODE == FP_POISSON) && last_pass) ? part_fin(e, e->d_part, grid.x * 4u) : PartFin{};
     switch (lpr) {
-    case 64: hipLaunchKernelGGL((k_fp_tile_reduce<64, MODE>), grid, block, 0, rs, part, rsptr, rsidx, b, e->d_rowsum, out, e->d_part, (int)e->nrows, e->sx, c0, ncp); break;
-    case 32: hipLaunchKernelGGL((k_fp_tile_reduce<32, MODE>), grid, block, 0, rs, part, rsptr, rsidx, b, e->d_rowsum, out, e->d_part, (int)e->nrows, e->sx, c0, ncp); break;
-    default: hipLaunchKernelGGL((k_fp_tile_reduce<16, MODE>), grid, block, 0, rs, part, rsptr, rsidx, b, e->d_rowsum, out, e->d_part, (int)e->nrows, e->sx, c0, ncp); break;
+    case 64: hipLaunchKernelGGL((k_fp_tile_reduce<64, MODE>), grid, block, 0, rs, part, rsptr, rsidx, b, e->d_rowsum, out, e->d_part, (int)e->nrows, e->sx, c0, ncp, fin); break;
+    case 32: hipLaunchKernelGGL((k_fp_tile_reduce<32, MODE>), grid, block, 0, rs, part, rsptr, rsidx, b, e->d_rowsum, out, e->d_part, (int)e->nrows, e->sx, c0, ncp, fin); break;
+    default: hipLaunchKernelGGL((k_fp_tile_reduce<16, MODE>), grid, block, 0, rs, part, rsptr, rsidx, b, e->d_rowsum, out, e->d_part, (int)e->nrows, e->sx, c0, ncp, fin); break;
     }
 }
 
@@ -69,7 +70,7 @@
         }
         {
             ProfScope ps(e, TOMO_K_FP_REDUCE);
-            launch_fp_reduce<MODE>(e, e->stream, *slot, e->d_fs_rsptr, e->d_fs_rsidx, b, out, c0, ncp);
+            launch_fp_reduce<MODE>(e, e->stream, *slot, e->d_fs_rsptr, e->d_fs_rsidx, b, out, c0, ncp, c0 + ncp >= nchunk);
             LAUNCHCHK();
         }
     }
@@ -108,7 +109,7 @@
         }
         {
             ProfScope ps(e, TOMO_K_FP_REDUCE);
-            launch_fp_reduce<MODE>(e, e->stream, *slot, e->d_fl_rsptr, e->d_fl_rsidx, b, out, c0, ncp);
+            launch_fp_reduce<MODE>(e, e->stream, *slot, e->d_fl_rsptr, e->d_fl_rsidx, b, out, c0, ncp, c0 + ncp >= nchunk);
             LAUNCHCHK();
         }
     }
@@ -191,7 +192,7 @@
         }
         {
             ProfScope ps(e, TOMO_K_FP_REDUCE, rs);
-            launch_fp_reduce<MODE>(e, rs, part, e->d_ft_rsptr, e->d_ft_rsidx, b, out, c0, ncp);
+            launch_fp_reduce<MODE>(e, rs, part, e->d_ft_rsptr, e->d_ft_rsidx, b, out, c0, ncp, c0 + ncp >= nchunk);
             LAUNCHCHK();
         }
         if (pipe) HIPCHK(hipEventRecord(e->ev_fp_red[which][half], rs));
diff --git a/tomo_tv_amd/csrc/engine_options.inc b/tomo_tv_amd/csrc/engine_options.inc
--- a/tomo_tv_amd/csrc/engine_options.inc
+++ b/tomo_tv_amd/csrc/engine_options.inc
@@ -30,6 +30,10 @@
     if (std::strcmp(name, "form_bp") == 0) { *value = select_forms(e).bp; return TOMO_OK; }
     if (std::strcmp(name, "form_sart") == 0) { *value = select_forms(e).sart; return TOMO_OK; }
     if (std::strcmp(name, "rccl_version") == 0) { *value = g_rccl.version; return TOMO_OK; }
+    if (std::strcmp(name, "reduce_inline") == 0) { *value = e->reduce_inline; return TOMO_OK; }
+    if (std::strcmp(name, "halo_from_sweep") == 0) { *value = e->halo_from_sweep; return TOMO_OK; }
+    if (std::strcmp(name, "finalize_launches") == 0) { *value = (int)std::min<int64_t>(e->finalize_launches, 0x7FFFFFFF); return TOMO_OK; }
+    if (std::strcmp(name, "halo_gathers") == 0) { *value = (int)std::min<int64_t>(e->halo_gathers, 0x7FFFFFFF); return TOMO_OK; }
     if (std::strcmp(name, "comm_rounds") == 0) { *value = (int)std::min<int64_t>(e->comm_rounds, 0x7FFFFFFF); return TOMO_OK; }
     return fail(TOMO_ERR_ARG, std::string("unknown option ") + name);
 }
@@ -72,6 +76,8 @@
         if (value < 0 || value >= TOMO_S_COUNT) return fail(TOMO_ERR_ARG, "bad scalar slot");
         e->gnorm_slot = value; return TOMO_OK;
     }
+    if (std::strcmp(name, "reduce_inline") == 0) { e->reduce_inline = value ? 1 : 0; return TOMO_OK; }
+    if (std::strcmp(name, "halo_from_sweep") == 0) { e->halo_from_sweep = value ? 1 : 0; halo_forget(e); return TOMO_OK; }
     if (std::strcmp(name, "tv_tz") == 0) { e->tv_tz = value == 4 ? 4 : 8; return TOMO_OK; }
     if (std::strcmp(name, "tv_halo_fold") == 0) { e->tv_halo_fold = value < 0 ? -1 : (value ? 1 : 0); return TOMO_OK; }
     if (std::strcmp(name, "tv_march4") == 0) { e->tv_march4 = value ? 1 : 0; return TOMO_OK; }
diff --git a/tomo_tv_amd/csrc/engine_tv.inc b/tomo_tv_amd/csrc/engine_tv.inc
--- a/tomo_tv_amd/csrc/engine_tv.inc
+++ b/tomo_tv_amd/csrc/engine_tv.inc
@@ -10,6 +10,7 @@
 {
     NEED(e);
     HIPCHK(hipStreamSynchronize(e->stream));
+    halo_forget(e);
     e->halo_lo = device_lo ? (float *)device_lo : e->halo_lo_own;
     e->halo_hi = device_hi ? (float *)device_hi : e->halo_hi_own;
     return TOMO_OK;
@@ -41,7 +42,25 @@
     float *x; int rc; if ((rc = field_ptr(e, field, &x))) return rc;
     hipLaunchKernelGGL(k_halo_wrap, dim3((unsigned)((e->npix + 255) / 256)), dim3(256), 0, e->stream, x, e->halo_lo, e->halo_hi, (int)e->npix, e->sx, e->nx);
     LAUNCHCHK();
-    return TOMO_OK;
+    ++e->halo_gathers;
+    halo_forget(e);
+    return TOMO_OK;
+}
+
+int tomo_read_halo(tomo_engine *e, float *lo, float *hi)
+{
+    NEED(e);
+    if (!lo || !hi) return fail(TOMO_ERR_ARG, "null plane buffer");
+    HIPCHK(hipMemcpyAsync(lo, e->halo_lo, e->npix * sizeof(float), hipMemcpyDeviceToHost, e->stream));
+    HIPCHK(hipMemcpyAsync(hi, e->halo_hi, e->npix * sizeof(float), hipMemcpyDeviceToHost, e->stream));
+    HIPCHK(hipStreamSynchronize(e->stream));
+    return TOMO_OK;
+}
+
+static int tv_wrap_target(tomo_engine *e)
+{
+    if (halo_is_wrap_of(e, e->tv_target)) return TOMO_OK;
+    return tomo_halo_local(e, e->tv_target);
 }
 
 
@@ -108,10 +127,12 @@
         return reduce_end(e, TOMO_S_TV);
     }
     if (!e->d_part_tv) { if ((rc = dev_alloc((void **)&e->d_part_tv, NPART * sizeof(double), true, e->stream))) return rc; }
-    if ((rc = part_begin(e, e->d_part_tv))) return rc;
+    if ((rc = part_begin(e, e->d_part_tv, TOMO_S_TV))) return rc;
     const int yseg = 32;
     if (e->tv_lds == 1 && e->tv_march4 && e->nx % 64 == 0 && e->n % 8 == 0) {
-        hipLaunchKernelGGL((k_tv_march4<8, true, TVM_VALUE, false>), dim3(tv_march_grid(e->n, 8, e->sxc / 64, (e->n + yseg - 1) / yseg)), dim3(256), 0, e->stream, x, h, (double *)nullptr, eps, e->n, e->nx, e->sx, yseg, e->d_part_tv, TvUpd{});
+        const unsigned grid = tv_march_grid(e->n, 8, e->sxc / 64, (e->n + yseg - 1) / yseg);
+        hipLaunchKernelGGL((k_tv_march4<8, true, TVM_VALUE, false>), dim3(grid), dim3(256), 0, e->stream, x, h, (double *)nullptr, eps, e->n, e->nx, e->sx, yseg, e->d_part_tv, TvUpd{},
+                           PartFin{}, part_fin(e, e->d_part_tv, grid));
     } else if (e->tv_lds == 1) {
         hipLaunchKernelGGL((k_tv_grad_reg<8, true, false>), dim3(tv_march_grid(e->n, 8, e->sxc / 64, (e->n + yseg - 1) / yseg)), dim3(256), 0, e->stream, x, h, (float *)nullptr, (double *)nullptr, eps, e->n, e->nx, e->sx, yseg, e->d_part_tv, TvUpd{});
     } else {
@@ -137,13 +158,13 @@
     float *x, *g; int rc;
     if ((rc = get_vol(e, e->tv_target, &x))) return rc;
     if ((rc = get_scratch(e, &e->tvg, &g))) return rc;
-    if ((rc = reduce_begin(e))) return rc;
+    if ((rc = reduce_begin(e, TOMO_S_GNORM))) return rc;
     Halo h{e->halo_lo, e->halo_hi};
     if ((g_first || g_last) && !(e->tv_lds == 1 && e->tv_recompute)) return fail(TOMO_ERR_STATE, "gradient planes need the recompute form of the TV march (tv_lds = 1, tv_recompute = 1)");
     if (with_tv && e->tv_lds != 8 && e->tv_lds != 1) with_tv = false;
     if (with_tv) {
         if (!e->d_part_tv) { if ((rc = dev_alloc((void **)&e->d_part_tv, NPART * sizeof(double), true, e->stream))) return rc; }
-        if ((rc = part_begin(e, e->d_part_tv))) return rc;
+        if ((rc = part_begin(e, e->d_part_tv, TOMO_S_TV))) return rc;
     }
     {
         ProfScope ps(e, TOMO_K_TV_GRAD);
@@ -160,7 +181,8 @@
             dim3 grid(tv_march_grid(e->n, 8, e->sxc / 64, (e->n + yseg - 1) / yseg));
             if (e->tv_march4) {
                 const bool edge = e->nx % 64 != 0 || e->n % 8 != 0;
-#define TV4_NORM(WTV, EDGE, PTV) hipLaunchKernelGGL((k_tv_march4<8, WTV, TVM_NORM, EDGE>), grid, dim3(256), 0, e->stream, x, h, e->d_part, eps, e->n, e->nx, e->sx, yseg, PTV, gp)
+                const PartFin fg = part_fin(e, e->d_part, grid.x), ft = with_tv ? part_fin(e, e->d_part_tv, grid.x) : PartFin{};
+#define TV4_NORM(WTV, EDGE, PTV) hipLaunchKernelGGL((k_tv_march4<8, WTV, TVM_NORM, EDGE>), grid, dim3(256), 0, e->stream, x, h, e->d_part, eps, e->n, e->nx, e->sx, yseg, PTV, gp, fg, ft)
                 if (with_tv) { if (edge) TV4_NORM(true, true, e->d_part_tv); else TV4_NORM(true, false, e->d_part_tv); }
                 else { if (edge) TV4_NORM(false, true, (double *)nullptr); else TV4_NORM(false, false, (double *)nullptr); }
 #undef TV4_NORM
@@ -240,7 +262,7 @@
         if (slot < 0 || slot >= TOMO_S_COUNT) return fail(TOMO_ERR_ARG, "bad scalar slot");
         if ((rc = get_vol(e, track_vol, &track))) return rc;
         if ((rc = order_after_async(e))) return rc;
-        if ((rc = reduce_begin(e))) return rc;
+        if ((rc = reduce_begin(e, slot))) return rc;
     }
     if (e->tv_lds == 1 && e->tv_recompute) {
         float *alt;
@@ -277,7 +299,8 @@
             dim3 grid(tv_march_grid(e->n, 8, e->sxc / 64, (e->n + yseg - 1) / yseg));
             if (e->tv_march4) {
                 const bool edge = e->nx % 64 != 0 || e->n % 8 != 0, trk = track != nullptr, strm = up.stream != 0;
-#define TV4_UPD(EDGE, TRK, STRM) hipLaunchKernelGGL((k_tv_march4<8, false, TVM_UPDATE, EDGE, TRK, STRM>), grid, dim3(256), 0, e->stream, x, h, e->d_part, e->tv_last_eps, e->n, e->nx, e->sx, yseg, (double *)nullptr, up)
+                const PartFin fu = trk ? part_fin(e, e->d_part, grid.x) : PartFin{};
+#define TV4_UPD(EDGE, TRK, STRM) hipLaunchKernelGGL((k_tv_march4<8, false, TVM_UPDATE, EDGE, TRK, STRM>), grid, dim3(256), 0, e->stream, x, h, e->d_part, e->tv_last_eps, e->n, e->nx, e->sx, yseg, (double *)nullptr, up, fu)
                 if (edge) { if (trk) { if (strm) TV4_UPD(true, true, true); else TV4_UPD(true, true, false); } else { if (strm) TV4_UPD(true, false, true); else TV4_UPD(true, false, false); } }
                 else { if (trk) { if (strm) TV4_UPD(false, true, true); else TV4_UPD(false, true, false); } else { if (strm) TV4_UPD(false, false, true); else TV4_UPD(false, false, false); } }
 #undef TV4_UPD
@@ -287,6 +310,7 @@
         }
         LAUNCHCHK();
         e->vol[e->tv_target] = alt; e->tv_alt = x;
+        halo_forget(e);
         if (wrap && own_halo) { e->halo_lo = wl; e->halo_hi = wh; }
         else if (wrap) { if ((rc = tomo_halo_local(e, e->tv_target))) return rc; }
         if (fold) { e->halo_lo = up.ho_lo; e->halo_hi = up.ho_hi; }
@@ -383,8 +407,8 @@
     int rc;
     if (!e) return fail(TOMO_ERR_ARG, "null engine");
     const bool fold_tv = ng > 0 && (e->tv_lds == 8 || e->tv_lds == 1);
-    if (fold_tv) { if ((rc = tomo_halo_local(e, e->tv_target))) return rc; }
-    else if ((rc = tomo_tv(e, e->tv_target, eps))) return rc;
+    if (fold_tv) { if ((rc = tv_wrap_target(e))) return rc; }
+    else if ((rc = tv_wrap_target(e)) || (rc = tomo_tv_partial(e, e->tv_target, eps))) return rc;
     for (int g = 0; g < ng; ++g) {
         if ((rc = tv_grad_impl(e, eps, fold_tv && g == 0))) return rc;
         if ((rc = tv_update_impl(e, dPOCS, g == ng - 1, g == ng - 1 ? track_vol : -1, slot, g < ng - 1))) return rc;
@@ -515,6 +539,7 @@
     }
     LAUNCHCHK();
     std::swap(e->vol[e->fgp_target], e->fgp_q[0]);
+    halo_forget(e);
     ++e->vol_version[e->fgp_target];
     return TOMO_OK;
 }
diff --git a/tomo_tv_amd/csrc/kernels_common.hip.h b/tomo_tv_amd/csrc/kernels_common.hip.h
--- a/tomo_tv_amd/csrc/kernels_common.hip.h
+++ b/tomo_tv_amd/csrc/kernels_common.hip.h
@@ -78,6 +78,68 @@
     }
 }
 
+constexpr int NTICKET = 65;
+struct PartFin { double *dst; unsigned *ticket; unsigned total; };
+
+__device__ __forceinline__ void part_add_done(double *p, double v)
+{
+    double old = __hip_atomic_fetch_add(p, v, __ATOMIC_RELAXED, __HIP_MEMORY_SCOPE_AGENT);
+    asm volatile("s_waitcnt vmcnt(0)" : "+v"(old) : : "memory");
+}
+
+__device__ __forceinline__ bool part_last_unit(unsigned *ticket, unsigned total)
+{
+    unsigned last = 0;
+    if ((threadIdx.x & 63) == 0) last = __hip_atomic_fetch_add(ticket, 1u, __ATOMIC_RELAXED, __HIP_MEMORY_SCOPE_AGENT) + 1u == total ? 1u : 0u;
+    return __builtin_amdgcn_readfirstlane(last) != 0;
+}
+
+__device__ __forceinline__ bool part_last_unit2(unsigned *ticket, unsigned unit, unsigned total)
+{
+    unsigned last = 0;
+    if ((threadIdx.x & 63) == 0) {
+        const unsigned j = unit & 63u, nj = (total - j + 63u) >> 6;
+        unsigned *tj = ticket + 1 + j;
+        if (__hip_atomic_fetch_add(tj, 1u, __ATOMIC_RELAXED, __HIP_MEMORY_SCOPE_AGENT) + 1u == nj) {
+            __hip_atomic_store(tj, 0u, __ATOMIC_RELAXED, __HIP_MEMORY_SCOPE_AGENT);
+            last = __hip_atomic_fetch_add(ticket, 1u, __ATOMIC_RELAXED, __HIP_MEMORY_SCOPE_AGENT) + 1u == (total < 64u ? total : 64u) ? 1u : 0u;
+        }
+    }
+    return __builtin_amdgcn_readfirstlane(last) != 0;
+}
+
+__device__ __forceinline__ void part_finalize_wave(double *part, const PartFin &f)
+{
+    const int lane = threadIdx.x & 63;
+    double s = 0;
+#pragma unroll
+    for (int w = 0; w < NPART / 64; ++w) {
+        unsigned long long bits = __hip_atomic_exchange(reinterpret_cast<unsigned long long *>(part) + w * 64 + lane, 0ull, __ATOMIC_RELAXED, __HIP_MEMORY_SCOPE_AGENT);
+        s += wave_sum(__longlong_as_double((long long)bits));
+    }
+    if (lane == 0) {
+        *f.dst = s;
+        __hip_atomic_store(f.ticket, 0u, __ATOMIC_RELAXED, __HIP_MEMORY_SCOPE_AGENT);
+    }
+}
+
+__device__ __forceinline__ void block_accumulate_fin(double v, double *__restrict__ part, const PartFin &f)
+{
+    __shared__ double red[4];
+    v = wave_sum(v);
+    int w = threadIdx.x >> 6;
+    if ((threadIdx.x & 63) == 0) red[w] = v;
+    __syncthreads();
+    if (f.dst == nullptr) {
+        if (threadIdx.x == 0) atomicAdd(&part[blockIdx.x & (NPART - 1)], red[0] + red[1] + red[2] + red[3]);
+        return;
+    }
+    if (threadIdx.x < 64) {
+        if (threadIdx.x == 0) part_add_done(&part[blockIdx.x & (NPART - 1)], red[0] + red[1] + red[2] + red[3]);
+        if (part_last_unit(f.ticket, f.total)) part_finalize_wave(part, f);
+    }
+}
+
 __global__ __launch_bounds__(256) void k_transpose_in(const float *__restrict__ src, float *__restrict__ dst,
                                                        int ns, int64_t m, int sx)
 {
diff --git a/tomo_tv_amd/csrc/kernels_fp.hip.h b/tomo_tv_amd/csrc/kernels_fp.hip.h
--- a/tomo_tv_amd/csrc/kernels_fp.hip.h
+++ b/tomo_tv_amd/csrc/kernels_fp.hip.h
@@ -385,7 +385,8 @@
 __global__ __launch_bounds__(256) void k_fp_tile_reduce(const float *__restrict__ part, const uint32_t *__restrict__ rsptr,
                                                          const uint32_t *__restrict__ rsidx, const float *__restrict__ b,
                                                          const float *__restrict__ rowsum, float *__restrict__ out,
-                                                         double *__restrict__ dpart, int nrows, int sx, int chunk0, int ncp)
+                                                         double *__restrict__ dpart, int nrows, int sx, int chunk0, int ncp,
+                                                         PartFin fin = PartFin{})
 {
     typedef VecOf<4>::T V;
     constexpr int R = 64 / LPR, U = 8;
@@ -395,7 +396,11 @@
     int64_t item = ((int64_t)blockIdx.x * 4 + wave) * R + grp;
     int row = (int)(item / spans), span = (int)(item - (int64_t)row * spans);
     bool valid = row < nrows;
-    if (!__any(valid)) return;
+    if (!__any(valid)) {
+        if ((MODE == FP_DD || MODE == FP_POISSON) && fin.dst != nullptr &&
+            part_last_unit2(fin.ticket, blockIdx.x * 4u + (unsigned)wave, fin.total)) part_finalize_wave(dpart, fin);
+        return;
+    }
     if (!valid) row = 0;
     uint32_t kb = rsptr[row], ke = valid ? rsptr[row + 1] : kb;
     const float *pp = part + (size_t)span * (LPR * 4) + gl * 4;
@@ -447,7 +452,12 @@
     }
     if (MODE == FP_DD || MODE == FP_POISSON) {
         local = wave_sum(local);
-        if (lane == 0) atomicAdd(&dpart[blockIdx.x & (NPART - 1)], local);
+        if (fin.dst == nullptr) {
+            if (lane == 0) atomicAdd(&dpart[blockIdx.x & (NPART - 1)], local);
+        } else {
+            if (lane == 0) part_add_done(&dpart[blockIdx.x & (NPART - 1)], local);
+            if (part_last_unit2(fin.ticket, blockIdx.x * 4u + (unsigned)wave, fin.total)) part_finalize_wave(dpart, fin);
+        }
     }
 }
 
diff --git a/tomo_tv_amd/csrc/kernels_tv.hip.h b/tomo_tv_amd/csrc/kernels_tv.hip.h
--- a/tomo_tv_amd/csrc/kernels_tv.hip.h
+++ b/tomo_tv_amd/csrc/kernels_tv.hip.h
@@ -482,7 +482,8 @@
 #define TV4_OCC __attribute__((amdgpu_waves_per_eu((MODE == TVM_UPDATE && !TRACK) ? TV4_UPD_WAVES : 4, (MODE == TVM_UPDATE && !TRACK) ? TV4_UPD_WAVES : 8)))
 template <int TZ, bool WITH_TV, int MODE, bool EDGE, bool TRACK = false, bool STREAM = false>
 __global__ __launch_bounds__(256) TV4_OCC void k_tv_march4(const float *__restrict__ x, Halo h, double *__restrict__ part, float eps,
-                                                    int n, int nx, int sx, int yseg, double *__restrict__ part_tv, TvUpd up)
+                                                    int n, int nx, int sx, int yseg, double *__restrict__ part_tv, TvUpd up,
+                                                    PartFin fin = PartFin{}, PartFin fin_tv = PartFin{})
 {
     static_assert(MODE == TVM_NORM || MODE == TVM_UPDATE || MODE == TVM_VALUE, "modes without a stored gradient");
     static_assert(MODE != TVM_VALUE || WITH_TV, "the value mode sums the TV integrand");
@@ -740,10 +741,11 @@
 #undef TV4_ROW
 #undef TV4_RINV
     }
-    if (MODE != TVM_VALUE) block_accumulate(acc, part);
+    if (MODE == TVM_NORM || (MODE == TVM_UPDATE && TRACK)) block_accumulate_fin(acc, part, fin);
+    else if (MODE != TVM_VALUE) block_accumulate(acc, part);
     if (WITH_TV) {
         __syncthreads();
-        block_accumulate(tvacc, part_tv);
+        block_accumulate_fin(tvacc, part_tv, fin_tv);
     }
 }
 
diff --git a/tomo_tv_amd/csrc/sart_resident.hip.h b/tomo_tv_amd/csrc/sart_resident.hip.h
--- a/tomo_tv_amd/csrc/sart_resident.hip.h
+++ b/tomo_tv_amd/csrc/sart_resident.hip.h
@@ -28,6 +28,10 @@
     unsigned epoch0, spin_limit;
     float beta;
     long long *prof;
+    double *fin_dst;
+    unsigned *fin_ticket;
+    float *halo_lo, *halo_hi;
+    int nx;
 };
 #ifdef RS_PROF
 #define RS_STAMP(q) { const long long now_ = (long long)__builtin_amdgcn_s_memrealtime(); if (wave == 0) tacc[q] += now_ - tprev; tprev = now_; }
@@ -168,6 +172,7 @@
     __shared__ float rs_sbuf[RS_WAVES][64];
     __shared__ float rs_dump[RS_WAVES][64];
     __shared__ int rs_dirty, rs_go, rs_store;
+    __shared__ int rs_failed;
     const int lane = threadIdx.x & 63;
     const int wave = __builtin_amdgcn_readfirstlane(threadIdx.x >> 6);
     v32f xlo, xhi;
@@ -182,10 +187,11 @@
         tile = (int)blockIdx.x % A->ntiles; grp = (int)blockIdx.x / A->ntiles; ngrp = (int)gridDim.x / A->ntiles;
         chunk = A->chunk0 + grp; chunk_end = A->chunk0 + A->nchunk; steps = A->steps;
     }
+    if (threadIdx.x == 0) rs_failed = 0;
     for (int it = 0; chunk < chunk_end; chunk += ngrp, ++it) {
         const uint32_t voff = (uint32_t)(chunk * 64 + lane) * 4u;
         {
-            if (threadIdx.x == 0) { rs_dirty = 0; rs_go = rs_abort_ld(rs_args()->abort_word) == 0 ? 1 : 0; }
+            if (threadIdx.x == 0) { rs_dirty = 0; rs_go = rs_abort_ld(rs_args()->abort_word) == 0 ? 1 : 0; if (rs_go == 0) rs_failed = 1; }
             __syncthreads();
             if (rs_go == 0) break;
         }
@@ -390,6 +396,7 @@
                 if (ok && tile == 0)
                     __hip_atomic_store((__attribute__((address_space(1))) int *)(A->done_host + chunk), (int)A->seq, __ATOMIC_RELAXED, __HIP_MEMORY_SCOPE_SYSTEM);
                 rs_store = ok ? 1 : 0;
+                if (!ok) rs_failed = 1;
             }
             __syncthreads();
             if (rs_store == 0) continue;
@@ -425,7 +432,8 @@
                     for (int l = 0; l < 64; ++l) local += red[l];
                     const uint32_t slot = (blockIdx.x & (NPART - 1)) * 8u;
                     double *part = A->part;
-                    asm volatile("global_atomic_add_f64 %0, %1, %2" :: "v"(slot), "v"(local), "s"(part) : "memory");
+                    asm volatile("global_atomic_add_f64 v[58:59], %0, %1, %2 sc0\n"
+                                 "s_waitcnt vmcnt(0)" :: "v"(slot), "v"(local), "s"(part) : "v58", "v59", "memory");
                 }
             } else {
                 asm volatile("s_cmp_eq_u32 %[in], 0\n"
@@ -437,6 +445,39 @@
                              :
                              : "{v[64:95]}"(xlo), "{v[96:127]}"(xhi), [in] "s"(in), [xb] "s"(xb), [voff] "v"(voff), [ps] "s"(ps), [rs] "s"(rs)
                              : "s36", "s37", "scc", "memory");
+            }
+            if (in && A->halo_lo) {
+                const int nx = A->nx, clast = (nx - 1) >> 6;
+                if (chunk == 0 || chunk == clast) {
+                    float *hl = A->halo_lo, *hh = A->halo_hi;
+                    const bool w_hi = chunk == 0 && lane == 0, w_lo = chunk == clast && lane == ((nx - 1) & 63);
+#pragma unroll
+                    for (int q = 0; q < 64; ++q) {
+                        const int pix = (y0 + (q >> 3)) * n + z0 + (q & 7);
+                        const float v = q < 32 ? xlo[q & 31] : xhi[q & 31];
+                        if (w_hi) hh[pix] = v;
+                        if (w_lo) hl[pix] = v;
+                    }
+                }
+            }
+        }
+    }
+    {
+        RsArgsP A = rs_args();
+        if (A->fin_dst) {
+            __syncthreads();
+            if (wave == 0) {
+                unsigned *ticket = A->fin_ticket;
+                unsigned t = 0;
+                if (lane == 0) {
+                    const unsigned mine = 1u + (rs_failed ? 0x10000u : 0u);
+                    t = __hip_atomic_fetch_add(ticket, mine, __ATOMIC_RELAXED, __HIP_MEMORY_SCOPE_AGENT) + mine;
+                }
+                t = __builtin_amdgcn_readfirstlane(t);
+                if ((t & 0xFFFFu) == gridDim.x) {
+                    if ((t >> 16) == 0) part_finalize_wave(A->part, PartFin{A->fin_dst, ticket, gridDim.x});
+                    else if (lane == 0) __hip_atomic_store(ticket, 0u, __ATOMIC_RELAXED, __HIP_MEMORY_SCOPE_AGENT);
+                }
             }
         }
     }
diff --git a/tomo_tv_amd/csrc/tomo_engine.hip b/tomo_tv_amd/csrc/tomo_engine.hip
--- a/tomo_tv_amd/csrc/tomo_engine.hip
+++ b/tomo_tv_amd/csrc/tomo_engine.hip
@@ -237,6 +237,13 @@
     hipEvent_t ev_snap = nullptr;
     bool snap_pending = false;
     bool part_open[3] = {false, false, false};
+    unsigned *d_tickets = nullptr;
+    int part_slot[3] = {-1, -1, -1};
+    bool part_inline[3] = {false, false, false};
+    int reduce_inline = 1;
+    int64_t finalize_launches = 0, halo_gathers = 0;
+    int halo_from_sweep = 1;
+    struct { int vol = -1; uint64_t ver = 0; const float *lo = nullptr, *hi = nullptr; } halo_cur;
     hipStream_t aux = nullptr;
     hipEvent_t ev_fork = nullptr, ev_join = nullptr;
     bool async_pending = false;
@@ -305,10 +312,18 @@
     return TOMO_OK;
 }
 
+static void halo_forget(tomo_engine *e) { e->halo_cur.vol = -1; }
+static bool halo_is_wrap_of(const tomo_engine *e, int vol)
+{
+    return e->halo_from_sweep && vol >= 0 && vol < TOMO_VOL_SLOTS && e->halo_cur.vol == vol && e->halo_cur.ver == e->vol_version[vol]
+           && e->halo_cur.lo == e->halo_lo && e->halo_cur.hi == e->halo_hi;
+}
+
 static int get_vol(tomo_engine *e, int id, float **out)
 {
     if (id < 0 || id >= TOMO_VOL_SLOTS) return fail(TOMO_ERR_ARG, "bad volume id");
     ++e->vol_version[id];
+    if (id == e->halo_cur.vol || (e->old_is_recon && (id == TOMO_VOL_RECON || id == TOMO_VOL_RECON_OLD))) halo_forget(e);
     if (e->old_is_recon && (id == TOMO_VOL_RECON || id == TOMO_VOL_RECON_OLD)) {
         e->old_is_recon = false;
         float *src, *dst; int rc;
@@ -392,25 +407,43 @@
     ~ProfScope() { if (stop) (void)hipEventRecord(stop, st); }
 };
 
-static bool &part_open(tomo_engine *e, const double *part)
-{
-    return part == e->d_part_tv ? e->part_open[2] : part == e->d_part_aux ? e->part_open[1] : e->part_open[0];
-}
-static int part_begin(tomo_engine *e, double *part)
-{
-    bool &open = part_open(e, part);
-    if (open) HIPCHK(hipMemsetAsync(part, 0, NPART * sizeof(double), e->stream));
-    open = true;
-    return TOMO_OK;
-}
+static int part_index(const tomo_engine *e, const double *part)
+{
+    return part == e->d_part_tv ? 2 : part == e->d_part_aux ? 1 : 0;
+}
+static int part_begin(tomo_engine *e, double *part, int slot = -1)
+{
+    const int i = part_index(e, part);
+    if (e->part_open[i]) {
+        HIPCHK(hipMemsetAsync(part, 0, NPART * sizeof(double), e->stream));
+        HIPCHK(hipMemsetAsync(e->d_tickets + i * NTICKET, 0, NTICKET * sizeof(unsigned), e->stream));
+    }
+    e->part_open[i] = true;
+    e->part_slot[i] = slot;
+    e->part_inline[i] = false;
+    return TOMO_OK;
+}
+static PartFin part_fin(tomo_engine *e, const double *part, unsigned units)
+{
+    const int i = part_index(e, part);
+    if (!e->reduce_inline || !e->part_open[i] || e->part_slot[i] < 0 || units == 0) return PartFin{nullptr, nullptr, units};
+    e->part_inline[i] = true;
+    return PartFin{e->d_scal + e->part_slot[i], e->d_tickets + i * NTICKET, units};
+}
+static void part_fin_revoke(tomo_engine *e, const double *part) { e->part_inline[part_index(e, part)] = false; }
 static int part_end(tomo_engine *e, double *part, int slot)
 {
-    hipLaunchKernelGGL(k_finalize, dim3(1), dim3(NPART), 0, e->stream, part, e->d_scal + slot);
-    LAUNCHCHK();
-    part_open(e, part) = false;
-    return TOMO_OK;
-}
-static int reduce_begin(tomo_engine *e) { return part_begin(e, e->d_part); }
+    const int i = part_index(e, part);
+    if (!(e->part_inline[i] && e->part_slot[i] == slot)) {
+        hipLaunchKernelGGL(k_finalize, dim3(1), dim3(NPART), 0, e->stream, part, e->d_scal + slot);
+        LAUNCHCHK();
+        ++e->finalize_launches;
+    }
+    e->part_open[i] = false;
+    e->part_inline[i] = false;
+    return TOMO_OK;
+}
+static int reduce_begin(tomo_engine *e, int slot = -1) { return part_begin(e, e->d_part, slot); }
 static int reduce_end(tomo_engine *e, int slot) { return part_end(e, e->d_part, slot); }
 
 constexpr int TV_YSEG_MIN = 8, TV_WAVES_WANTED = 4096;
```

Result: slower. 10.46 Gvoxel-updates/s (-1.4%).
